# VisionLearningGroup/UDA_PoseEstimation

Hardware: AMD Instinct MI355X
Metric: images/sec (student+teacher step) 256x256 b=32 (higher is better)
Workload: dtype bf16; 1 GPU; pose_resnet101 K=16 mean-teacher step (student fwd+bwd on 2x32, teacher fwd on 32, JointsMSE+Cons, Adam, EMA), 256x256, b=32/GPU, no AdaIN (BASELINE.json configs[1]); global_batch=32, parallelism=dp1

## Files before the change

include/udapose.h:

```cpp
#ifndef UDAPOSE_H
#define UDAPOSE_H
#include <stddef.h>
#include <stdint.h>
#ifdef __cplusplus
extern "C" {
#endif

#define UDAPOSE_OK 0
#define UDAPOSE_ERR_ARG (-1)
#define UDAPOSE_ERR_LAUNCH (-2)
#define UDAPOSE_ERR_UNSUPPORTED (-3)
#define UDAPOSE_ERR_NOT_PREPARED (-4)

int udapose_version(void);
int udapose_elem_kind(void);

typedef struct {
    int igemm_tile, igemm_h3, igemm_lean, igemm_short_lds, igemm_tap0;
    int wgrad_tile, wgrad_ksplit, wgrad_fastgeo;
    int wgrad_group, wgrad_stages, wgrad_group_stem;
    int bn_bwd_fused, bn_fwd_chunked, bn_bwd_chunked, bn_bwd_pre_legacy;
    int igemm_wg_min;
    int wgrad_row3;
    int bn3_mask;
    int stem_fused;
    int debug_sync;
    int igemm_big_min;
    int patch_conv;
    int eval_fold;
    int bn_xcd_rows;
    int wgrad_det;
    int igemm_ns3_k;
    void* timeline;
} udapose_policy;
void udapose_policy_default(udapose_policy* p);

typedef struct {
    int N, Hi, Wi, Ci;
    int Co, KH, KW, stride, pad;
    int transposed;
    int reflect;
    int upsample;
    const udapose_policy* policy;
} udapose_conv_desc;
int udapose_conv_prepare(const udapose_conv_desc* d);

#define UDAPOSE_EPI_RELU 1
#define UDAPOSE_EPI_OUT_F32 2
#define UDAPOSE_EPI_F32 4
#define UDAPOSE_EPI_SPLIT 8
void udapose_conv_out_hw(const udapose_conv_desc* d, int* Ho, int* Wo);
int udapose_conv_stat_rows(const udapose_conv_desc* d);
int udapose_conv2d_fwd(void* stream, const udapose_conv_desc* d, const void* x, const void* w_fwd, void* y, const void* res,
                       const float* bias, float* stats, int epilogue_flags);
int udapose_conv2d_bwd_data(void* stream, const udapose_conv_desc* d, const void* dy, const void* w_bwd, void* dx, const void* res,
                            int out_f32);
int udapose_conv_bwd_stat_rows(const udapose_conv_desc* d);
int udapose_conv2d_bwd_data_bn(void* stream, const udapose_conv_desc* d, const void* dy, const void* w_bwd, void* dx, const void* res,
                               int out_f32, const void* bn_y, const void* bn_z, const float* bn_mean, const float* bn_invstd,
                               const float* bn_gamma, const float* bn_beta, float* slab);
int udapose_conv2d_bwd_weight(void* stream, const udapose_conv_desc* d, const void* dy, const void* x, float* dw, int accumulate);
int udapose_cast_f32_bf16(void* stream, const float* src, void* dst, size_t n);
int udapose_transpose_cast(void* stream, const float* src, void* dst, int A, int T, int B);
int udapose_pack_strided(void* stream, const float* src, void* dst, int A, int KH, int KWp, int KW, int Bp, int B, long sa, long skh,
                         long skw, long sb);

int udapose_nchw_f32_to_nhwc_bf16(void* stream, const float* src, void* dst, int N, int C, int HW, int Cpad);
int udapose_nchw_f32_to_nhwc_f32(void* stream, const float* src, float* dst, int N, int C, int HW, int Cpad);
int udapose_nchw_f32_to_nhwc_split(void* stream, const float* src, void* dst, int N, int C, int HW, int Cpad);
int udapose_f32_to_split(void* stream, const float* src, void* dst, size_t n);
int udapose_split_to_f32(void* stream, const void* src, float* dst, size_t n);
int udapose_nhwc_to_nchw_f32(void* stream, const void* src, int src_is_f32, float* dst, int N, int C, int HW, int Cstride,
                             const float* lo, const float* hi);

int udapose_bn_finalize(void* stream, const float* stats, int stat_rows, int C, double count, const float* gamma, const float* beta,
                        float* running_mean, float* running_var, long long* num_batches_tracked, float momentum, float eps,
                        float* scale, float* shift, float* save_mean, float* save_invstd);
int udapose_bn_eval_coeff(void* stream, int C, const float* gamma, const float* beta, const float* running_mean,
                          const float* running_var, float eps, float* scale, float* shift);
int udapose_bn_apply(void* stream, const void* y, const void* res, void* z, size_t numel, int C, const float* scale, const float* shift,
                     int relu);
int udapose_bn_bwd_rows(size_t npix);
int udapose_bn_bwd(void* stream, const void* dz, int dz_is_f32, const void* z, const void* y, void* dy, void* gout, size_t npix, int C,
                   const float* gamma, const float* save_mean, const float* save_invstd, int relu, float* slab, float* coef,
                   float* dgamma, float* dbeta, float beta_acc, const float* beta);
int udapose_bn_bwd_pre(void* stream, const void* g, int g_is_f32, const void* y, void* dy, size_t npix, int C, const float* gamma,
                       const float* save_mean, const float* save_invstd, const float* slab, int rows, float* coef, float* dgamma,
                       float* dbeta, float beta_acc);

int udapose_maxpool3x3s2_fwd(void* stream, const void* x, void* y, unsigned char* idx, int N, int H, int W, int C);
int udapose_maxpool3x3s2_bwd(void* stream, const void* dy, const unsigned char* idx, void* dx, int N, int H, int W, int C);
int udapose_maxpool2x2_ceil(void* stream, const void* x, void* y, int N, int H, int W, int C);
int udapose_maxpool2x2_ceil_f32(void* stream, const float* x, float* y, int N, int H, int W, int C);
int udapose_maxpool2x2_ceil_split(void* stream, const void* x, void* y, int N, int H, int W, int C);

typedef void* udapose_net_t;
int udapose_net_create(const int layers[4], int num_keypoints, int N, int H, int W, int fp32, udapose_net_t* out);
void udapose_net_destroy(udapose_net_t net);
int udapose_net_num_params(udapose_net_t net);
int udapose_net_num_buffers(udapose_net_t net);
long long udapose_net_param_numel(udapose_net_t net, int i);
size_t udapose_net_wpack_bytes(udapose_net_t net);
size_t udapose_net_act_bytes(udapose_net_t net);
size_t udapose_net_ws_bytes(udapose_net_t net);
void udapose_net_out_shape(udapose_net_t net, int shape[4]);
int udapose_net_set_policy(udapose_net_t net, const udapose_policy* p);
int udapose_net_get_policy(udapose_net_t net, udapose_policy* p);
int udapose_net_bind(udapose_net_t net, const void* const* h_params, void* const* h_buffers, void* wpack);
int udapose_net_bind_grads(udapose_net_t net, void* const* h_grads);
int udapose_net_pack_weights(udapose_net_t net, void* stream, const void* const* h_params, void* wpack, int with_bwd);
int udapose_net_forward(udapose_net_t net, void* stream, const float* x_nchw, const void* const* h_params, void* const* h_buffers,
                        const void* wpack, void* act, void* ws, float* out_nchw, int training, float momentum);
int udapose_net_apply_running(udapose_net_t net, void* stream, const void* act, void* const* h_buffers, float momentum);
int udapose_axpy_f32(void* stream, float* y, const float* x, size_t n);
int udapose_net_backward(udapose_net_t net, void* stream, const float* dout_nchw, const void* const* h_params, const void* wpack,
                         void* act, void* ws, void* const* h_grads, float beta);
int udapose_net_backward_part(udapose_net_t net, void* stream, const float* dout_nchw, const void* const* h_params, const void* wpack,
                              void* act, void* ws, void* const* h_grads, float beta, int part);
int udapose_net_backward_phase(udapose_net_t net, void* stream, const float* dout_nchw, const void* const* h_params, const void* wpack,
                               void* act, void* ws, void* const* h_grads, float beta, int part, int phase);
int udapose_net_wgrad_pair(udapose_net_t net, void* stream, const void* act_a, void* ws_a, void* const* h_grads_a, float beta_a,
                           const void* act_b, void* ws_b, void* const* h_grads_b, float beta_b, int part);
long long udapose_net_grad_split_param(udapose_net_t net);

int udapose_joints_mse_fwd(void* stream, const float* pred, const float* gt, const float* w, int R, int HW, float* rows, float* mean_out);
int udapose_joints_mse_bwd(void* stream, const float* pred, const float* gt, const float* w, const float* gscale, int R, int HW,
                           float* dpred);
int udapose_cons_loss_fwd(void* stream, const float* stu, const float* tea, const unsigned char* mask, int R, int HW, float* rows,
                          float* mean_out);
int udapose_cons_loss_bwd(void* stream, const float* stu, const float* tea, const unsigned char* mask, const float* gscale, int R,
                          int HW, float* dstu);
int udapose_mask_count(void* stream, const unsigned char* mask, size_t n, float* count);
int udapose_cons_loss_valid_fwd(void* stream, const float* stu, const float* tea, const unsigned char* mask, const unsigned char* valid,
                                const float* valid_count, int R, int K, int HW, float* rows, float* mean_out);
int udapose_cons_loss_valid_bwd(void* stream, const float* stu, const float* tea, const unsigned char* mask, const unsigned char* valid,
                                const float* valid_count, const float* gscale, int R, int K, int HW, float* dstu);
int udapose_joints_kl_fwd(void* stream, const float* pred, const float* gt, const float* w, float epsilon, int R, int group, int HW, float* rows,
                          float* stats, float* out);
int udapose_joints_kl_bwd(void* stream, const float* pred, const float* gt, const float* w, float epsilon, const float* stats,
                          const float* gscale, int R, int HW, float* dpred);
int udapose_entropy_loss_fwd(void* stream, const float* x, int R, int group, int HW, float threshold, float* rows, float* stats, float* out,
                             float* count);
int udapose_entropy_loss_bwd(void* stream, const float* x, const float* rows, const float* stats, const float* count, const float* gscale,
                             float threshold, int R, int HW, float* dx);
int udapose_cons_softmax_fwd(void* stream, const float* stu, const float* tea, const unsigned char* mask, const unsigned char* valid,
                             const float* valid_count, int R, int K, int HW, float* rows, float* stats, float* out);
int udapose_cons_softmax_bwd(void* stream, const float* stu, const float* tea, const unsigned char* mask, const unsigned char* valid,
                             const float* valid_count, const float* stats, const float* gscale, int R, int K, int HW, float* dstu);
int udapose_cons_kl_fwd(void* stream, const float* stu, const float* tea, const unsigned char* mask, const unsigned char* valid,
                        const float* valid_count, int log_target, int R, int K, int HW, float* rows, float* stats, float* out);
int udapose_cons_kl_bwd(void* stream, const float* stu, const float* tea, const unsigned char* mask, const unsigned char* valid,
                        const float* valid_count, int log_target, const float* stats, const float* gscale, int R, int K, int HW, float* dstu);
int udapose_heatmap_argmax(void* stream, const float* hm, int R, int H, int W, float* maxvals, int* flat_idx, float* preds_xy,
                           float* rectified, const float* patch, int rad);
int udapose_kth_mask(void* stream, const float* act, const float* tea_mask, int n, int k, float* thr_out, unsigned char* mask,
                     const float* act_local, int n_local);
int udapose_pck(void* stream, const float* pred_xy, const float* gt_xy, int B, int K, float norm_x, float norm_y, float thr, float* acc,
                float* avg_cnt);

int udapose_multi_chunk(void);
int udapose_ema_multi(void* stream, const long long* tgt_ptrs, const long long* src_ptrs, const long long* sizes, const int* blk_tensor,
                      const long long* blk_off, int nblocks, float alpha, float one_minus_alpha);
int udapose_adam_multi(void* stream, const long long* p, const long long* g, const long long* m, const long long* v,
                       const long long* sizes, const int* blk_tensor, const long long* blk_off, int nblocks, float lr, float beta1,
                       float beta2, float eps, float weight_decay, int step, float grad_scale, float* dev_state);
int udapose_sgd_multi(void* stream, const long long* p, const long long* g, const long long* buf, const long long* sizes,
                      const int* blk_tensor, const long long* blk_off, int nblocks, float lr, float momentum, float weight_decay,
                      int nesterov, int first_step, float grad_scale, float* dev_state);

int udapose_net_bind_update(udapose_net_t student, udapose_net_t teacher, void* const* h_params_s, void* const* h_grads,
                            void* const* h_exp_avg, void* const* h_exp_avg_sq, void* const* h_params_t, void* wpack_s, void* wpack_t);
int udapose_net_fused_update(udapose_net_t student, udapose_net_t teacher, void* stream, void* const* h_params_s, void* const* h_grads,
                             void* const* h_exp_avg, void* const* h_params_t, void* wpack_s, void* wpack_t, float lr, float beta1,
                             float beta2, float eps, float weight_decay, int step, float grad_scale, float* dev_state, float alpha,
                             float one_minus_alpha, int do_adam, long long grad2_delta_bytes);
// ... 67 lines not shown
```

uda_poseestimation_amd/_hip.py:

```python
import ctypes as C
import os

import torch

_HERE = os.path.dirname(os.path.abspath(__file__))
LIB_PATH = os.path.join(_HERE, "libudapose_hip.so")
LIB_PATHS = {"bf16": LIB_PATH, "fp16": os.path.join(_HERE, "libudapose_hip_f16.so")}
_libs = {}

vp, ci, cf, cd, sz, ll, cl = C.c_void_p, C.c_int, C.c_float, C.c_double, C.c_size_t, C.c_longlong, C.c_long


class Policy(C.Structure):
    _fields_ = [(k, C.c_int) for k in ("igemm_tile", "igemm_h3", "igemm_lean", "igemm_short_lds", "igemm_tap0", "wgrad_tile", "wgrad_ksplit",
                                       "wgrad_fastgeo", "wgrad_group", "wgrad_stages", "wgrad_group_stem", "bn_bwd_fused", "bn_fwd_chunked",
                                       "bn_bwd_chunked", "bn_bwd_pre_legacy", "igemm_wg_min", "wgrad_row3", "bn3_mask", "stem_fused", "debug_sync", "igemm_big_min", "patch_conv",
                                       "eval_fold", "bn_xcd_rows", "wgrad_det", "igemm_ns3_k")] + [("timeline", C.c_void_p)]


def policy(**overrides):
    p = Policy()
    lib().udapose_policy_default(C.byref(p))
    for k, v in overrides.items():
        if k not in dict(Policy._fields_):
            raise KeyError(f"udapose_policy has no field {k!r}")
        setattr(p, k, v)
    return p


class ConvDesc(C.Structure):
    _fields_ = [(k, C.c_int) for k in ("N", "Hi", "Wi", "Ci", "Co", "KH", "KW", "stride", "pad", "transposed", "reflect", "upsample")] + \
               [("policy", C.POINTER(Policy))]


_SIGS = {
    "udapose_version": (ci, []),
    "udapose_elem_kind": (ci, []),
    "udapose_grad_scaler_check": (ci, [vp, vp, vp, vp, vp, ci, vp]),
    "udapose_grad_scaler_check2": (ci, [vp, vp, vp, vp, vp, ci, vp, ll]),
    "udapose_grad_scaler_update": (ci, [vp, vp, cf, cf, ci]),
    "udapose_policy_default": (None, [vp]),
    "udapose_conv_prepare": (ci, [vp]),
    "udapose_net_set_policy": (ci, [vp, vp]),
    "udapose_net_get_policy": (ci, [vp, vp]),
    "udapose_net_bind": (ci, [vp, vp, vp, vp]),
    "udapose_net_bind_grads": (ci, [vp, vp]),
    "udapose_conv_out_hw": (None, [vp, vp, vp]),
    "udapose_conv_stat_rows": (ci, [vp]),
    "udapose_conv2d_fwd": (ci, [vp, vp, vp, vp, vp, vp, vp, vp, ci]),
    "udapose_conv2d_bwd_data": (ci, [vp, vp, vp, vp, vp, vp, ci]),
    "udapose_conv_bwd_stat_rows": (ci, [vp]),
    "udapose_conv2d_bwd_data_bn": (ci, [vp, vp, vp, vp, vp, vp, ci, vp, vp, vp, vp, vp, vp, vp]),
    "udapose_conv2d_bwd_weight": (ci, [vp, vp, vp, vp, vp, ci]),
    "udapose_cast_f32_bf16": (ci, [vp, vp, vp, sz]),
    "udapose_transpose_cast": (ci, [vp, vp, vp, ci, ci, ci]),
    "udapose_pack_strided": (ci, [vp, vp, vp, ci, ci, ci, ci, ci, ci, cl, cl, cl, cl]),
    "udapose_nchw_f32_to_nhwc_bf16": (ci, [vp, vp, vp, ci, ci, ci, ci]),
    "udapose_nchw_f32_to_nhwc_f32": (ci, [vp, vp, vp, ci, ci, ci, ci]),
    "udapose_nhwc_to_nchw_f32": (ci, [vp, vp, ci, vp, ci, ci, ci, ci, vp, vp]),
    "udapose_nchw_f32_to_nhwc_split": (ci, [vp, vp, vp, ci, ci, ci, ci]),
    "udapose_f32_to_split": (ci, [vp, vp, vp, sz]),
    "udapose_split_to_f32": (ci, [vp, vp, vp, sz]),
    "udapose_maxpool2x2_ceil_split": (ci, [vp, vp, vp, ci, ci, ci, ci]),
    "udapose_adain_split": (ci, [vp, vp, vp, vp, ci, ci, ci, ci, cf, cf, vp, vp]),
    "udapose_bn_finalize": (ci, [vp, vp, ci, ci, cd, vp, vp, vp, vp, vp, cf, cf, vp, vp, vp, vp]),
    "udapose_bn_eval_coeff": (ci, [vp, ci, vp, vp, vp, vp, cf, vp, vp]),
    "udapose_bn_apply": (ci, [vp, vp, vp, vp, sz, ci, vp, vp, ci]),
    "udapose_bn_bwd_rows": (ci, [sz]),
    "udapose_bn_bwd": (ci, [vp, vp, ci, vp, vp, vp, vp, sz, ci, vp, vp, vp, ci, vp, vp, vp, vp, cf, vp]),
    "udapose_bn_bwd_pre": (ci, [vp, vp, ci, vp, vp, sz, ci, vp, vp, vp, vp, ci, vp, vp, vp, cf]),
    "udapose_maxpool3x3s2_fwd": (ci, [vp, vp, vp, vp, ci, ci, ci, ci]),
    "udapose_maxpool3x3s2_bwd": (ci, [vp, vp, vp, vp, ci, ci, ci, ci]),
    "udapose_maxpool2x2_ceil": (ci, [vp, vp, vp, ci, ci, ci, ci]),
    "udapose_maxpool2x2_ceil_f32": (ci, [vp, vp, vp, ci, ci, ci, ci]),
    "udapose_net_create": (ci, [vp, ci, ci, ci, ci, ci, vp]),
    "udapose_net_destroy": (None, [vp]),
    "udapose_net_num_params": (ci, [vp]),
    "udapose_net_num_buffers": (ci, [vp]),
    "udapose_net_param_numel": (ll, [vp, ci]),
    "udapose_net_wpack_bytes": (sz, [vp]),
    "udapose_net_act_bytes": (sz, [vp]),
    "udapose_net_ws_bytes": (sz, [vp]),
    "udapose_net_out_shape": (None, [vp, vp]),
    "udapose_net_pack_weights": (ci, [vp, vp, vp, vp, ci]),
    "udapose_net_forward": (ci, [vp, vp, vp, vp, vp, vp, vp, vp, vp, ci, cf]),
    "udapose_net_apply_running": (ci, [vp, vp, vp, vp, cf]),
    "udapose_axpy_f32": (ci, [vp, vp, vp, sz]),
    "udapose_net_backward": (ci, [vp, vp, vp, vp, vp, vp, vp, vp, cf]),
    "udapose_net_backward_part": (ci, [vp, vp, vp, vp, vp, vp, vp, vp, cf, ci]),
    "udapose_net_backward_phase": (ci, [vp, vp, vp, vp, vp, vp, vp, vp, cf, ci, ci]),
    "udapose_net_wgrad_pair": (ci, [vp, vp, vp, vp, vp, cf, vp, vp, vp, cf, ci]),
    "udapose_net_grad_split_param": (ll, [vp]),
    "udapose_net_bind_update": (ci, [vp, vp, vp, vp, vp, vp, vp, vp, vp]),
    "udapose_net_fused_update": (ci, [vp, vp, vp, vp, vp, vp, vp, vp, vp, cf, cf, cf, cf, cf, ci, cf, vp, cf, cf, ci, ll]),
    "udapose_joints_mse_fwd": (ci, [vp, vp, vp, vp, ci, ci, vp, vp]),
    "udapose_joints_mse_bwd": (ci, [vp, vp, vp, vp, vp, ci, ci, vp]),
    "udapose_cons_loss_fwd": (ci, [vp, vp, vp, vp, ci, ci, vp, vp]),
    "udapose_cons_loss_bwd": (ci, [vp, vp, vp, vp, vp, ci, ci, vp]),
    "udapose_mask_count": (ci, [vp, vp, sz, vp]),
    "udapose_cons_loss_valid_fwd": (ci, [vp, vp, vp, vp, vp, vp, ci, ci, ci, vp, vp]),
    "udapose_cons_loss_valid_bwd": (ci, [vp, vp, vp, vp, vp, vp, vp, ci, ci, ci, vp]),
    "udapose_joints_kl_fwd": (ci, [vp, vp, vp, vp, cf, ci, ci, ci, vp, vp, vp]),
    "udapose_joints_kl_bwd": (ci, [vp, vp, vp, vp, cf, vp, vp, ci, ci, vp]),
    "udapose_entropy_loss_fwd": (ci, [vp, vp, ci, ci, ci, cf, vp, vp, vp, vp]),
    "udapose_entropy_loss_bwd": (ci, [vp, vp, vp, vp, vp, vp, cf, ci, ci, vp]),
    "udapose_cons_softmax_fwd": (ci, [vp, vp, vp, vp, vp, vp, ci, ci, ci, vp, vp, vp]),
    "udapose_cons_softmax_bwd": (ci, [vp, vp, vp, vp, vp, vp, vp, vp, ci, ci, ci, vp]),
    "udapose_cons_kl_fwd": (ci, [vp, vp, vp, vp, vp, vp, ci, ci, ci, ci, vp, vp, vp]),
    "udapose_cons_kl_bwd": (ci, [vp, vp, vp, vp, vp, vp, ci, vp, vp, ci, ci, ci, vp]),
    "udapose_heatmap_argmax": (ci, [vp, vp, ci, ci, ci, vp, vp, vp, vp, vp, ci]),
    "udapose_kth_mask": (ci, [vp, vp, vp, ci, ci, vp, vp, vp, ci]),
    "udapose_pck": (ci, [vp, vp, vp, ci, ci, cf, cf, cf, vp, vp]),
    "udapose_multi_chunk": (ci, []),
    "udapose_ema_multi": (ci, [vp, vp, vp, vp, vp, vp, ci, cf, cf]),
    "udapose_adam_multi": (ci, [vp, vp, vp, vp, vp, vp, vp, vp, ci, cf, cf, cf, cf, cf, ci, cf, vp]),
    "udapose_sgd_multi": (ci, [vp, vp, vp, vp, vp, vp, vp, ci, cf, cf, cf, ci, ci, cf, vp]),
    "udapose_comm_pack_bf16": (ci, [vp, vp, ll, vp, ll]),
    "udapose_comm_shard_mean": (ci, [vp, vp, ci, ll, vp]),
    "udapose_comm_unpack_bf16": (ci, [vp, vp, vp, ll]),
    "udapose_adain": (ci, [vp, vp, vp, vp, ci, ci, ci, ci, cf, cf, vp]),
    "udapose_adain_f32": (ci, [vp, vp, vp, vp, ci, ci, ci, ci, cf, cf, vp]),
    "udapose_adain_alpha_dev": (ci, [vp, vp, vp, vp, ci, ci, ci, ci, cf, vp, vp, ci]),
    "udapose_patch_paste": (ci, [vp, vp, vp, ci, ci, ci, ci, ci]),
    "udapose_occlusion_pick": (ci, [vp, vp, vp, vp, ci, ci, ci, cd, ci, cf, cf, ci, vp, vp]),
    "udapose_select_rows": (ci, [vp, vp, vp, vp, vp, ci, sz]),
    "udapose_aug_affine_u8": (ci, [vp, vp, vp, vp, ci, ci, ci]),
    "udapose_aug_color_op": (ci, [vp, vp, vp, vp, vp, ci, ci]),
    "udapose_aug_to_tensor": (ci, [vp, vp, vp, ci, ci, vp, vp]),
    "udapose_aug_gaussian_blur_u8": (ci, [vp, vp, vp, vp, ci, ci, ci]),
    "udapose_aug_resized_crop_u8": (ci, [vp, vp, vp, vp, vp, vp, vp, ci, ci, ci, ci, ci]),
    "udapose_gaussian_labels": (ci, [vp, vp, vp, vp, vp, ci, ci, ci, cd, cd, vp, ci]),
    "udapose_split_saturations": (ci, [ci, vp]),
    "udapose_mean_views": (ci, [vp, vp, ci, vp, sz]),
    "udapose_draw_labelmap_ori": (ci, [vp, vp, vp, vp, vp, vp, ci, ci, ci, cf, vp, ci]),
    "udapose_prof_begin": (None, []),
    "udapose_prof_end": (ci, [vp]),
    "udapose_affine_nearest": (ci, [vp, vp, vp, vp, ci, ci, ci, ci, ci, ci]),
    "udapose_recon_thetas": (ci, [vp, vp, ci, cd, vp, vp]),
    "udapose_conv_bwd_ws_bytes": (ll, [vp]),
    "udapose_conv_bwd_prepare": (ci, [vp]),
    "udapose_conv2d_bwd_data_reflect_padded": (ci, [vp, vp, vp, vp, vp]),
    "udapose_reflect_fold": (ci, [vp, vp, ci, vp, ci, vp, vp, vp, vp, cf, vp, ci, vp, ci, ci, ci, ci, cf]),
    "udapose_conv2d_bwd_data_reflect": (ci, [vp, vp, vp, vp, vp, vp, vp]),
    "udapose_conv2d_bwd_weight_reflect": (ci, [vp, vp, vp, vp, vp, ci, vp, cf]),
# ... 72 lines not shown
```

uda_poseestimation_amd/csrc/capi.hip:

```cpp
#include <cstdio>
#include "conv_plan.h"
#include "../../include/udapose.h"

int pw_nchw_f32_to_nhwc_bf16(hipStream_t, const float*, elem_t*, int, int, int, int);
int pw_nhwc_to_nchw_f32(hipStream_t, const void*, int, float*, int, int, int, int, const float*, const float*);
int pw_cast_f32_bf16(hipStream_t, const float*, elem_t*, size_t);
int pw_transpose_cast(hipStream_t, const float*, elem_t*, int, int, int);
int pw_pack_strided(hipStream_t, const float*, elem_t*, int, int, int, int, int, int, long, long, long, long);
int pw_bn_finalize(hipStream_t, const float*, int, int, double, const float*, const float*, float*, float*, long long*, float, float, float*, float*,
                   float*, float*, const float*);
int pw_bn_eval_coeff(hipStream_t, int, const float*, const float*, const float*, const float*, float, float*, float*);
int pw_bn_apply(hipStream_t, const elem_t*, const elem_t*, elem_t*, size_t, int, const float*, const float*, int, unsigned char*, int);
int pw_bn_bwd_rows(size_t);
int pw_bn_bwd_pre(hipStream_t, const void*, int, const elem_t*, elem_t*, size_t, int, const float*, const float*, const float*, const float*, int, float*,
                  float*, float*, float, int, int);
int pw_bn_bwd(hipStream_t, const void*, int, const elem_t*, const elem_t*, elem_t*, elem_t*, size_t, int, const float*, const float*, const float*, int,
              float*, float*, float*, float*, float, const float*, int);
int pw_maxpool3x3s2_fwd(hipStream_t, const elem_t*, elem_t*, unsigned char*, int, int, int, int);

size_t conv_bwd_ws_bytes(const ConvGeom& g);
int conv_bwd_prepare(const ConvGeom& g);
int conv_dgrad_reflect_padded(hipStream_t s, const ConvGeom& g, const elem_t* dy, const elem_t* w_bwd, elem_t* dP);
int reflect_fold(hipStream_t s, const elem_t* dP, int up, const elem_t* x, int mask, const float* stats, const float* gs_s, const elem_t* t,
                 const float* gs_c, float c_scale, const float* add_nchw, int add_c, elem_t* dx, int N, int H, int W, int C, float term_scale);
// ... 35 lines not shown
int opt_ema(hipStream_t, const long long*, const long long*, const long long*, const int*, const long long*, int, float, float);
int opt_adam(hipStream_t, const long long*, const long long*, const long long*, const long long*, const long long*, const int*, const long long*, int,
             float, float, float, float, float, int, float, float*);
int opt_sgd(hipStream_t, const long long*, const long long*, const long long*, const long long*, const int*, const long long*, int, float, float, float,
            int, int, float, float*);
int opt_grad_check(hipStream_t, const long long*, const long long*, const int*, const long long*, int, float*, long long);
int opt_scaler_update(hipStream_t, float*, float, float, int);
int comm_pack_bf16(hipStream_t, const float*, long long, void*, long long);
int comm_shard_mean(hipStream_t, const void*, int, long long, void*);
int comm_unpack_bf16(hipStream_t, const void*, float*, long long);
int adain_launch(hipStream_t, const elem_t*, const elem_t*, elem_t*, int, int, int, int, float, float, const float*, float*);
int aug_affine_u8(hipStream_t, const unsigned char*, unsigned char*, const long long*, int, int, int);
int aug_color_op(hipStream_t, unsigned char*, const int*, const float*, int*, int, int);
int aug_gaussian_blur_u8(hipStream_t, unsigned char*, unsigned char*, const unsigned int*, int, int, int);
int aug_resized_crop_u8(hipStream_t, const unsigned char*, unsigned char*, unsigned char*, const int*, const int*, const int*, int, int, int, int, int);
int aug_to_tensor(hipStream_t, const unsigned char*, float*, int, int, const float*, const float*);
int aug_gaussian_labels(hipStream_t, const double*, const float*, float*, float*, int, int, int, double, double, const float*, int);
int aug_draw_labelmap_ori(hipStream_t, const float*, const float*, const unsigned char*, float*, float*, int, int, int, float, const float*, int);
int affine_warp_chain(hipStream_t, const float*, float*, const float*, int, int, int, int, int, int);
int affine_recon_thetas(hipStream_t, const double*, int, double, float*, float*);
int affine_mean_views(hipStream_t, const float* const*, int, float*, size_t);
unsigned long long sp_sat_read_adain(int);
unsigned long long sp_sat_read_igemm(int);
unsigned long long sp_sat_read_patchconv(int);
unsigned long long sp_sat_read_pointwise(int);
int patch_paste(hipStream_t, float*, const int*, int, int, int, int, int);
int occlusion_pick(hipStream_t, const float*, const int*, const float*, int, int, int, double, int, float, float, int, int*, unsigned char*);
int select_rows(hipStream_t, float*, const float*, const float*, const unsigned char*, int, size_t);
int net_apply_running(void*, hipStream_t, const void*, void* const*, float);
int pw_axpy(hipStream_t, float*, const float*, size_t);
void prof_begin();
int prof_end(double*);
void* net_create(const int layers[4], int K, int N, int H, int W, int mode);
void net_destroy(void*);
void net_set_policy(void*, const Policy&);
const Policy& net_get_policy(void*);
int net_bind(void*, const void* const*, void* const*, void*);
int net_bind_grads(void*, void* const*);
long long net_grad_split_param(void*);
int net_bind_update(void*, void*, void* const*, void* const*, void* const*, void* const*, void* const*, void*, void*);
int net_fused_update(void*, void*, hipStream_t, void* const*, void* const*, void* const*, void* const*, void*, void*, float, float, float, float, float,
                     int, float, float*, float, float, int, long long);
int net_num_params(void*);
int net_num_buffers(void*);
long long net_param_numel(void*, int);
size_t net_wpack_bytes(void*);
size_t net_act_bytes(void*);
size_t net_ws_bytes(void*);
void net_out_shape(void*, int*);
int net_pack_weights(void*, hipStream_t, const void* const*, void*, int);
int net_forward(void*, hipStream_t, const float*, const void* const*, void* const*, const void*, void*, void*, float*, int, float);
int net_backward(void*, hipStream_t, const float*, const void* const*, const void*, void*, void*, void* const*, float, int, int);
int net_wgrad_pair(void*, hipStream_t, const void*, void*, void* const*, float, const void*, void*, void* const*, float, int);

static Policy from_c(const udapose_policy& c) {
    Policy p;
    p.igemm_tile = c.igemm_tile; p.igemm_h3 = c.igemm_h3; p.igemm_lean = c.igemm_lean; p.igemm_short_lds = c.igemm_short_lds;
    p.igemm_tap0 = c.igemm_tap0; p.wgrad_tile = c.wgrad_tile; p.wgrad_ksplit = c.wgrad_ksplit; p.wgrad_fastgeo = c.wgrad_fastgeo;
    p.wgrad_group = c.wgrad_group; p.wgrad_stages = c.wgrad_stages > 0 ? c.wgrad_stages : 128; p.wgrad_group_stem = c.wgrad_group_stem;
    p.bn_bwd_fused = c.bn_bwd_fused; p.bn_fwd_chunked = c.bn_fwd_chunked; p.bn_bwd_chunked = c.bn_bwd_chunked;
    p.bn_bwd_pre_legacy = c.bn_bwd_pre_legacy; p.igemm_wg_min = c.igemm_wg_min; p.wgrad_row3 = c.wgrad_row3; p.bn3_mask = c.bn3_mask; p.stem_fused = c.stem_fused; p.debug_sync = c.debug_sync; p.igemm_big_min = c.igemm_big_min; p.patch_conv = c.patch_conv; p.eval_fold = c.eval_fold; p.bn_xcd_rows = c.bn_xcd_rows; p.igemm_ns3_k = c.igemm_ns3_k; p.wgrad_det = c.wgrad_det; p.timeline = (unsigned long long*)c.timeline;
    return p;
}
static void to_c(const Policy& p, udapose_policy* c) {
    c->igemm_tile = p.igemm_tile; c->igemm_h3 = p.igemm_h3; c->igemm_lean = p.igemm_lean; c->igemm_short_lds = p.igemm_short_lds;
    c->igemm_tap0 = p.igemm_tap0; c->wgrad_tile = p.wgrad_tile; c->wgrad_ksplit = p.wgrad_ksplit; c->wgrad_fastgeo = p.wgrad_fastgeo;
    c->wgrad_group = p.wgrad_group; c->wgrad_stages = p.wgrad_stages; c->wgrad_group_stem = p.wgrad_group_stem;
    c->bn_bwd_fused = p.bn_bwd_fused; c->bn_fwd_chunked = p.bn_fwd_chunked; c->bn_bwd_chunked = p.bn_bwd_chunked;
    c->bn_bwd_pre_legacy = p.bn_bwd_pre_legacy; c->igemm_wg_min = p.igemm_wg_min; c->wgrad_row3 = p.wgrad_row3; c->bn3_mask = p.bn3_mask; c->stem_fused = p.stem_fused; c->debug_sync = p.debug_sync; c->igemm_big_min = p.igemm_big_min; c->patch_conv = p.patch_conv; c->eval_fold = p.eval_fold; c->bn_xcd_rows = p.bn_xcd_rows; c->igemm_ns3_k = p.igemm_ns3_k; c->wgrad_det = p.wgrad_det; c->timeline = p.timeline;
}
struct Geom {
    Policy pol;
    ConvGeom g;
    explicit Geom(const udapose_conv_desc* d)
        : g{d->N, d->Hi, d->Wi, d->Ci, d->Co, d->KH, d->KW, d->stride, d->pad, d->transposed, d->reflect, d->upsample} {
        if (d->policy) { pol = from_c(*d->policy); g.pol = &pol; }
    }
};
#define S(x) ((hipStream_t)(x))
#define B16(x) ((elem_t*)(x))
#define CB16(x) ((const elem_t*)(x))

extern "C" {

int udapose_version(void) { return 200; }
int udapose_elem_kind(void) { return UDAPOSE_ELEM_KIND; }

void udapose_policy_default(udapose_policy* p) { if (p) to_c(default_policy(), p); }
void udapose_conv_out_hw(const udapose_conv_desc* d, int* Ho, int* Wo) { Geom G(d); *Ho = G.g.Ho(); *Wo = G.g.Wo(); }
int udapose_conv_stat_rows(const udapose_conv_desc* d) { Geom G(d); return conv_stat_rows(G.g); }
int udapose_conv_prepare(const udapose_conv_desc* d) { if (!d) return UDAPOSE_ERR_ARG; Geom G(d); return conv_prepare(G.g); }
int udapose_conv2d_fwd(void* stream, const udapose_conv_desc* d, const void* x, const void* w_fwd, void* y, const void* res, const float* bias,
                       float* stats, int flags) {
    if (!d || !x || !w_fwd || !y) return UDAPOSE_ERR_ARG;
    ConvEpilogue e;
    e.res = CB16(res); e.bias = bias; e.stats = stats; e.relu = (flags & UDAPOSE_EPI_RELU) != 0; e.out_f32 = (flags & UDAPOSE_EPI_OUT_F32) != 0; e.f32 = (flags & UDAPOSE_EPI_F32) != 0;
    e.split = (flags & UDAPOSE_EPI_SPLIT) != 0;
    if (e.split && e.f32) return UDAPOSE_ERR_ARG;
    Geom G(d);
    return conv_fprop(S(stream), G.g, CB16(x), CB16(w_fwd), y, e);
}
int udapose_conv2d_bwd_data(void* stream, const udapose_conv_desc* d, const void* dy, const void* w_bwd, void* dx, const void* res, int out_f32) {
    if (!d || !dy || !w_bwd || !dx) return UDAPOSE_ERR_ARG;
    Geom G(d);
    return conv_dgrad(S(stream), G.g, CB16(dy), CB16(w_bwd), dx, CB16(res), out_f32);
}
int udapose_conv_bwd_stat_rows(const udapose_conv_desc* d) { if (!d) return UDAPOSE_ERR_ARG; Geom G(d); return conv_dgrad_stat_rows(G.g); }
int udapose_conv2d_bwd_data_bn(void* stream, const udapose_conv_desc* d, const void* dy, const void* w_bwd, void* dx, const void* res, int out_f32,
                               const void* bn_y, const void* bn_z, const float* bn_mean, const float* bn_invstd, const float* bn_gamma,
                               const float* bn_beta, float* slab) {
    if (!d || !dy || !w_bwd || !dx || !bn_y || !bn_mean || !bn_invstd || !slab) return UDAPOSE_ERR_ARG;
    DgradBnStat st;
    st.y = CB16(bn_y); st.z = CB16(bn_z); st.mean = bn_mean; st.invstd = bn_invstd; st.gamma = bn_gamma; st.beta = bn_beta; st.slab = slab;
    Geom G(d);
    return conv_dgrad(S(stream), G.g, CB16(dy), CB16(w_bwd), dx, CB16(res), out_f32, &st);
}
int udapose_conv2d_bwd_weight(void* stream, const udapose_conv_desc* d, const void* dy, const void* x, float* dw, int accumulate) {
    if (!d || !dy || !x || !dw) return UDAPOSE_ERR_ARG;
    Geom G(d);
    return conv_wgrad(S(stream), G.g, CB16(dy), CB16(x), dw, accumulate, -1);
}
int udapose_cast_f32_bf16(void* stream, const float* src, void* dst, size_t n) { return pw_cast_f32_bf16(S(stream), src, B16(dst), n); }
// ... 69 lines not shown
    return *out ? UDAPOSE_OK : UDAPOSE_ERR_ARG;
}
void udapose_net_destroy(udapose_net_t n) { net_destroy(n); }
int udapose_net_set_policy(udapose_net_t n, const udapose_policy* p) {
    if (!n || !p) return UDAPOSE_ERR_ARG;
    net_set_policy(n, from_c(*p));
    return UDAPOSE_OK;
}
int udapose_net_get_policy(udapose_net_t n, udapose_policy* p) {
    if (!n || !p) return UDAPOSE_ERR_ARG;
    to_c(net_get_policy(n), p);
    return UDAPOSE_OK;
}
int udapose_net_bind(udapose_net_t n, const void* const* params, void* const* buffers, void* wpack) {
    if (!n || !params || !wpack) return UDAPOSE_ERR_ARG;
    return net_bind(n, params, buffers, wpack);
}
int udapose_net_bind_grads(udapose_net_t n, void* const* grads) {
    if (!n || !grads) return UDAPOSE_ERR_ARG;
    return net_bind_grads(n, grads);
}
int udapose_net_num_params(udapose_net_t n) { return net_num_params(n); }
int udapose_net_num_buffers(udapose_net_t n) { return net_num_buffers(n); }
long long udapose_net_param_numel(udapose_net_t n, int i) { return net_param_numel(n, i); }
size_t udapose_net_wpack_bytes(udapose_net_t n) { return net_wpack_bytes(n); }
size_t udapose_net_act_bytes(udapose_net_t n) { return net_act_bytes(n); }
size_t udapose_net_ws_bytes(udapose_net_t n) { return net_ws_bytes(n); }
void udapose_net_out_shape(udapose_net_t n, int shape[4]) { net_out_shape(n, shape); }
int udapose_net_pack_weights(udapose_net_t n, void* stream, const void* const* params, void* wpack, int with_bwd) {
    return net_pack_weights(n, S(stream), params, wpack, with_bwd);
}
int udapose_net_forward(udapose_net_t n, void* stream, const float* x, const void* const* params, void* const* buffers, const void* wpack, void* act,
                        void* ws, float* out, int training, float momentum) {
    return net_forward(n, S(stream), x, params, buffers, wpack, act, ws, out, training, momentum);
}
int udapose_net_apply_running(udapose_net_t n, void* stream, const void* act, void* const* buffers, float momentum) {
    return net_apply_running(n, S(stream), act, buffers, momentum);
}
int udapose_axpy_f32(void* stream, float* y, const float* x, size_t n) { return pw_axpy(S(stream), y, x, n); }
int udapose_net_backward(udapose_net_t n, void* stream, const float* dout, const void* const* params, const void* wpack, void* act, void* ws,
                         void* const* grads, float beta) {
    return net_backward(n, S(stream), dout, params, wpack, act, ws, grads, beta, 0, 0);
}
int udapose_net_backward_part(udapose_net_t n, void* stream, const float* dout, const void* const* params, const void* wpack, void* act,
                              void* ws, void* const* grads, float beta, int part) {
    if (part != 1 && part != 2) return UDAPOSE_ERR_ARG;
    return net_backward(n, S(stream), dout, params, wpack, act, ws, grads, beta, part, 0);
}
int udapose_net_wgrad_pair(udapose_net_t n, void* stream, const void* act_a, void* ws_a, void* const* grads_a, float beta_a, const void* act_b,
                           void* ws_b, void* const* grads_b, float beta_b, int part) {
    if (!n || !act_a || !ws_a || !grads_a || !act_b || !ws_b || !grads_b) return UDAPOSE_ERR_ARG;
    return net_wgrad_pair(n, S(stream), act_a, ws_a, grads_a, beta_a, act_b, ws_b, grads_b, beta_b, part);
}
int udapose_net_backward_phase(udapose_net_t n, void* stream, const float* dout, const void* const* params, const void* wpack, void* act,
                               void* ws, void* const* grads, float beta, int part, int phase) {
    if (!n) return UDAPOSE_ERR_ARG;
    return net_backward(n, S(stream), dout, params, wpack, act, ws, grads, beta, part, phase);
}
long long udapose_net_grad_split_param(udapose_net_t n) { return net_grad_split_param(n); }
int udapose_net_bind_update(udapose_net_t student, udapose_net_t teacher, void* const* params_s, void* const* grads, void* const* exp_avg,
                            void* const* exp_avg_sq, void* const* params_t, void* wpack_s, void* wpack_t) {
    if (!student || !teacher || !params_s || !grads || !exp_avg || !exp_avg_sq || !params_t || !wpack_s || !wpack_t) return UDAPOSE_ERR_ARG;
    return net_bind_update(student, teacher, params_s, grads, exp_avg, exp_avg_sq, params_t, wpack_s, wpack_t);
}
int udapose_net_fused_update(udapose_net_t student, udapose_net_t teacher, void* stream, void* const* params_s, void* const* grads,
                             void* const* exp_avg, void* const* params_t, void* wpack_s, void* wpack_t, float lr, float beta1, float beta2,
                             float eps, float weight_decay, int step, float grad_scale, float* dev_state, float alpha, float one_minus_alpha,
                             int do_adam, long long grad2_delta_bytes) {
    if (!student || !teacher) return UDAPOSE_ERR_ARG;
    return net_fused_update(student, teacher, S(stream), params_s, grads, exp_avg, params_t, wpack_s, wpack_t, lr, beta1, beta2, eps, weight_decay,
                            step, grad_scale, dev_state, alpha, one_minus_alpha, do_adam, grad2_delta_bytes);
}

int udapose_joints_mse_fwd(void* stream, const float* pred, const float* gt, const float* w, int R, int HW, float* rows, float* mean_out) {
    return hm_sqdiff_rows(S(stream), pred, gt, w, nullptr, R, HW, 0.5f, rows, mean_out, nullptr, nullptr, 1);
}
int udapose_joints_mse_bwd(void* stream, const float* pred, const float* gt, const float* w, const float* gscale, int R, int HW, float* dpred) {
    return hm_sqdiff_bwd(S(stream), pred, gt, w, nullptr, gscale, (float)(1.0 / ((double)R * HW)), R, HW, dpred, nullptr, nullptr, 1);
}
int udapose_cons_loss_fwd(void* stream, const float* stu, const float* tea, const unsigned char* mask, int R, int HW, float* rows, float* mean_out) {
    return hm_sqdiff_rows(S(stream), stu, tea, nullptr, mask, R, HW, 1.0f, rows, mean_out, nullptr, nullptr, 1);
}
int udapose_cons_loss_bwd(void* stream, const float* stu, const float* tea, const unsigned char* mask, const float* gscale, int R, int HW, float* dstu) {
    return hm_sqdiff_bwd(S(stream), stu, tea, nullptr, mask, gscale, (float)(2.0 / ((double)R * HW)), R, HW, dstu, nullptr, nullptr, 1);
}
int udapose_mask_count(void* stream, const unsigned char* mask, size_t n, float* count) {
    if (!mask || !count) return UDAPOSE_ERR_ARG;
    return hm_mask_count(S(stream), mask, n, count);
}
int udapose_cons_loss_valid_fwd(void* stream, const float* stu, const float* tea, const unsigned char* mask, const unsigned char* valid,
                                const float* valid_count, int R, int K, int HW, float* rows, float* mean_out) {
    if (!valid || !valid_count) return UDAPOSE_ERR_ARG;
    return hm_sqdiff_rows(S(stream), stu, tea, nullptr, mask, R, HW, 1.0f, rows, mean_out, valid, valid_count, K);
}
int udapose_cons_loss_valid_bwd(void* stream, const float* stu, const float* tea, const unsigned char* mask, const unsigned char* valid,
                                const float* valid_count, const float* gscale, int R, int K, int HW, float* dstu) {
    if (!valid || !valid_count) return UDAPOSE_ERR_ARG;
    return hm_sqdiff_bwd(S(stream), stu, tea, nullptr, mask, gscale, (float)(2.0 / ((double)R * HW)), R, HW, dstu, valid, valid_count, K);
}
int udapose_joints_kl_fwd(void* stream, const float* pred, const float* gt, const float* w, float epsilon, int R, int group, int HW, float* rows,
                          float* stats, float* out) {
    return sml_kl_fwd(S(stream), pred, gt, w, epsilon, R, group, HW, rows, stats, out);
}
int udapose_joints_kl_bwd(void* stream, const float* pred, const float* gt, const float* w, float epsilon, const float* stats,
                          const float* gscale, int R, int HW, float* dpred) {
    return sml_kl_bwd(S(stream), pred, gt, w, epsilon, stats, gscale, R, HW, dpred);
// ... 206 lines not shown
```

uda_poseestimation_amd/csrc/conv_plan.h:

```cpp
#pragma once
#include <atomic>
#include <mutex>
#include <vector>
#include "igemm.h"

struct Policy {
    int igemm_tile = -1;
    int igemm_h3 = 1;
    int igemm_lean = 1;
    int igemm_short_lds = 1;
    int igemm_tap0 = 1;
    int wgrad_tile = -1;
    int wgrad_ksplit = -1;
    int wgrad_fastgeo = 2;
    int wgrad_group = 1;
    int wgrad_stages = 128;
    int wgrad_group_stem = 1;
    int bn_bwd_fused = 1;
    int bn_fwd_chunked = 1;
    int bn_bwd_chunked = 1;
    int bn_bwd_pre_legacy = 0;
    int igemm_wg_min = 512;
    int wgrad_row3 = 1;
    int bn3_mask = 1;
    int stem_fused = 1;
    int igemm_big_min = 0;
    int patch_conv = 2;
    int eval_fold = 1;
    int bn_xcd_rows = 1;
    int wgrad_det = 1;
    int igemm_ns3_k = 0;
    int debug_sync = 0;
    unsigned long long* timeline = nullptr;
};
inline const Policy& default_policy() { static const Policy p; return p; }

template <typename F>
inline void once_per_device(std::atomic<unsigned long long>& done, std::mutex& mu, F&& f) {
    int dev = 0;
    (void)hipGetDevice(&dev);
    const unsigned long long bit = 1ull << (dev & 63);
    if (done.load(std::memory_order_acquire) & bit) return;
    std::lock_guard<std::mutex> lk(mu);
    if (done.load(std::memory_order_relaxed) & bit) return;
    f();
    done.fetch_or(bit, std::memory_order_release);
}

struct ConvGeom {
    int N, Hi, Wi, Ci;
    int Co, KH, KW, stride, pad;
    int transposed;
    int reflect;
    int upsample;
    const Policy* pol = nullptr;
    const Policy& policy() const { return pol ? *pol : default_policy(); }
    int Ho() const { return transposed ? (Hi - 1) * stride - 2 * pad + KH : (((Hi << upsample) + 2 * pad - KH) / stride + 1); }
    int Wo() const { return transposed ? (Wi - 1) * stride - 2 * pad + KW : (((Wi << upsample) + 2 * pad - KW) / stride + 1); }
    bool smallc() const { return Ci == 8; }
    int KWp() const { return smallc() ? ((KW + 7) & ~7) : KW; }
    int wtaps() const { return KH * KWp(); }
};

struct TapPlan {
    std::vector<IgTap> taps;
    int nclass = 1;
    IgClass cls[4];
    const IgTap* d_taps = nullptr;
};

const TapPlan* get_tap_plan(const ConvGeom& g, int direction, hipStream_t stream = nullptr);
int conv_prepare(const ConvGeom& g);

int igemm_pick_tile(int M, int Co, int nclass, int K, int h3_ok, const Policy& pol);
int conv_h3_ok(const ConvGeom& g);
int igemm_stat_rows(int M, int Co, int nclass, int tile);
int igemm_launch(IgParams& p, int tile, hipStream_t stream, const Policy& pol);
int wgrad_pick_tile(int Rdim, int Cdim, int smallc, const Policy& pol);
int wgrad_launch(WgParams& p, int tile, int accumulate, hipStream_t stream, const Policy& pol);
int wgrad_parts_plan(int M, int Ci, int Co, int total_taps, int* tile_out);
int wgrad_launch_parts(WgParams& p, float* parts, hipStream_t stream);
#define WG_CLASSES 2
int wgrad_group_plan(WgParams& p, int accumulate, int stages_per_block, const Policy& pol);
int wgrad_group_launch(hipStream_t stream, int tile, const WgParams* d_tab, const WgGroupBlk* d_blk, int per_xcd, const void* x_base,
                       const void* dy_base, void* dw_base, const WgParams* d_tab2 = nullptr, const WgGroupBlk* d_blk2 = nullptr,
                       const void* x_base2 = nullptr, const void* dy_base2 = nullptr, void* dw_base2 = nullptr);

struct ConvEpilogue {
    const elem_t* res = nullptr;
    const float* bias = nullptr;
    const float* scale = nullptr;
    float* stats = nullptr;
    int relu = 0;
    int out_f32 = 0;
    int f32 = 0;
    int split = 0;
};
int conv_fprop(hipStream_t s, const ConvGeom& g, const elem_t* x, const elem_t* w_fwd, void* y, const ConvEpilogue& e);
int patch_conv_ok(const ConvGeom& g, const ConvEpilogue& e);
int patch_conv_fprop(hipStream_t s, const ConvGeom& g, const void* x, const void* w_fwd, void* y, const ConvEpilogue& e);
struct DgradBnStat {
    const elem_t* y = nullptr;
    const elem_t* z = nullptr;
    const unsigned char* mask = nullptr;
    const float* mean = nullptr; const float* invstd = nullptr; const float* gamma = nullptr; const float* beta = nullptr;
    float* slab = nullptr;
    int rows = 0;
};
int conv_dgrad(hipStream_t s, const ConvGeom& g, const elem_t* dy, const elem_t* w_bwd, void* dx, const elem_t* res, int out_f32,
               DgradBnStat* bs = nullptr);
int conv_wgrad(hipStream_t s, const ConvGeom& g, const elem_t* dy, const elem_t* x, float* dw, int accumulate, int rows_valid);
int conv_wgrad_params(const ConvGeom& g, const elem_t* dy, const elem_t* x, float* dw, int rows_valid, WgParams* out, double* flops);
int conv_prof_before(hipStream_t s, int kind, double flops);
void conv_prof_after(hipStream_t s, int token);
int conv_stat_rows(const ConvGeom& g);
int conv_dgrad_stat_rows(const ConvGeom& g);
```

uda_poseestimation_amd/csrc/net.hip:

```cpp
#include <algorithm>
#include <deque>
#include <cstdio>
#include <cstdlib>
#include <string>
#include <vector>
#include "conv_plan.h"

int pw_nchw_f32_to_nhwc_bf16(hipStream_t, const float*, elem_t*, int, int, int, int);
int pw_nhwc_to_nchw_f32(hipStream_t, const void*, int, float*, int, int, int, int, const float*, const float*);
int pw_cast_f32_bf16(hipStream_t, const float*, elem_t*, size_t);
int pw_transpose_cast(hipStream_t, const float*, elem_t*, int, int, int);
int pw_pack_strided(hipStream_t, const float*, elem_t*, int, int, int, int, int, int, long, long, long, long);
int pw_unpack_strided(hipStream_t, const float*, float*, int, int, int, int, int, int, long, long, long, long, float);
int pw_bn_finalize(hipStream_t, const float*, int, int, double, const float*, const float*, float*, float*, long long*, float, float, float*, float*,
                   float*, float*, const float*);
int pw_bn_eval_coeff(hipStream_t, int, const float*, const float*, const float*, const float*, float, float*, float*);
int pw_bn_apply(hipStream_t, const elem_t*, const elem_t*, elem_t*, size_t, int, const float*, const float*, int, unsigned char*, int);
int pw_bn_bwd_rows(size_t);
int pw_bn_bwd(hipStream_t, const void*, int, const elem_t*, const elem_t*, elem_t*, elem_t*, size_t, int, const float*, const float*, const float*, int,
              float*, float*, float*, float*, float, const float*, int);
int pw_bn_bwd_pre(hipStream_t, const void*, int, const elem_t*, elem_t*, size_t, int, const float*, const float*, const float*, const float*, int, float*,
                  float*, float*, float, int, int);
int pw_maxpool3x3s2_fwd(hipStream_t, const elem_t*, elem_t*, unsigned char*, int, int, int, int);
int pw_maxpool3x3s2_bwd(hipStream_t, const elem_t*, const unsigned char*, elem_t*, int, int, int, int);
int pw_bn_relu_maxpool3x3s2(hipStream_t, const elem_t*, elem_t*, unsigned char*, int, int, int, int, const float*, const float*);
int pw_bn_bwd_pooled(hipStream_t, const elem_t*, const unsigned char*, int, int, const elem_t*, elem_t*, size_t, int, const float*, const float*,
                     const float*, float*, float*, float*, float*, float, const float*);
int pw_plane_sum(hipStream_t, const float*, float*, int, int, int, float);
int pw_bn_running_update(hipStream_t, const float*, int, float*, float*, long long*, float);
int pw_bn_running_update_multi(hipStream_t, const BnRunJob*, int, int, const void*, float);
int pw_bn_train_fused(hipStream_t, const elem_t*, const elem_t*, elem_t*, size_t, int, const float*, int, const float*, const float*, float*, float*,
                      long long*, float, float, float*, int, int, unsigned char*);
int pw_zero_multi(hipStream_t, const ZeroJob*, int, void*);
int pw_pack_multi(hipStream_t, const void*, const int*, const int*, int);
int pw_nchw_f32_to_nhwc_f32(hipStream_t, const float*, float*, int, int, int, int);
size_t opt_tail_job_bytes();
int opt_chunk();
void opt_tail_job_fill(void*, float*, const float*, float*, float*, float*, void*, void*, void*, void*, int, int, int, int, long long);
int opt_tail(hipStream_t, const void*, const int*, const int*, int, float, float, float, float, float, int, float, float*, float, float, int, long long, int);
int pw_transpose_f32(hipStream_t, const float*, float*, int, int, int);
int pw_pack_strided_f32(hipStream_t, const float*, float*, int, int, int, int, int, int, long, long, long, long);
int pw_bn_apply_f32(hipStream_t, const float*, const float*, float*, size_t, int, const float*, const float*, int);
int pw_maxpool3x3s2_fwd_f32(hipStream_t, const float*, float*, unsigned char*, int, int, int, int);
int pw_nchw_f32_to_nhwc_split(hipStream_t, const float*, void*, int, int, int, int, void*);
int pw_f32_to_split(hipStream_t, const float*, void*, size_t);
int pw_transpose_split(hipStream_t, const float*, void*, int, int, int);
int pw_pack_strided_split(hipStream_t, const float*, void*, int, int, int, int, int, int, long, long, long, long);
int pw_bn_apply_split(hipStream_t, const float*, const void*, void*, size_t, int, const float*, const float*, int, void*, void*, unsigned char*, int);
int pw_bn_train_fused_split(hipStream_t, const float*, const void*, void*, size_t, int, const float*, int, const float*, const float*, float*, float*,
                            long long*, float, float, float*, int, int, void*, void*, unsigned char*);
int pw_maxpool3x3s2_fwd_split(hipStream_t, const void*, void*, unsigned char*, int, int, int, int, void*);

namespace {

inline size_t align_up(size_t v, size_t a = 256) { return (v + a - 1) / a * a; }
static thread_local int t_dbg_sync = 0;
struct DbgSyncScope { int prev; explicit DbgSyncScope(int on) : prev(t_dbg_sync) { t_dbg_sync = on; } ~DbgSyncScope() { t_dbg_sync = prev; } };
#define CK(expr) do { int _e = (expr); \
    if (t_dbg_sync) { fprintf(stderr, "[udapose] net.hip:%d %s\n", __LINE__, #expr); fflush(stderr); \
        if (hipDeviceSynchronize() != hipSuccess) { fprintf(stderr, "[udapose] FAILED at net.hip:%d\n", __LINE__); return UDAPOSE_ERR_LAUNCH; } } \
    if (_e != UDAPOSE_OK) return _e; } while (0)

struct ConvL {
    ConvGeom g;
    int w_idx = -1;
    int bias_idx = -1;
    size_t wf_off = 0, wb_off = 0;
    size_t in_off = 0;
    size_t y_off = 0;
    size_t fin_off = 0, fy_off = 0;
    size_t dy_off = 0;
};
struct BnL {
    int C = 0;
    int g_idx = -1, b_idx = -1;
    int rm_idx = -1, rv_idx = -1, nbt_idx = -1;
    size_t save_off = 0;
    size_t z_off = 0;
    size_t mask_off = 0;
    size_t fz_off = 0;
    size_t npix = 0;
};
struct Block {
    ConvL c1, c2, c3, cd;
    BnL b1, b2, b3, bd;
    bool has_ds = false;
    size_t in_off = 0, zd_off = 0;
    size_t fin_off = 0, fzd_off = 0;
    size_t npix_in = 0;
};

struct Net {
    int layers[4], K, N, H, W;
    int split_dz_idx = -1;
    Policy policy;
    int f32 = 0;
    int strict = 0;
    int fwd_only = 0;
    struct Scratch { size_t need[6] = {0, 0, 0, 0, 0, 0}, off[6] = {0, 0, 0, 0, 0, 0}; bool sizing = false; } sc;
    int deconv_bias = 0;
    size_t es = 2;
    int n_params = 0, n_buffers = 0;
    std::vector<long long> param_numel;
    ConvL stem; BnL stem_bn;
    size_t x8_off = 0, pool_off = 0, poolidx_off = 0;
    size_t fx8_off = 0, fpool_off = 0;
    int Hs = 0, Ws = 0, Hp = 0, Wp = 0;
    std::vector<Block> blocks;
    ConvL up[3]; BnL up_bn[3];
    ConvL head;
    size_t head_out_off = 0;
    int fc_w_idx = -1, fc_b_idx = -1;
    size_t act_bytes = 0, wpack_bytes = 0, ws_bytes = 0;
    size_t ws_slab = 0, ws_slabf = 0, ws_coef = 0, ws_gbuf[6] = {0, 0, 0, 0, 0, 0}, ws_dyhead = 0, ws_dwtmp = 0, ws_headbwd = 0;
    size_t ws_wgpart = 0, ws_wgpart_bytes = 0;
    size_t gbuf_bytes = 0;
    int Hout = 0, Wout = 0;
    struct PackTab { void* jobs = nullptr; int* blk_job = nullptr; int* blk_sub = nullptr; int nblocks = 0; const void* key0 = nullptr;
                     const void* key1 = nullptr; const void* keyw = nullptr; };
    PackTab pack_fwd, pack_all;
    struct WgGroup {
        float k_beta = -1.f; int k_stages = 0; int k_part = 0;
        bool k_det = false, k_stem = false;
        size_t part_bytes = 0;
        std::vector<std::pair<int, ptrdiff_t>> rel;
        std::vector<size_t> rel_bytes;
        std::vector<int> rel_cls;
        WgParams* d_tab[WG_CLASSES] = {}; WgGroupBlk* d_blk[WG_CLASSES] = {}; int per_xcd[WG_CLASSES] = {};
        double flops[WG_CLASSES] = {};
        std::vector<std::pair<ptrdiff_t, size_t>> zero;
        ZeroJob* d_zero = nullptr; int n_zero = 0;
        SumJob* d_sum = nullptr; int* d_sum_blk = nullptr; int n_sum_blk = 0;
        unsigned long long last_use = 0;
    };
    std::deque<WgGroup> wg_groups;
    struct UpdTab { void* jobs = nullptr; int* blk_job = nullptr; int* blk_sub = nullptr; int nblocks = 0;
                    const void* k_ps = nullptr; const void* k_pt = nullptr; const void* k_g = nullptr; const void* k_m = nullptr;
                    const void* k_ws = nullptr; const void* k_wt = nullptr; };
    UpdTab upd;
    BnRunJob* d_runjobs = nullptr; int n_runjobs = 0; const void* runjobs_key = nullptr;
    unsigned long long wg_tick = 0;
};
struct PackJobH { const float* src; elem_t* dst; int A, T, B, kind; long long n; };

size_t act_alloc(Net& n, size_t bytes) { size_t o = n.act_bytes; n.act_bytes = align_up(o + bytes); return o; }
size_t wp_alloc(Net& n, size_t bytes) { size_t o = n.wpack_bytes; n.wpack_bytes = align_up(o + bytes); return o; }

enum { SC_Y = 0, SC_A, SC_B, SC_MID, SC_MID2, SC_DS, SC_COUNT };
size_t sc_take(Net& n, int slot, size_t bytes) {
    if (n.sc.sizing) { n.sc.need[slot] = std::max(n.sc.need[slot], align_up(bytes)); return 0; }
    return n.sc.off[slot];
}
void add_conv(Net& n, ConvL& c, int Hi, int Wi, int Ci, int Co, int K, int stride, int pad, int transposed, size_t in_off, size_t fin_off, bool need_bwd_pack,
              int y_slot = -1) {
    c.g = ConvGeom{n.N, Hi, Wi, Ci, Co, K, K, stride, pad, transposed, 0, 0};
    c.w_idx = n.n_params++;
    n.param_numel.push_back((long long)Co * (Ci == 8 ? 3 : Ci) * K * K);
    c.in_off = in_off;
    c.fin_off = fin_off;
    const size_t welems = (size_t)Co * c.g.wtaps() * Ci;
    if (n.f32 != 1 || c.g.smallc() || transposed) c.wf_off = wp_alloc(n, welems * (n.f32 ? 4 : 2));
    if (need_bwd_pack && (!n.f32 || n.strict)) c.wb_off = wp_alloc(n, welems * 2);
    const size_t ybytes = (size_t)n.N * c.g.Ho() * c.g.Wo() * Co * n.es;
    c.y_off = (n.fwd_only && y_slot >= 0) ? sc_take(n, y_slot, ybytes) : act_alloc(n, ybytes);
    c.fy_off = n.strict ? sc_take(n, y_slot, (size_t)n.N * c.g.Ho() * c.g.Wo() * Co * 4) : c.y_off;
}
void add_bn(Net& n, BnL& b, int C, size_t npix, bool alloc_z = true, int z_slot = -1) {
    b.C = C;
    b.g_idx = n.n_params++; n.param_numel.push_back(C);
    b.b_idx = n.n_params++; n.param_numel.push_back(C);
    b.rm_idx = n.n_buffers++; b.rv_idx = n.n_buffers++; b.nbt_idx = n.n_buffers++;
    b.save_off = act_alloc(n, (size_t)3 * C * 4);
    b.npix = npix;
    if (alloc_z) {
        b.z_off = (n.fwd_only && z_slot >= 0) ? sc_take(n, z_slot, npix * C * n.es) : act_alloc(n, npix * C * n.es);
        b.fz_off = n.strict ? sc_take(n, z_slot, npix * C * 4) : b.z_off;
    }
}

Net* build(const int layers[4], int K, int N, int H, int W, int mode) {
    Net* np = new Net();
    Net& n = *np;
    const int f32 = mode & 0xff;
    n.deconv_bias = (mode >> 8) & 1;
    n.strict = f32 == 3;
    n.f32 = f32 >= 2 ? 2 : (f32 ? 1 : 0);
    n.es = (f32 && !n.strict) ? 4 : 2;
    for (int i = 0; i < 4; ++i) n.layers[i] = layers[i];
    n.K = K; n.N = N; n.H = H; n.W = W;
    n.fwd_only = (mode >> 9) & 1;
    auto layout = [&](Net& n) {
    const bool fo = n.fwd_only != 0;
// ... 409 lines not shown
    if (pre)
        CK(pw_bn_bwd_pre(s, dz, dz_f32, (const elem_t*)(act + c.y_off), dy, b.npix, b.C, (const float*)params[b.g_idx], save, save + b.C, pre->slab,
                         pre->rows, coef, (float*)grads[b.g_idx], (float*)grads[b.b_idx], beta, n.policy.bn_bwd_chunked | (n.policy.bn_xcd_rows ? (1 << 30) : 0) | (n.policy.bn_xcd_rows >= 2 ? (1 << 29) : 0),
                         n.policy.bn_bwd_pre_legacy));
    else
        CK(pw_bn_bwd(s, dz, dz_f32, (const elem_t*)(act + b.z_off), (const elem_t*)(act + c.y_off), dy, gout, b.npix, b.C, (const float*)params[b.g_idx],
                     save, save + b.C, relu, slab, coef, (float*)grads[b.g_idx], (float*)grads[b.b_idx], beta, (const float*)params[b.b_idx],
                     n.policy.bn_bwd_chunked));
    const elem_t* xin = (const elem_t*)(act + c.in_off);
    if (c.bias_idx >= 0 && beta == 0.f) {
        if (pw_zero(s, grads[c.bias_idx], (size_t)c.g.Co * sizeof(float)) != UDAPOSE_OK) return UDAPOSE_ERR_LAUNCH;
    }
    if (c.g.smallc() && grouped_wgrad && n.policy.wgrad_group_stem) {
    } else if (c.g.smallc()) {
        float* tmp = (float*)(ws + n.ws_dwtmp);
        CK(conv_wgrad(s, c.g, dy, xin, tmp, 0, -1));
        CK(pw_unpack_strided(s, tmp, (float*)grads[c.w_idx], c.g.Co, c.g.KH, c.g.KWp(), c.g.KW, 8, 3, (long)c.g.KH * c.g.KW * 3, (long)c.g.KW * 3, 3, 1,
                             beta));
    } else if (!grouped_wgrad) {
        CK(conv_wgrad(s, c.g, dy, xin, (float*)grads[c.w_idx], beta != 0.f, -1));
    }
    if (need_dx) {
        elem_t* dx = pool.get();
        if (!dx) return UDAPOSE_ERR_ARG;
        CK(conv_dgrad(s, c.g, dy, (const elem_t*)(wpack + c.wb_off), dx, dx_res, dx_f32, next));
        *dx_out = dx;
    }
    return UDAPOSE_OK;
}

DgradBnStat bn_stat_of(const Net& n, const ConvL& c, const BnL& b, const void* const* params, char* act, char* ws, int relu) {
    DgradBnStat st;
    const float* save = (const float*)(act + b.save_off);
    st.y = (const elem_t*)(act + c.y_off);
    st.z = relu == 1 ? (const elem_t*)(act + b.z_off) : nullptr;
    st.mask = (relu == 1 && b.mask_off && n.policy.bn3_mask) ? (const unsigned char*)(act + b.mask_off) : nullptr;
    st.mean = save; st.invstd = save + b.C;
    st.gamma = (const float*)params[b.g_idx]; st.beta = (const float*)params[b.b_idx];
    st.slab = (float*)(ws + n.ws_slabf);
    return st;
}


inline int split_block(const Net& n) { return n.layers[0] + n.layers[1]; }

struct PartSel { bool head_up; int hi, lo; bool stem; };
PartSel part_sel(const Net& n, int part) {
    const int nb = (int)n.blocks.size(), split = split_block(n);
    if (part == 1) return PartSel{true, nb - 1, split, false};
    if (part == 2) return PartSel{false, split - 1, 0, true};
    return PartSel{true, nb - 1, 0, true};
}

int build_wg_group(Net& n, Net::WgGroup& G, void* const* grads, float beta, int part, bool sizing = false, size_t* need = nullptr) {
    const PartSel sel = part_sel(n, part);
    const bool upper = sel.head_up, lower = sel.stem;
    std::vector<WgParams> tab[WG_CLASSES];
    struct Unit { int prob, z, nblk; long load; };
    std::vector<Unit> units[WG_CLASSES];
    G.zero.clear();
    G.rel.clear();
    G.rel_bytes.clear();
    G.rel_cls.clear();
    for (int t = 0; t < WG_CLASSES; ++t) G.flops[t] = 0.0;
    std::vector<SumJob> sums;
    size_t part_cur = 0;
    const bool det = n.policy.wgrad_det && n.policy.wgrad_group;
    auto make_partial = [&](WgParams& p, long long dst_off, int dst_ws, int Cdim) -> int {
        const int ms_total = (p.M + 63) / 64, per = (ms_total + p.ksplit - 1) / p.ksplit;
        const int ks_eff = (ms_total + per - 1) / per;
        const size_t span = (size_t)p.rows_valid * p.wtaps * Cdim;
        if (span >= (1ull << 31) || (span & 3)) return UDAPOSE_ERR_UNSUPPORTED;
        p.flags = (p.flags & ~WG_FLAG_ATOMIC) | WG_FLAG_DW_WS;
        p.dw = (float*)(n.ws_wgpart + part_cur);
        p.part_stride = (unsigned)span;
        sums.push_back(SumJob{(long long)(n.ws_wgpart + part_cur), dst_off, (unsigned)span, (unsigned)span, ks_eff, dst_ws, dst_ws ? 0.f : beta, 0});
        part_cur = align_up(part_cur + (size_t)ks_eff * span * sizeof(float));
        return UDAPOSE_OK;
    };
    auto add_geom = [&](const ConvGeom& g, int w_idx, size_t dy_off, size_t in_off, int rows_valid) -> int {
        if (g.smallc()) return UDAPOSE_OK;
        WgParams p;
        double fl = 0.0;
        const ptrdiff_t drel = sizing ? 0 : (const char*)grads[w_idx] - (const char*)grads[0];
        G.rel.push_back({w_idx, drel});
        CK(conv_wgrad_params(g, (const elem_t*)dy_off, (const elem_t*)in_off, (float*)drel, rows_valid, &p, &fl));
        const int t = wgrad_group_plan(p, beta != 0.f, n.policy.wgrad_stages, n.policy);
        if (t < 0) return UDAPOSE_ERR_UNSUPPORTED;
        G.rel_bytes.push_back((size_t)p.rows_valid * p.wtaps * ((p.flags & WG_FLAG_SWAP) ? p.Co : p.Ci) * sizeof(float));
        if (p.ksplit > 1) {
            const bool swap = (p.flags & WG_FLAG_SWAP) != 0;
            if (det) CK(make_partial(p, (long long)drel, 0, swap ? p.Co : p.Ci));
            else if (beta == 0.f) G.zero.push_back({drel, (size_t)p.rows_valid * p.wtaps * (swap ? p.Co : p.Ci) * sizeof(float)});
        }
        const int prob = (int)tab[t].size();
        G.rel_cls.push_back(t);
        tab[t].push_back(p);
        G.flops[t] += fl;
        const int nblk = p.r_tiles * p.c_tiles * p.total_taps;
        const int ms_total = (p.M + 63) / 64, per = (ms_total + p.ksplit - 1) / p.ksplit;
        for (int z = 0; z < p.ksplit; ++z) {
            const int st = std::min(per, ms_total - z * per);
            if (st > 0) units[t].push_back(Unit{prob, z, nblk, (long)nblk * (st + 4)});
        }
        return UDAPOSE_OK;
    };
    auto add = [&](const ConvL& c) -> int { return add_geom(c.g, c.w_idx, c.dy_off, c.in_off, -1); };
    if (upper) {
        ConvGeom hg = n.head.g;
        hg.Co = 64;
        CK(add_geom(hg, n.head.w_idx, n.ws_dyhead, n.head.in_off, n.K));
        G.flops[1] -= 2.0 * n.N * n.Hout * n.Wout * 256.0 * (64 - n.K);
    }
    if (lower && n.policy.wgrad_group_stem) {
        WgParams p;
        double fl = 0.0;
        CK(conv_wgrad_params(n.stem.g, (const elem_t*)n.stem.dy_off, (const elem_t*)n.stem.in_off, (float*)n.ws_dwtmp, -2, &p, &fl));
        p.flags |= WG_FLAG_DW_WS;
        const int t = wgrad_group_plan(p, 1, n.policy.wgrad_stages, n.policy);
        if (t != 1) return UDAPOSE_ERR_UNSUPPORTED;
        if (det) CK(make_partial(p, (long long)n.ws_dwtmp, 1, 64));
        const int prob = (int)tab[t].size();
        tab[t].push_back(p);
        G.flops[t] += fl;
        const int nblk = p.r_tiles * p.c_tiles * p.total_taps;
        const int ms_total = (p.M + 63) / 64, per = (ms_total + p.ksplit - 1) / p.ksplit;
        for (int z = 0; z < p.ksplit; ++z) {
            const int st = std::min(per, ms_total - z * per);
            if (st > 0) units[t].push_back(Unit{prob, z, nblk, (long)nblk * (st + 4)});
        }
    }
    if (upper) for (int i = 2; i >= 0; --i) CK(add(n.up[i]));
    for (int bi = sel.hi; bi >= sel.lo; --bi) {
        Block& b = n.blocks[bi];
        CK(add(b.c3)); CK(add(b.c2));
        if (b.has_ds) CK(add(b.cd));
        CK(add(b.c1));
    }
    if (sizing) { if (need) *need = part_cur; return UDAPOSE_OK; }
    if (part_cur > n.ws_wgpart_bytes) return UDAPOSE_ERR_NOT_PREPARED;
    for (int t = 0; t < WG_CLASSES; ++t) {
        if (G.d_tab[t]) { (void)hipFree(G.d_tab[t]); G.d_tab[t] = nullptr; }
        if (G.d_blk[t]) { (void)hipFree(G.d_blk[t]); G.d_blk[t] = nullptr; }
        G.per_xcd[t] = 0;
        if (tab[t].empty()) continue;
        std::stable_sort(units[t].begin(), units[t].end(), [](const Unit& a, const Unit& b) { return a.load > b.load; });
        std::vector<WgGroupBlk> lst[8];
        long load[8] = {0, 0, 0, 0, 0, 0, 0, 0};
        for (const Unit& u : units[t]) {
            int x = 0;
            for (int k = 1; k < 8; ++k) if (load[k] < load[x]) x = k;
            load[x] += u.load;
            for (int l = 0; l < u.nblk; ++l) lst[x].push_back(WgGroupBlk{u.prob, u.z * u.nblk + l});
        }
        size_t per = 0;
        for (int k = 0; k < 8; ++k) per = std::max(per, lst[k].size());
        std::vector<WgGroupBlk> flat(8 * per, WgGroupBlk{-1, 0});
        for (int k = 0; k < 8; ++k) std::copy(lst[k].begin(), lst[k].end(), flat.begin() + k * per);
        if (hipMalloc((void**)&G.d_tab[t], tab[t].size() * sizeof(WgParams)) != hipSuccess) return UDAPOSE_ERR_LAUNCH;
        if (hipMalloc((void**)&G.d_blk[t], flat.size() * sizeof(WgGroupBlk)) != hipSuccess) return UDAPOSE_ERR_LAUNCH;
        if (hipMemcpy(G.d_tab[t], tab[t].data(), tab[t].size() * sizeof(WgParams), hipMemcpyHostToDevice) != hipSuccess) return UDAPOSE_ERR_LAUNCH;
        if (hipMemcpy(G.d_blk[t], flat.data(), flat.size() * sizeof(WgGroupBlk), hipMemcpyHostToDevice) != hipSuccess) return UDAPOSE_ERR_LAUNCH;
        G.per_xcd[t] = (int)per;
    }
    if (G.d_zero) { (void)hipFree(G.d_zero); G.d_zero = nullptr; }
    G.n_zero = 0;
    bool granular = !G.zero.empty();
    for (auto& z : G.zero) granular = granular && (z.second % 16 == 0) && ((((size_t)(const char*)grads[0]) + (size_t)z.first) % 16 == 0);
    if (granular) {
        std::vector<ZeroJob> zj;
        for (auto& z : G.zero) zj.push_back(ZeroJob{(long long)z.first, (long long)(z.second / 16)});
        if (hipMalloc((void**)&G.d_zero, zj.size() * sizeof(ZeroJob)) != hipSuccess) return UDAPOSE_ERR_LAUNCH;
        if (hipMemcpy(G.d_zero, zj.data(), zj.size() * sizeof(ZeroJob), hipMemcpyHostToDevice) != hipSuccess) return UDAPOSE_ERR_LAUNCH;
        G.n_zero = (int)zj.size();
    }
    if (G.d_sum) { (void)hipFree(G.d_sum); G.d_sum = nullptr; }
    if (G.d_sum_blk) { (void)hipFree(G.d_sum_blk); G.d_sum_blk = nullptr; }
    G.n_sum_blk = 0;
    if (!sums.empty()) {
        std::vector<int> blk;
        for (size_t j = 0; j < sums.size(); ++j)
            for (unsigned c = 0; c < (sums[j].n + UDAPOSE_SPLIT_SUM_CHUNK - 1u) / UDAPOSE_SPLIT_SUM_CHUNK; ++c) { blk.push_back((int)j); blk.push_back((int)c); }
        if (hipMalloc((void**)&G.d_sum, sums.size() * sizeof(SumJob)) != hipSuccess) return UDAPOSE_ERR_LAUNCH;
        if (hipMalloc((void**)&G.d_sum_blk, blk.size() * sizeof(int)) != hipSuccess) return UDAPOSE_ERR_LAUNCH;
        if (hipMemcpy(G.d_sum, sums.data(), sums.size() * sizeof(SumJob), hipMemcpyHostToDevice) != hipSuccess) return UDAPOSE_ERR_LAUNCH;
        if (hipMemcpy(G.d_sum_blk, blk.data(), blk.size() * sizeof(int), hipMemcpyHostToDevice) != hipSuccess) return UDAPOSE_ERR_LAUNCH;
        G.n_sum_blk = (int)(blk.size() / 2);
    }
    G.k_beta = beta; G.k_stages = n.policy.wgrad_stages; G.k_part = part;
    G.k_det = det; G.k_stem = n.policy.wgrad_group_stem != 0; G.part_bytes = part_cur;
    return UDAPOSE_OK;
}

size_t wg_partial_bytes(Net& n) {
    Net::WgGroup G;
    size_t need = 0;
    if (build_wg_group(n, G, nullptr, 0.f, 0, true, &need) != UDAPOSE_OK) return 0;
    return need;
}

Net::WgGroup* find_wg_group(Net& n, void* const* grads, float beta, int part) {
    const bool det = n.policy.wgrad_det && n.policy.wgrad_group, stem = n.policy.wgrad_group_stem != 0;
    for (auto& g : n.wg_groups) {
        if (g.k_beta != beta || g.k_stages != n.policy.wgrad_stages || g.k_part != part || g.k_det != det || g.k_stem != stem) continue;
        if (g.k_det && g.part_bytes > n.ws_wgpart_bytes) continue;
        bool same = true;
        for (auto& r : g.rel)
            if ((const char*)grads[r.first] - (const char*)grads[0] != r.second) { same = false; break; }
        if (same) return &g;
    }
    return nullptr;
}
int bind_wg_groups(Net& n, void* const* grads) {
    for (const int part : {0, 1, 2})
        for (const float beta : {0.f, 1.f}) {
            if (find_wg_group(n, grads, beta, part)) continue;
            n.wg_groups.emplace_back();
            Net::WgGroup* G = &n.wg_groups.back();
            const int rc = build_wg_group(n, *G, grads, beta, part);
            if (rc != UDAPOSE_OK) { n.wg_groups.pop_back(); return rc; }
            G->last_use = ++n.wg_tick;
        }
    return UDAPOSE_OK;
}
int wg_before(hipStream_t s, Net& n, Net::WgGroup* G, char* ws, void* const* grads, bool with_stem) {
    G->last_use = ++n.wg_tick;
    if (G->d_zero) {
        CK(pw_zero_multi(s, G->d_zero, G->n_zero, grads[0]));
    } else {
        for (auto& z : G->zero)
            if (pw_zero(s, (char*)grads[0] + z.first, z.second) != UDAPOSE_OK) return UDAPOSE_ERR_LAUNCH;
    }
    const ConvGeom& sg = n.stem.g;
    if (with_stem && !G->k_det && pw_zero(s, ws + n.ws_dwtmp, (size_t)sg.Co * sg.KH * 8 * 8 * sizeof(float)) != UDAPOSE_OK) return UDAPOSE_ERR_LAUNCH;
    return UDAPOSE_OK;
}
int wg_after(hipStream_t s, Net& n, Net::WgGroup* G, char* ws, void* const* grads, float beta, bool with_stem, bool sums_done = false) {
    if (G->n_sum_blk && !sums_done) CK(pw_split_sum(s, G->d_sum, G->d_sum_blk, G->n_sum_blk, ws, (char*)grads[0]));
    const ConvGeom& sg = n.stem.g;
    if (with_stem)
        CK(pw_unpack_strided(s, (const float*)(ws + n.ws_dwtmp), (float*)grads[n.stem.w_idx], sg.Co, sg.KH, sg.KWp(), sg.KW, 8, 3,
                             (long)sg.KH * sg.KW * 3, (long)sg.KW * 3, 3, 1, beta));
    return UDAPOSE_OK;
}
bool wg_overlap(const Net& n, const Net::WgGroup* GA, void* const* gradsA, const Net::WgGroup* GB, void* const* gradsB, bool with_stem) {
    auto span = [&](const Net::WgGroup* G, void* const* grads, uintptr_t& lo, uintptr_t& hi) {
        lo = UINTPTR_MAX; hi = 0;
        auto add = [&](int idx, size_t bytes) {
            const uintptr_t a = (uintptr_t)grads[idx];
            lo = std::min(lo, a); hi = std::max(hi, a + bytes);
        };
        for (size_t i = 0; i < G->rel.size(); ++i) add(G->rel[i].first, G->rel_bytes[i]);
        if (with_stem) add(n.stem.w_idx, (size_t)n.stem.g.Co * n.stem.g.KH * n.stem.g.KW * 3 * sizeof(float));
    };
    uintptr_t la, ha, lb, hb;
    span(GA, gradsA, la, ha);
    span(GB, gradsB, lb, hb);
    return la < hb && lb < ha;
}
int run_wg_group(hipStream_t s, Net& n, const char* act, char* ws, void* const* grads, float beta, int part) {
    Net::WgGroup* G = find_wg_group(n, grads, beta, part);
    if (!G) return UDAPOSE_ERR_NOT_PREPARED;
    const bool with_stem = part_sel(n, part).stem && G->k_stem;
    CK(wg_before(s, n, G, ws, grads, with_stem));
    for (int t = 0; t < WG_CLASSES; ++t) {
        if (!G->per_xcd[t]) continue;
        const int tok = conv_prof_before(s, 2, G->flops[t]);
        const int rc = wgrad_group_launch(s, t, G->d_tab[t], G->d_blk[t], G->per_xcd[t], act, ws, grads[0]);
        conv_prof_after(s, tok);
        CK(rc);
    }
    return wg_after(s, n, G, ws, grads, beta, with_stem);
}
int run_wg_pair(hipStream_t s, Net& n, const char* actA, char* wsA, void* const* gradsA, float betaA, const char* actB, char* wsB,
                void* const* gradsB, float betaB, int part) {
    Net::WgGroup* GA = find_wg_group(n, gradsA, betaA, part);
    Net::WgGroup* GB = find_wg_group(n, gradsB, betaB, part);
    if (!GA || !GB) return UDAPOSE_ERR_NOT_PREPARED;
    bool same = true;
    for (int t = 0; t < WG_CLASSES; ++t) same = same && GA->per_xcd[t] == GB->per_xcd[t];
    const bool with_stem = part_sel(n, part).stem && GA->k_stem;
    if (same && wg_overlap(n, GA, gradsA, GB, gradsB, with_stem)) same = false;
    if (!same) {
        CK(run_wg_group(s, n, actA, wsA, gradsA, betaA, part));
        return run_wg_group(s, n, actB, wsB, gradsB, betaB, part);
    }
    CK(wg_before(s, n, GA, wsA, gradsA, with_stem));
    CK(wg_before(s, n, GB, wsB, gradsB, with_stem));
    for (int t = 0; t < WG_CLASSES; ++t) {
        if (!GA->per_xcd[t]) continue;
        const int tok = conv_prof_before(s, 2, GA->flops[t] + GB->flops[t]);
        const int rc = wgrad_group_launch(s, t, GA->d_tab[t], GA->d_blk[t], GA->per_xcd[t], actA, wsA, gradsA[0], GB->d_tab[t], GB->d_blk[t], actB, wsB,
                                          gradsB[0]);
        conv_prof_after(s, tok);
        CK(rc);
    }
    const bool pair_sum = GA == GB && GA->n_sum_blk > 0;
    if (pair_sum) CK(pw_split_sum(s, GA->d_sum, GA->d_sum_blk, GA->n_sum_blk, wsA, (char*)gradsA[0], wsB, (char*)gradsB[0]));
    CK(wg_after(s, n, GA, wsA, gradsA, betaA, with_stem, pair_sum));
    return wg_after(s, n, GB, wsB, gradsB, betaB, with_stem, pair_sum);
}
}

int net_wgrad_pair(void* h, hipStream_t s, const void* actA, void* wsA, void* const* gradsA, float betaA, const void* actB, void* wsB,
                   void* const* gradsB, float betaB, int part) {
    Net& n = *(Net*)h;
    if (part < 0 || part > 2 || (n.f32 && !n.strict) || !n.policy.wgrad_group) return UDAPOSE_ERR_ARG;
    DbgSyncScope dbg(n.policy.debug_sync);
    return run_wg_pair(s, n, (const char*)actA, (char*)wsA, gradsA, betaA, (const char*)actB, (char*)wsB, gradsB, betaB, part);
}

int net_backward(void* h, hipStream_t s, const float* dout_nchw, const void* const* params, const void* wpack_, void* act_, void* ws_,
                 void* const* grads, float beta, int part, int phase) {
    Net& n = *(Net*)h;
    if (part < 0 || part > 2 || phase < 0 || phase > 2) return UDAPOSE_ERR_ARG;
    if (phase != 0 && !n.policy.wgrad_group) return UDAPOSE_ERR_ARG;
    if (phase == 2) {
        if ((n.f32 && !n.strict) || n.fwd_only) return UDAPOSE_ERR_UNSUPPORTED;
        DbgSyncScope dbg2(n.policy.debug_sync);
        return run_wg_group(s, n, (const char*)act_, (char*)ws_, grads, beta, part);
    }
    DbgSyncScope dbg(n.policy.debug_sync);
    if ((n.f32 && !n.strict) || n.fwd_only) return UDAPOSE_ERR_UNSUPPORTED;
    const char* wpack = (const char*)wpack_;
    char* act = (char*)act_;
    char* ws = (char*)ws_;
    Pool pool;
    pool.base = ws;
    for (int i = 0; i < 6; ++i) pool.off[i] = n.ws_gbuf[i];
    const bool grouped = n.policy.wgrad_group != 0;
    if (grouped && (!find_wg_group(n, grads, beta, part))) return UDAPOSE_ERR_NOT_PREPARED;
    const int HWo = n.Hout * n.Wout;
    const int split = split_block(n);
    const bool fused = n.policy.bn_bwd_fused != 0;
    DgradBnStat cur, nxt;
    bool have = false;
    elem_t* dz = nullptr;
    if (part != 2) {
    elem_t* dyh = (elem_t*)(ws + n.ws_dyhead);
    CK(pw_nchw_f32_to_nhwc_bf16(s, dout_nchw, dyh, n.N, n.K, HWo, 64));
    ConvGeom hg = n.head.g;
    hg.Co = 64;
    float* tmp = (float*)(ws + n.ws_dwtmp);
    if (!grouped) {
        CK(conv_wgrad(s, hg, dyh, (const elem_t*)(act + n.head.in_off), tmp, 0, n.K));
        CK(pw_unpack_strided(s, tmp, (float*)grads[n.head.w_idx], n.K, 1, 1, 1, 256, 256, 256, 0, 0, 1, beta));
    }
    dz = pool.get();
    if (fused) { cur = bn_stat_of(n, n.up[2], n.up_bn[2], params, act, ws, 2); have = true; }
    CK(conv_dgrad(s, hg, dyh, (const elem_t*)(wpack + n.head.wb_off), dz, nullptr, 1, have ? &cur : nullptr));
    CK(pw_plane_sum(s, dout_nchw, (float*)grads[n.head.bias_idx], n.N, n.K, HWo, beta));
    for (int i = 2; i >= 0; --i) {
        elem_t* dx = nullptr;
        if (fused) {
            if (i > 0) nxt = bn_stat_of(n, n.up[i - 1], n.up_bn[i - 1], params, act, ws, 2);
            else nxt = bn_stat_of(n, n.blocks.back().c3, n.blocks.back().b3, params, act, ws, 1);
        }
        CK(conv_bn_bwd(s, n, n.up[i], n.up_bn[i], params, wpack, act, ws, grads, beta, pool, dz, 1, nullptr, 2, nullptr, &dx, true, i > 0, grouped,
                       have ? &cur : nullptr, fused ? &nxt : nullptr));
        if (fused) cur = nxt;
        pool.put(dz);
        dz = dx;
// ... 49 lines not shown
        const float* save = (const float*)(act + sb.save_off);
        CK(pw_bn_bwd_pooled(s, dz, (const unsigned char*)(act + n.poolidx_off), n.Hs, n.Ws, (const elem_t*)(act + n.stem.y_off),
                            (elem_t*)(ws + n.stem.dy_off), sb.npix, sb.C, (const float*)params[sb.g_idx], save, save + sb.C, (float*)(ws + n.ws_slab),
                            (float*)(ws + n.ws_coef) + 4096, (float*)grads[sb.g_idx], (float*)grads[sb.b_idx], beta, (const float*)params[sb.b_idx]));
        pool.put(dz);
    } else {
    elem_t* dzs = pool.get();
    CK(pw_maxpool3x3s2_bwd(s, dz, (const unsigned char*)(act + n.poolidx_off), dzs, n.N, n.Hs, n.Ws, 64));
    pool.put(dz);
    elem_t* none = nullptr;
    CK(conv_bn_bwd(s, n, n.stem, n.stem_bn, params, wpack, act, ws, grads, beta, pool, dzs, 0, nullptr, 2, nullptr, &none, false, 0, grouped));
    pool.put(dzs);
    }
    if (grouped && phase == 0) CK(run_wg_group(s, n, act, ws, grads, beta, part));
    if (beta == 0.f && part == 0) {
        if (pw_zero(s, grads[n.fc_w_idx], (size_t)1000 * 2048 * 4) != UDAPOSE_OK) return UDAPOSE_ERR_LAUNCH;
        if (pw_zero(s, grads[n.fc_b_idx], (size_t)1000 * 4) != UDAPOSE_OK) return UDAPOSE_ERR_LAUNCH;
    }
    return UDAPOSE_OK;
}

int net_apply_running(void* h, hipStream_t s, const void* act_, void* const* buffers, float momentum) {
    Net& n = *(Net*)h;
    if (!n.d_runjobs || n.runjobs_key != buffers[0]) return UDAPOSE_ERR_NOT_PREPARED;
    return pw_bn_running_update_multi(s, n.d_runjobs, n.n_runjobs, 2048, act_, momentum);
}
int net_bind_grads(void* h, void* const* grads) {
    Net& n = *(Net*)h;
    if (n.f32 && !n.strict) return UDAPOSE_OK;
    if (n.fwd_only) return UDAPOSE_ERR_UNSUPPORTED;
    return bind_wg_groups(n, grads);
}
long long net_grad_split_param(void* h) {
    Net& n = *(Net*)h;
    const int split = split_block(n);
    if (split < 1 || split >= (int)n.blocks.size()) return -1;
    return n.blocks[split].c1.w_idx;
}

int net_bind_update(void* hs, void* ht, void* const* params_s, void* const* grads, void* const* h_m, void* const* h_v, void* const* params_t,
                    void* wpack_s_, void* wpack_t_) {
    Net& n = *(Net*)hs;
    const Net& nt = *(const Net*)ht;
    const bool t_split = nt.f32 == 2;
    const bool s_split = n.strict != 0;
    if ((n.f32 && !s_split) || nt.f32 == 1 || nt.strict || n.n_params != nt.n_params || (!t_split && (s_split || n.wpack_bytes != nt.wpack_bytes)))
        return UDAPOSE_ERR_UNSUPPORTED;
    char* ws_ = (char*)wpack_s_;
    char* wt_ = (char*)wpack_t_;
    const size_t jb = opt_tail_job_bytes();
    std::vector<char> jobs;
    std::vector<int> bj, bs;
    std::vector<char> covered(n.n_params, 0);
    auto push = [&](int idx, void* sd, void* td, void* sx, void* tx, int A, int T, int B) -> int {
        const long long numel = n.param_numel[idx];
        const int adam = (h_m[idx] && h_v[idx] && grads[idx]) ? 1 : 0;
        if (A) {
            const uintptr_t al = (uintptr_t)params_s[idx] | (uintptr_t)params_t[idx] | (adam ? ((uintptr_t)grads[idx] | (uintptr_t)h_m[idx] | (uintptr_t)h_v[idx]) : 0);
            if ((al & 15) || (A & 63) || (B & 63) || (long long)A * T * B != numel) return UDAPOSE_ERR_UNSUPPORTED;
        }
        jobs.resize(jobs.size() + jb);
        opt_tail_job_fill(jobs.data() + jobs.size() - jb, (float*)params_s[idx], (const float*)grads[idx], (float*)h_m[idx], (float*)h_v[idx],
                          (float*)params_t[idx], sd, td, sx, tx, A, T, B, adam, numel);
        const int j = (int)(jobs.size() / jb) - 1;
        const long nb = A ? (long)(A / 64) * (B / 64) * T : (long)((numel + opt_chunk() - 1) / opt_chunk());
        for (long k = 0; k < nb; ++k) { bj.push_back(j); bs.push_back((int)k); }
        covered[idx] = 1;
        return UDAPOSE_OK;
    };
    auto conv = [&](const ConvL& c) -> int {
        const ConvGeom& g = c.g;
        const int T = g.KH * g.KW;
        if (g.smallc()) return push(c.w_idx, nullptr, nullptr, nullptr, nullptr, 0, 0, 0);
        if (!g.transposed)
            return push(c.w_idx, s_split ? nullptr : ws_ + c.wf_off, t_split ? nullptr : wt_ + c.wf_off, ws_ + c.wb_off, nullptr, g.Co, T, g.Ci);
        return push(c.w_idx, ws_ + c.wb_off, nullptr, s_split ? nullptr : ws_ + c.wf_off, t_split ? nullptr : wt_ + c.wf_off, g.Ci, T, g.Co);
    };
    CK(conv(n.stem));
    for (auto& b : n.blocks) {
        CK(conv(b.c1)); CK(conv(b.c2)); CK(conv(b.c3));
        if (b.has_ds) CK(conv(b.cd));
    }
    for (int i = 0; i < 3; ++i) CK(conv(n.up[i]));
    CK(push(n.head.w_idx, s_split ? nullptr : ws_ + n.head.wf_off, t_split ? nullptr : wt_ + n.head.wf_off, nullptr, nullptr, 0, 0, 0));
    for (int i = 0; i < n.n_params; ++i)
        if (!covered[i]) CK(push(i, nullptr, nullptr, nullptr, nullptr, 0, 0, 0));
    Net::UpdTab& u = n.upd;
    if (u.jobs) { (void)hipFree(u.jobs); (void)hipFree(u.blk_job); (void)hipFree(u.blk_sub); u.jobs = nullptr; }
    if (hipMalloc(&u.jobs, jobs.size()) != hipSuccess) return UDAPOSE_ERR_LAUNCH;
    if (hipMalloc((void**)&u.blk_job, bj.size() * sizeof(int)) != hipSuccess) return UDAPOSE_ERR_LAUNCH;
    if (hipMalloc((void**)&u.blk_sub, bs.size() * sizeof(int)) != hipSuccess) return UDAPOSE_ERR_LAUNCH;
    if (hipMemcpy(u.jobs, jobs.data(), jobs.size(), hipMemcpyHostToDevice) != hipSuccess) return UDAPOSE_ERR_LAUNCH;
    if (hipMemcpy(u.blk_job, bj.data(), bj.size() * sizeof(int), hipMemcpyHostToDevice) != hipSuccess) return UDAPOSE_ERR_LAUNCH;
    if (hipMemcpy(u.blk_sub, bs.data(), bs.size() * sizeof(int), hipMemcpyHostToDevice) != hipSuccess) return UDAPOSE_ERR_LAUNCH;
    u.nblocks = (int)bj.size();
    u.k_ps = params_s[0]; u.k_pt = params_t[0]; u.k_g = grads[0]; u.k_m = h_m[0]; u.k_ws = wpack_s_; u.k_wt = wpack_t_;
    return UDAPOSE_OK;
}

int net_fused_update(void* hs, void* ht, hipStream_t s, void* const* params_s, void* const* grads, void* const* h_m, void* const* params_t,
                     void* wpack_s_, void* wpack_t_, float lr, float beta1, float beta2, float eps, float wd, int step, float gscale,
                     float* dev_state, float alpha, float oma, int do_adam, long long grad2_delta) {
    Net& n = *(Net*)hs;
    const Net& nt = *(const Net*)ht;
    DbgSyncScope dbg(n.policy.debug_sync);
    const Net::UpdTab& u = n.upd;
    if (!u.jobs || u.k_ps != params_s[0] || u.k_pt != params_t[0] || u.k_g != grads[0] || u.k_m != h_m[0] || u.k_ws != wpack_s_ || u.k_wt != wpack_t_)
        return UDAPOSE_ERR_NOT_PREPARED;
    CK(opt_tail(s, u.jobs, u.blk_job, u.blk_sub, u.nblocks, lr, beta1, beta2, eps, wd, step, gscale, dev_state, alpha, oma, do_adam, grad2_delta, 1));
    if (n.strict)
        CK(net_pack_weights(hs, s, (const void* const*)params_s, wpack_s_, 0));
    else
        CK(pack_conv(s, n, n.stem, (const void* const*)params_s, (char*)wpack_s_, false));
    if (nt.f32 != 2) CK(pack_conv(s, nt, nt.stem, (const void* const*)params_t, (char*)wpack_t_, false));
    CK(pw_pack_strided(s, (const float*)params_s[n.head.w_idx], (elem_t*)((char*)wpack_s_ + n.head.wb_off), 256, 1, 1, 1, 64, n.K, 1, 0, 0, 256));
    return UDAPOSE_OK;
}
```

uda_poseestimation_amd/csrc/optim.hip:

```cpp
#include "common.h"

#pragma clang fp contract(off)
__device__ __forceinline__ float ema1(float p, float s, float a, float b) {
    float t1 = p * a, t2 = s * b;
    asm volatile("" : "+v"(t1), "+v"(t2));
    return t1 + t2;
}

namespace {
constexpr int TPB = 256;
constexpr int CHUNK = 4096;

struct MtTable {
    const long long* a;
    const long long* b;
    const long long* c;
    const long long* d;
    const long long* sizes;
    const int* blk_tensor;
    const long long* blk_off;
};

__global__ void ema_k(MtTable t, float alpha, float one_minus_alpha) {
    const int ti = t.blk_tensor[blockIdx.x];
// ... 66 lines not shown
    const long long off = t.blk_off[blockIdx.x];
    float* p = (float*)t.a[ti];
    const float* g = (const float*)t.b[ti];
    float* buf = (float*)t.c[ti];
    const long long n = t.sizes[ti];
    const long long end = off + CHUNK < n ? off + CHUNK : n;
    for (long long i = off + threadIdx.x; i < end; i += TPB) {
        float gr = g[i] * gscale + wd * p[i];
        const float b = first_step ? gr : buf[i] * momentum + gr;
        buf[i] = b;
        gr = nesterov ? gr + momentum * b : b;
        p[i] -= lr * gr;
    }
}
__global__ void grad_check_k(MtTable t, float* __restrict__ state, long long g2) {
    const int ti = t.blk_tensor[blockIdx.x];
    const long long off = t.blk_off[blockIdx.x];
    const float* g = (const float*)t.b[ti];
    const long long n = t.sizes[ti];
    const long long end = off + CHUNK < n ? off + CHUNK : n;
    bool bad = false;
    long long i0 = off;
    if (((uintptr_t)(g + off) & 15) == 0 && (g2 & 15) == 0) {
        const long long n4 = (end - off) >> 2;
        for (long long q = threadIdx.x; q < n4; q += TPB) {
            f32x4 v = *(const f32x4*)(g + off + q * 4);
            if (g2) {
                const f32x4 w = *(const f32x4*)((const char*)(g + off + q * 4) + g2);
                v[0] += w[0]; v[1] += w[1]; v[2] += w[2]; v[3] += w[3];
            }
            bad = bad || !(fabsf(v[0]) <= 3.4028234e38f) || !(fabsf(v[1]) <= 3.4028234e38f) || !(fabsf(v[2]) <= 3.4028234e38f) || !(fabsf(v[3]) <= 3.4028234e38f);
        }
        i0 = off + n4 * 4;
    }
    for (long long i = i0 + threadIdx.x; i < end; i += TPB) {
        float v = g[i];
        if (g2) v += *(const float*)((const char*)(g + i) + g2);
        bad = bad || !(fabsf(v) <= 3.4028234e38f);
    }
    if (bad) state[5] = 1.f;
}
__global__ void scaler_update_k(float* __restrict__ state, float growth, float backoff, float interval) {
    float scale = state[6], tr = state[7];
    if (state[5] != 0.f) { scale *= backoff; tr = 0.f; }
    else { tr += 1.f; if (tr >= interval) { scale *= growth; tr = 0.f; } }
    state[6] = scale; state[7] = tr; state[5] = 0.f;
    state[4] = 1.f / scale;
}
struct TailJob {
    float* p; const float* g; float* m; float* v; float* t;
    elem_t* sd; elem_t* td; elem_t* sx; elem_t* tx;
    int A, T, B, adam;
    long long n;
};

struct TailHyper { float lr, beta1, beta2, eps, wd, bc1, bc2_sqrt, gscale, alpha, oma; int do_adam; long long g2; };

__device__ __forceinline__ void tail1(const TailHyper& h, bool adam, float& pv, float gr, float& mi, float& vi, float& tv) {
    if (adam) {
        gr *= h.gscale;
        if (h.wd != 0.f) gr += h.wd * pv;
        mi = mi * h.beta1 + (1.f - h.beta1) * gr;
        vi = vi * h.beta2 + (1.f - h.beta2) * gr * gr;
        pv = pv - (h.lr / h.bc1) * (mi / (sqrtf(vi) / h.bc2_sqrt + h.eps));
    }
    tv = ema1(tv, pv, h.alpha, h.oma);
}

__global__ __launch_bounds__(TPB) void opt_tail_k(const TailJob* __restrict__ jobs, const int* __restrict__ blk_job, const int* __restrict__ blk_sub,
                                                  TailHyper h, const float* __restrict__ dev_state) {
    __shared__ elem_t ts[64][66], tt[64][66];
    if (dev_state) {
        h.bc1 = dev_state[1]; h.bc2_sqrt = dev_state[2]; h.lr = dev_state[3]; h.gscale = dev_state[4];
        if (dev_state[5] != 0.f) h.do_adam = 0;
    }
    const TailJob j = jobs[blk_job[blockIdx.x]];
    const int sub = blk_sub[blockIdx.x];
    const bool adam = j.adam && h.do_adam;
    if (j.A == 0) {
        const long long off = (long long)sub * CHUNK;
        const long long end = off + CHUNK < j.n ? off + CHUNK : j.n;
        for (long long i = off + threadIdx.x; i < end; i += TPB) {
            float pv = j.p[i], tv = j.t[i], mi = 0.f, vi = 0.f;
            if (adam) { mi = j.m[i]; vi = j.v[i]; }
            float gr = adam ? j.g[i] : 0.f;
            if (adam && h.g2) gr += *(const float*)((const char*)(j.g + i) + h.g2);
            tail1(h, adam, pv, gr, mi, vi, tv);
            if (adam) { j.p[i] = pv; j.m[i] = mi; j.v[i] = vi; }
            j.t[i] = tv;
            if (j.sd) j.sd[i] = (elem_t)pv;
            if (j.td) j.td[i] = (elem_t)tv;
        }
        return;
    }
    const int tb = j.B >> 6;
    const int t = sub % j.T, tile = sub / j.T;
    const int a0 = (tile / tb) << 6, b0 = (tile % tb) << 6;
    const int r = threadIdx.x >> 4, c4 = (threadIdx.x & 15) << 2;
#pragma unroll
    for (int i = 0; i < 4; ++i) {
        const int a = r + 16 * i;
        const size_t idx = ((size_t)(a0 + a) * j.T + t) * j.B + b0 + c4;
        f32x4 pv = *(const f32x4*)(j.p + idx), tv = *(const f32x4*)(j.t + idx);
        f32x4 mi = {0.f, 0.f, 0.f, 0.f}, vi = mi, gr = mi;
        if (adam) {
            mi = *(const f32x4*)(j.m + idx); vi = *(const f32x4*)(j.v + idx); gr = *(const f32x4*)(j.g + idx);
            if (h.g2) { const f32x4 g2 = *(const f32x4*)((const char*)(j.g + idx) + h.g2); gr[0] += g2[0]; gr[1] += g2[1]; gr[2] += g2[2]; gr[3] += g2[3]; }
        }
#pragma unroll
        for (int e = 0; e < 4; ++e) {
            float p1 = pv[e], m1 = mi[e], v1 = vi[e], t1 = tv[e];
            tail1(h, adam, p1, gr[e], m1, v1, t1);
            pv[e] = p1; mi[e] = m1; vi[e] = v1; tv[e] = t1;
        }
        if (adam) { *(f32x4*)(j.p + idx) = pv; *(f32x4*)(j.m + idx) = mi; *(f32x4*)(j.v + idx) = vi; }
        *(f32x4*)(j.t + idx) = tv;
        const elem4 ps = {(elem_t)pv[0], (elem_t)pv[1], (elem_t)pv[2], (elem_t)pv[3]};
        const elem4 pt = {(elem_t)tv[0], (elem_t)tv[1], (elem_t)tv[2], (elem_t)tv[3]};
        if (j.sd) *(elem4*)(j.sd + idx) = ps;
        if (j.td) *(elem4*)(j.td + idx) = pt;
        if (j.sx) { ts[a][c4] = ps[0]; ts[a][c4 + 1] = ps[1]; ts[a][c4 + 2] = ps[2]; ts[a][c4 + 3] = ps[3]; }
        if (j.tx) { tt[a][c4] = pt[0]; tt[a][c4 + 1] = pt[1]; tt[a][c4 + 2] = pt[2]; tt[a][c4 + 3] = pt[3]; }
    }
    if (!j.sx && !j.tx) return;
    __syncthreads();
#pragma unroll
    for (int i = 0; i < 4; ++i) {
        const int b = r + 16 * i;
        const size_t idx = ((size_t)(b0 + b) * j.T + t) * j.A + a0 + c4;
        if (j.sx) { const elem4 o = {ts[c4][b], ts[c4 + 1][b], ts[c4 + 2][b], ts[c4 + 3][b]}; *(elem4*)(j.sx + idx) = o; }
        if (j.tx) { const elem4 o = {tt[c4][b], tt[c4 + 1][b], tt[c4 + 2][b], tt[c4 + 3][b]}; *(elem4*)(j.tx + idx) = o; }
    }
}
}

int opt_chunk() { return CHUNK; }
size_t opt_tail_job_bytes() { return sizeof(TailJob); }
void opt_tail_job_fill(void* dst, float* p, const float* g, float* m, float* v, float* t, void* sd, void* td, void* sx, void* tx, int A, int T, int B,
                       int adam, long long n) {
    TailJob j{p, g, m, v, t, (elem_t*)sd, (elem_t*)td, (elem_t*)sx, (elem_t*)tx, A, T, B, adam, n};
    *(TailJob*)dst = j;
}
int opt_tail(hipStream_t s, const void* d_jobs, const int* blk_job, const int* blk_sub, int nblocks, float lr, float beta1, float beta2, float eps,
             float wd, int step, float gscale, float* dev_state, float alpha, float oma, int do_adam, long long grad2_delta, int tick) {
    if (grad2_delta % 16) return UDAPOSE_ERR_ARG;
    double bc1 = 1.0, bc2 = 1.0;
    if (dev_state) { if (do_adam && tick) hipLaunchKernelGGL(adam_tick_k, dim3(1), dim3(1), 0, s, dev_state, beta1, beta2); }
    else { bc1 = 1.0 - pow((double)beta1, (double)step); bc2 = 1.0 - pow((double)beta2, (double)step); }
    if (nblocks <= 0) return UDAPOSE_OK;
    TailHyper h{lr, beta1, beta2, eps, wd, (float)bc1, (float)sqrt(bc2), gscale, alpha, oma, do_adam, grad2_delta};
    hipLaunchKernelGGL(opt_tail_k, dim3(nblocks), dim3(TPB), 0, s, (const TailJob*)d_jobs, blk_job, blk_sub, h, dev_state);
    return udapose_check_launch();
}
int opt_grad_check(hipStream_t s, const long long* g, const long long* sizes, const int* blk_tensor, const long long* blk_off, int nblocks,
                   float* dev_state, long long grad2_delta) {
    if (!dev_state || grad2_delta % 4) return UDAPOSE_ERR_ARG;
    MtTable t{nullptr, g, nullptr, nullptr, sizes, blk_tensor, blk_off};
    if (nblocks <= 0) return UDAPOSE_OK;
    hipLaunchKernelGGL(grad_check_k, dim3(nblocks), dim3(TPB), 0, s, t, dev_state, grad2_delta);
    return udapose_check_launch();
}
int opt_scaler_update(hipStream_t s, float* dev_state, float growth, float backoff, int interval) {
    if (!dev_state || interval < 1) return UDAPOSE_ERR_ARG;
    hipLaunchKernelGGL(scaler_update_k, dim3(1), dim3(1), 0, s, dev_state, growth, backoff, (float)interval);
    return udapose_check_launch();
}

int opt_ema(hipStream_t s, const long long* tgt, const long long* src, const long long* sizes, const int* blk_tensor, const long long* blk_off,
            int nblocks, float alpha, float one_minus_alpha) {
    MtTable t{tgt, src, nullptr, nullptr, sizes, blk_tensor, blk_off};
    if (nblocks <= 0) return UDAPOSE_OK;
    hipLaunchKernelGGL(ema_k, dim3(nblocks), dim3(TPB), 0, s, t, alpha, one_minus_alpha);
    return udapose_check_launch();
}
int opt_adam(hipStream_t s, const long long* p, const long long* g, const long long* m, const long long* v, const long long* sizes,
             const int* blk_tensor, const long long* blk_off, int nblocks, float lr, float beta1, float beta2, float eps, float wd, int step,
             float gscale, float* dev_state) {
    MtTable t{p, g, m, v, sizes, blk_tensor, blk_off};
    if (nblocks <= 0) return UDAPOSE_OK;
    double bc1 = 1.0, bc2 = 1.0;
    if (dev_state) hipLaunchKernelGGL(adam_tick_k, dim3(1), dim3(1), 0, s, dev_state, beta1, beta2);
    else { bc1 = 1.0 - pow((double)beta1, (double)step); bc2 = 1.0 - pow((double)beta2, (double)step); }
    hipLaunchKernelGGL(adam_k, dim3(nblocks), dim3(TPB), 0, s, t, lr, beta1, beta2, eps, wd, (float)bc1, (float)sqrt(bc2), gscale, dev_state);
    return udapose_check_launch();
}
int opt_sgd(hipStream_t s, const long long* p, const long long* g, const long long* buf, const long long* sizes, const int* blk_tensor,
            const long long* blk_off, int nblocks, float lr, float momentum, float wd, int nesterov, int first_step, float gscale,
            float* dev_state) {
    MtTable t{p, g, buf, nullptr, sizes, blk_tensor, blk_off};
    if (nblocks <= 0) return UDAPOSE_OK;
    if (dev_state) hipLaunchKernelGGL(sgd_tick_k, dim3(1), dim3(1), 0, s, dev_state);
    hipLaunchKernelGGL(sgd_k, dim3(nblocks), dim3(TPB), 0, s, t, lr, momentum, wd, nesterov, first_step, gscale, dev_state);
    return udapose_check_launch();
}

namespace {
__global__ void comm_pack_bf16_k(const float* __restrict__ src, long long n, __bf16* __restrict__ dst, long long npad) {
    for (long long i = (long long)blockIdx.x * 256 + threadIdx.x; i < npad; i += (long long)gridDim.x * 256) dst[i] = (__bf16)(i < n ? src[i] : 0.f);
}
__global__ void comm_shard_mean_k(const __bf16* __restrict__ in, int W, long long m, float inv_w, __bf16* __restrict__ out) {
    for (long long i = (long long)blockIdx.x * 256 + threadIdx.x; i < m; i += (long long)gridDim.x * 256) {
        float a = 0.f;
        for (int w = 0; w < W; ++w) a += (float)in[(long long)w * m + i];
        out[i] = (__bf16)(a * inv_w);
// ... 23 lines not shown
```

uda_poseestimation_amd/csrc/wgrad.hip:

```cpp
#include <stdlib.h>
#include "conv_plan.h"

namespace {

template <int RT, int CT, int WR, int WC>
struct WgCfg {
    static constexpr int TR = RT / WR, TC = CT / WC;
    static constexpr int MT = TR / 16, NT = TC / 16;
    static constexpr int PSTR = RT * 2 + 32, QSTR = CT * 2 + 32;
    static constexpr int P_BYTES = 32 * PSTR, Q_BYTES = 32 * QSTR;
    static constexpr int P_CH = (32 * RT / 8 + 255) / 256, Q_CH = (32 * CT / 8 + 255) / 256;
    static constexpr int LDS_BYTES = 2 * (P_BYTES + Q_BYTES);
};

template <int RT, int CT, int WR, int WC>
__global__ __launch_bounds__(256) void wgrad_kernel(const WgParams p) {
    using C = WgCfg<RT, CT, WR, WC>;
    constexpr int TR = C::TR, TC = C::TC, MT = C::MT, NT = C::NT;
    extern __shared__ __attribute__((aligned(16))) char smem[];
    const int tid = threadIdx.x, lane = tid & 63, wid = tid >> 6;
    const int wr = wid / WC, wc = wid % WC;
    const bool smallc = (p.flags & IG_FLAG_SMALLC) != 0;
    const bool swap = (p.flags & WG_FLAG_SWAP) != 0;
    const int c_tile = blockIdx.x % p.c_tiles, r_tile = blockIdx.x / p.c_tiles;
// ... 666 lines not shown
                        const int row = 32 * kk + 16 * h + 4 * g + qq + t;
                        const int off = row * 128 + ((((col >> 3) ^ wswz<64>(row)) << 4) | ((col & 4) << 1));
                        const s16x4 v = __builtin_amdgcn_ds_read_tr16_b64_v4i16(LDS_PTR(s16x4, Q + off));
                        if (h == 0) bfr[j].s.a = v; else bfr[j].s.b = v;
                    }
                }
#pragma unroll
                for (int i = 0; i < 2; ++i) {
                    F8 a = af[i];
                    if (t == 0) { a.w[0] &= mL[kk][0]; a.w[1] &= mL[kk][1]; a.w[2] &= mL[kk][2]; a.w[3] &= mL[kk][3]; }
                    if (t == 2) { a.w[0] &= mR[kk][0]; a.w[1] &= mR[kk][1]; a.w[2] &= mR[kk][2]; a.w[3] &= mR[kk][3]; }
#pragma unroll
                    for (int j = 0; j < 2; ++j) acc[t][i][j] = UDAPOSE_MFMA_16x16x32(a.v, bfr[j].v, acc[t][i][j]);
                }
            }
        }
    }

    const bool atomic = (p.flags & WG_FLAG_ATOMIC) != 0;
#pragma unroll
    for (int t = 0; t < 3; ++t)
#pragma unroll
        for (int i = 0; i < 2; ++i)
#pragma unroll
            for (int j = 0; j < 2; ++j)
#pragma unroll
                for (int r = 0; r < 4; ++r) {
                    const int rr = r0 + wr * 32 + i * 16 + (lane >> 4) * 4 + r;
                    const int cc = c0 + wc * 32 + j * 16 + (lane & 15);
                    if (rr >= p.Co || rr >= p.rows_valid || cc >= p.Ci) continue;
                    const size_t off = ((size_t)rr * p.wtaps + (3 * by + t)) * p.Ci + cc + part_off;
                    const float v = acc[t][i][j][r];
                    if (atomic) atomicAdd(p.dw + off, v);
                    else p.dw[off] = v;
                }
}

template <int RT, int CT, int WR, int WC, int NS>
__global__ __launch_bounds__(256) void wgrad_dma_kernel(const WgParams p) {
    extern __shared__ __attribute__((aligned(16))) char smem[];
    const uint32_t gxy = gridDim.x * gridDim.y;
    const uint32_t lin = xcd_remap(blockIdx.x + gridDim.x * (blockIdx.y + gridDim.y * blockIdx.z), gxy * gridDim.z);
    const uint32_t bz = lin / gxy, bxy = lin - bz * gxy;
    const uint32_t by = bxy / gridDim.x, bx = bxy - by * gridDim.x;
    if constexpr (RT == 64 && CT == 64) {
        if (p.flags & WG_FLAG_ROW3) { wgrad_row3_body<NS>(p, bx, by, bz, smem); return; }
    }
    if (p.flags & WG_FLAG_FAST2) wgrad_fast2_body<RT, CT, WR, WC, NS, 64>(p, bx, by, bz, smem);
    else if (p.flags & WG_FLAG_FASTGEO) wgrad_dma_body<RT, CT, WR, WC, NS, 64, true>(p, bx, by, bz, smem);
    else wgrad_dma_body<RT, CT, WR, WC, NS>(p, bx, by, bz, smem);
}

template <int RT, int CT, int WR, int WC, int NS, int PX>
__global__ __launch_bounds__(256) __attribute__((amdgpu_waves_per_eu(4))) void wgrad_dma_group_kernel(const WgParams* __restrict__ tab, const WgGroupBlk* __restrict__ blk,
                                                              const uint32_t per_xcd, const char* x_base, const char* dy_base, char* dw_base,
                                                              const WgParams* __restrict__ tab2, const WgGroupBlk* __restrict__ blk2,
                                                              const char* x_base2, const char* dy_base2, char* dw_base2) {
    extern __shared__ __attribute__((aligned(16))) char smem[];
    uint32_t slot = blockIdx.x >> 3;
    if (tab2) {
        if (slot & 1u) { tab = tab2; blk = blk2; x_base = x_base2; dy_base = dy_base2; dw_base = dw_base2; }
        slot >>= 1;
    }
    const WgGroupBlk b = blk[(blockIdx.x & 7u) * per_xcd + slot];
    if (b.prob < 0) return;
    const WgParams& p = tab[b.prob];
    const uint32_t gx = (uint32_t)(p.r_tiles * p.c_tiles), gxy = gx * (uint32_t)p.total_taps;
    const uint32_t bz = (uint32_t)b.local / gxy, bxy = (uint32_t)b.local - bz * gxy;
    const uint32_t by = bxy / gx, bx = bxy - by * gx;
    if constexpr (RT == 64 && CT == 64 && PX == 64) {
        if (p.flags & WG_FLAG_ROW3) { wgrad_row3_body<NS>(p, bx, by, bz, smem, (uintptr_t)x_base, (uintptr_t)dy_base, (uintptr_t)dw_base); return; }
    }
    if (p.flags & WG_FLAG_FAST2) wgrad_fast2_body<RT, CT, WR, WC, NS, PX>(p, bx, by, bz, smem, (uintptr_t)x_base, (uintptr_t)dy_base, (uintptr_t)dw_base);
    else if (p.flags & WG_FLAG_FASTGEO) wgrad_dma_body<RT, CT, WR, WC, NS, PX, true>(p, bx, by, bz, smem, (uintptr_t)x_base, (uintptr_t)dy_base, (uintptr_t)dw_base);
    else wgrad_dma_body<RT, CT, WR, WC, NS, PX>(p, bx, by, bz, smem, (uintptr_t)x_base, (uintptr_t)dy_base, (uintptr_t)dw_base);
}

template <int RT, int CT, int WR, int WC, int NS, int PX>
int launch_wd_group(const WgParams* d_tab, const WgGroupBlk* d_blk, int per_xcd, const void* x_base, const void* dy_base, void* dw_base,
                    hipStream_t stream, const WgParams* d_tab2 = nullptr, const WgGroupBlk* d_blk2 = nullptr, const void* x_base2 = nullptr,
                    const void* dy_base2 = nullptr, void* dw_base2 = nullptr) {
    using C = WdCfg<RT, CT, WR, WC, NS, PX>;
    constexpr int LDS = (RT == 64 && CT == 64 && PX == 64 && Row3Cfg::lds_bytes(NS) > C::LDS_BYTES) ? Row3Cfg::lds_bytes(NS) : C::LDS_BYTES;
    static std::atomic<unsigned long long> attr_done{0};
    static std::mutex attr_mu;
    once_per_device(attr_done, attr_mu, [] {
        (void)hipFuncSetAttribute((const void*)wgrad_dma_group_kernel<RT, CT, WR, WC, NS, PX>, hipFuncAttributeMaxDynamicSharedMemorySize, LDS);
    });
    hipLaunchKernelGGL((wgrad_dma_group_kernel<RT, CT, WR, WC, NS, PX>), dim3(8 * per_xcd * (d_tab2 ? 2 : 1)), dim3(256), LDS, stream, d_tab, d_blk,
                       (uint32_t)per_xcd, (const char*)x_base, (const char*)dy_base, (char*)dw_base, d_tab2, d_blk2, (const char*)x_base2,
                       (const char*)dy_base2, (char*)dw_base2);
    return udapose_check_launch();
}

template <int RT, int CT, int WR, int WC, int NS>
int launch_wd(WgParams& p, hipStream_t stream) {
    using C = WdCfg<RT, CT, WR, WC, NS>;
    constexpr int LDS = (RT == 64 && CT == 64 && Row3Cfg::lds_bytes(NS) > C::LDS_BYTES) ? Row3Cfg::lds_bytes(NS) : C::LDS_BYTES;
    const bool swap = (p.flags & WG_FLAG_SWAP) != 0;
    const int Rdim = swap ? p.Ci : p.Co, Cdim = swap ? p.Co : p.Ci;
    p.r_tiles = (Rdim + RT - 1) / RT;
    p.c_tiles = (Cdim + CT - 1) / CT;
    static std::atomic<unsigned long long> attr_done{0};
    static std::mutex attr_mu;
    once_per_device(attr_done, attr_mu, [] {
        (void)hipFuncSetAttribute((const void*)wgrad_dma_kernel<RT, CT, WR, WC, NS>, hipFuncAttributeMaxDynamicSharedMemorySize, LDS);
    });
    dim3 grid(p.r_tiles * p.c_tiles, p.total_taps, p.ksplit);
    hipLaunchKernelGGL((wgrad_dma_kernel<RT, CT, WR, WC, NS>), grid, dim3(256), LDS, stream, p);
    return udapose_check_launch();
}

template <int RT, int CT, int WR, int WC>
int launch_wg(WgParams& p, hipStream_t stream) {
    using C = WgCfg<RT, CT, WR, WC>;
    const bool swap = (p.flags & WG_FLAG_SWAP) != 0;
    const bool smallc = (p.flags & IG_FLAG_SMALLC) != 0;
    const int Rdim = swap ? p.Ci : p.Co, Cdim = swap ? p.Co : p.Ci;
    p.r_tiles = (Rdim + RT - 1) / RT;
    p.c_tiles = smallc ? 1 : (Cdim + CT - 1) / CT;
    const int tapsy = smallc ? p.total_taps / 4 : p.total_taps;
    dim3 grid(p.r_tiles * p.c_tiles, tapsy, p.ksplit);
    hipLaunchKernelGGL((wgrad_kernel<RT, CT, WR, WC>), grid, dim3(256), C::LDS_BYTES, stream, p);
    return udapose_check_launch();
}

}

static bool wg_fastgeo_ok(const WgParams& p, const Policy& pol) {
    const bool pow2 = ((p.Hi & (p.Hi - 1)) | (p.Wi & (p.Wi - 1))) == 0;
    return pol.wgrad_fastgeo && !(p.flags & (IG_FLAG_SMALLC | WG_FLAG_SWAP)) && p.s == 1 && p.os == 1 && p.nclass == 1 && p.Hg == p.Hi && p.Wg == p.Wi &&
           p.Hg == p.Ho && p.Wg == p.Wo && pow2 && p.Hi > 0 && p.M < (1 << 24) && p.Ci < (1 << 24) && p.Co < (1 << 24) &&
           (long long)p.M * (p.Ci > p.Co ? p.Ci : p.Co) < (1ll << 31);
}

static bool wg_row3_ok(const WgParams& p, const Policy& pol) {
    return pol.wgrad_row3 && (p.flags & WG_FLAG_ROW3_OK) && p.total_taps == 9 && p.wtaps == 9 && wg_fastgeo_ok(p, pol) && p.Wi >= 8 && p.Wi <= 64 &&
           p.Ci % 64 == 0 && p.Co % 64 == 0;
}

int wgrad_pick_tile(int Rdim, int Cdim, int smallc, const Policy& pol) {
    if (smallc) return 2;
    if (pol.wgrad_tile >= 0 && Rdim > 32) return pol.wgrad_tile;
    if (Rdim <= 32) return 3;
// ... 25 lines not shown
    while (tiles * ks < 512 && ms_total / (ks * 2) >= min_stages) ks *= 2;
    if (pol.wgrad_ksplit > 0) { ks = pol.wgrad_ksplit; while (ks > 1 && ms_total / ks < 1) ks /= 2; }
    p.ksplit = ks;
    p.part_stride = 0;
    p.msteps_per_split = (ms_total + ks - 1) / ks;
    if (ks > 1 || accumulate) p.flags |= WG_FLAG_ATOMIC; else p.flags &= ~WG_FLAG_ATOMIC;
    if (ks > 1 && !accumulate) {
        const size_t n = (size_t)Rdim * p.wtaps * Cdim;
        if (pw_zero(stream, p.dw, n * sizeof(float)) != UDAPOSE_OK) return UDAPOSE_ERR_LAUNCH;
    }
    if (wg_fastgeo_ok(p, pol)) p.flags |= WG_FLAG_FASTGEO; else p.flags &= ~WG_FLAG_FASTGEO;
    if ((p.flags & WG_FLAG_FASTGEO) && !(p.flags & WG_FLAG_ROW3) && pol.wgrad_fastgeo >= 2 && p.M % 64 == 0) p.flags |= WG_FLAG_FAST2; else p.flags &= ~WG_FLAG_FAST2;
    if (dma) return tile == 0 ? launch_wd<128, 128, 2, 2, 2>(p, stream) : launch_wd<64, 64, 2, 2, 4>(p, stream);
    switch (tile) {
        case 0: return launch_wg<128, 128, 2, 2>(p, stream);
        case 1: return launch_wg<64, 64, 2, 2>(p, stream);
        case 2: return launch_wg<64, 32, 2, 2>(p, stream);
        case 3: return launch_wg<32, 128, 1, 4>(p, stream);
        default: return UDAPOSE_ERR_ARG;
    }
}

int wgrad_group_plan(WgParams& p, int accumulate, int stages_per_block, const Policy& pol) {
    const bool smallc = (p.flags & IG_FLAG_SMALLC) != 0;
    const bool swap = (p.flags & WG_FLAG_SWAP) != 0;
    if (smallc && (swap || p.Co % 64 != 0 || p.kw <= 0 || p.kw > 8)) return -1;
    if (!smallc && (p.Ci % 64 != 0 || p.Co % 64 != 0)) return -1;
    const int Rdim = swap ? p.Ci : p.Co, Cdim = smallc ? 64 : (swap ? p.Co : p.Ci);
    p.div_hw = make_fastdiv((uint32_t)(p.Hg * p.Wg));
    p.div_w = make_fastdiv((uint32_t)p.Wg);
    int tile = (Rdim >= 128 && Cdim >= 128) ? 0 : 1;
    if (wg_row3_ok(p, pol)) {
        tile = 1;
        p.flags |= WG_FLAG_ROW3;
        p.total_taps = 3;
    }
    const int TRr = tile == 0 ? 128 : 64, TCc = tile == 1 ? 64 : 128;
    p.r_tiles = (Rdim + TRr - 1) / TRr;
    p.c_tiles = (Cdim + TCc - 1) / TCc;
    const int ms_total = (p.M + 63) / 64;
    int ks = (ms_total + stages_per_block / 2) / stages_per_block;
    if (ks < 1) ks = 1;
    p.ksplit = ks;
    p.part_stride = 0;
    p.msteps_per_split = (ms_total + ks - 1) / ks;
    if (ks > 1 || accumulate) p.flags |= WG_FLAG_ATOMIC; else p.flags &= ~WG_FLAG_ATOMIC;
    if (wg_fastgeo_ok(p, pol)) p.flags |= WG_FLAG_FASTGEO; else p.flags &= ~WG_FLAG_FASTGEO;
    if ((p.flags & WG_FLAG_FASTGEO) && !(p.flags & WG_FLAG_ROW3) && pol.wgrad_fastgeo >= 2 && p.M % 64 == 0) p.flags |= WG_FLAG_FAST2; else p.flags &= ~WG_FLAG_FAST2;
    return tile;
}

int wgrad_group_launch(hipStream_t stream, int tile, const WgParams* d_tab, const WgGroupBlk* d_blk, int per_xcd, const void* x_base,
                       const void* dy_base, void* dw_base, const WgParams* d_tab2, const WgGroupBlk* d_blk2, const void* x_base2,
                       const void* dy_base2, void* dw_base2) {
    if (per_xcd <= 0) return UDAPOSE_OK;
    if (tile == 0) return launch_wd_group<128, 128, 2, 2, 2, 32>(d_tab, d_blk, per_xcd, x_base, dy_base, dw_base, stream, d_tab2, d_blk2, x_base2, dy_base2, dw_base2);
    return launch_wd_group<64, 64, 2, 2, 2, 64>(d_tab, d_blk, per_xcd, x_base, dy_base, dw_base, stream, d_tab2, d_blk2, x_base2, dy_base2, dw_base2);
}

int wgrad_parts_plan(int M, int Ci, int Co, int total_taps, int* tile_out) {
    const int tile = (Co >= 128 && Ci >= 128 && total_taps >= 9) ? 0 : 1;
    const int RT = tile == 0 ? 128 : 64;
    const long tiles = (long)((Co + RT - 1) / RT) * ((Ci + RT - 1) / RT) * total_taps;
    const int ms_total = (M + 63) / 64;
    const int min_stages = tile == 0 ? 16 : 4;
    int ks = 1;
    while (ks < 64 && tiles * ks < 512 && ms_total / (ks * 2) >= min_stages) ks *= 2;
    if (tile_out) *tile_out = tile;
    return ks;
}

int wgrad_launch_parts(WgParams& p, float* parts, hipStream_t stream) {
    if (p.Ci % 64 || p.Co % 64 || (p.flags & (IG_FLAG_SMALLC | WG_FLAG_SWAP | WG_FLAG_ROW3_OK))) return UDAPOSE_ERR_ARG;
    int tile = 1;
    const int ks = wgrad_parts_plan(p.M, p.Ci, p.Co, p.total_taps, &tile);
    p.div_hw = make_fastdiv((uint32_t)(p.Hg * p.Wg));
    p.div_w = make_fastdiv((uint32_t)p.Wg);
    p.ksplit = ks;
    p.msteps_per_split = ((p.M + 63) / 64 + ks - 1) / ks;
    p.dw = parts;
    p.part_stride = (unsigned)((size_t)p.Co * p.wtaps * p.Ci);
    p.flags &= ~(WG_FLAG_ATOMIC | WG_FLAG_FASTGEO | WG_FLAG_FAST2 | WG_FLAG_ROW3);
    return tile == 0 ? launch_wd<128, 128, 2, 2, 2>(p, stream) : launch_wd<64, 64, 2, 2, 4>(p, stream);
}
```

uda_poseestimation_amd/engine.py:

```python
import numpy as np
import os

import torch
import torch.distributed as dist

from . import optim as fused_optim
from . import utils as mt
from . import warp
from .lib import keypoint_detection as kd
from .lib.models.loss import ConsLoss, JointsMSELoss


def _dist_on():
    if not (dist.is_available() and dist.is_initialized()):
        return False
    return dist.get_world_size() > 1 or os.environ.get("UDAPOSE_FORCE_DIST", "0") == "1"


class GradSync:

    def __init__(self, model, comm_dtype="fp32"):
        self.model = model
        self._work, self._upper, self._cstream = None, None, None
        self.comm_dtype = comm_dtype
# ... 137 lines not shown
                 t2s_alpha=(0.0, 1.0), rng=None, occlude_rate=-1.0, occlude_thresh=0.9, occlude_size=10, image_px=None, precision=None,
                 loss_scale_init=65536.0, loss_scale_interval=2000, grad_comm="fp32", criterion=None, con_criterion=None, ent_criterion=None,
                 lambda_ent=0.0):
        student, teacher = getattr(student, "module", student), getattr(teacher, "module", teacher)
        self.student, self.teacher = student, teacher
        self.criterion = criterion if criterion is not None else JointsMSELoss()
        self.con_criterion = con_criterion if con_criterion is not None else ConsLoss()
        self.ent_criterion, self.lambda_ent = ent_criterion, lambda_ent
        stu_m, tea_m = getattr(student, "module", student), getattr(teacher, "module", teacher)
        if precision in ("reference", "reference_fp32"):
            hi = "f16x2" if precision == "reference" else "fp32"
            stu_m.precision, tea_m.precision = "fp16", hi
            sn = getattr(style_net, "module", style_net)
            if sn is not None and hasattr(sn, "precision"):
                sn.precision = hi
        elif precision == "strict":
            stu_m.precision, tea_m.precision = "strict", "f16x2"
            sn = getattr(style_net, "module", style_net)
            if sn is not None and hasattr(sn, "precision"):
                sn.precision = "f16x2"
        elif precision is not None:
            stu_m.precision = precision
            tea_m.precision = precision
        sp = getattr(stu_m, "precision", "bf16")
        scaled = sp in ("fp16", "auto", "strict")
        if hasattr(tea_m, "aux_lib_kind"):
            tea_m.aux_lib_kind = "fp16" if sp in ("fp16", "strict") else "bf16"
        sc = dict(dynamic_loss_scale=True, init_scale=loss_scale_init, growth_interval=loss_scale_interval) if scaled else {}
        if use_sgd:
            self.stu_optimizer = fused_optim.FusedSGD(student.parameters(), lr=lr, momentum=0.9, weight_decay=1e-4, nesterov=True, **sc)
        else:
            self.stu_optimizer = fused_optim.FusedAdam(student.parameters(), lr=lr, **sc)
        self.tea_optimizer = mt.OldWeightEMA(teacher, student, alpha=teacher_alpha)
        self.sync = GradSync(student, comm_dtype=grad_comm)
        self.lambda_c, self.mask_ratio, self.sigma = lambda_c, mask_ratio, sigma
        self.ratio = image_size / heatmap_size
        self.style_net, self.recover = style_net, recover
        self.s2t_freq, self.t2s_freq, self.s2t_alpha, self.t2s_alpha = s2t_freq, t2s_freq, s2t_alpha, t2s_alpha
        self.rng = rng if rng is not None else np.random
        self._side = None
        self.fuse_rectify = True
        self.concurrent = True
        self.occlude_rate, self.occlude_thresh, self.occlude_size = occlude_rate, occlude_thresh, occlude_size
        self.image_px = image_px if image_px is not None else image_size
        self.device_occlusion = False
        self.occl_rng = self.rng
        self._occl = None
        self.overlap_allreduce = None
        self.fuse_tail = True
        self.stream_priority = 0
        self.merge_wgrad = True
        self.single_graph = True
        self.sum_grads_in_tail = True
        self.fused_last = False

    def _check_scaler(self):
        hd = getattr(getattr(self.student, "module", self.student), "_last_hd", None)
        if hd is not None and hd.precision in ("fp16", "strict") and getattr(self.stu_optimizer, "_scaler", None) is None:
            raise RuntimeError(f"the student ran in {hd.precision} (an fp16 backward) but the trainer's optimizer has no dynamic loss scaling: fp16 "
                               "heat-map gradients underflow without it - construct MeanTeacherTrainer with precision='fp16' / 'reference' / "
                               "'strict' / 'auto'")

    def pretrain_step(self, x_s, label_s, weight_s, x_t=None):
        self.student.train()
        self.stu_optimizer.zero_grad()
        if self.style_net is not None and self.s2t_freq > self.rng.rand():
            a = self.rng.uniform(*self.s2t_alpha)
            x_s = self.style_net(x_s, x_t, a, clamp=self.recover)[2]
        y_s = self.student(x_s)
        loss = self.criterion(y_s, label_s, weight_s)
        self._check_scaler()
        overlap = self._overlap()
        self.student.split_backward = overlap
        self.stu_optimizer.scale_loss(loss).backward()
        self.student.split_backward = False
        if overlap:
            self.sync.start_upper()
        self._sync_grads()
        self.stu_optimizer.step()
        return {"loss_all": loss.detach(), "loss_s": loss.detach(), "y_s": y_s.detach()}

    def train_step(self, x_s, label_s, weight_s, x_t_stu, x_t_teas, aug_param_stu, aug_params_tea, with_accuracy=False):
        if not isinstance(x_t_teas, (list, tuple)):
            x_t_teas, aug_params_tea = [x_t_teas], [aug_params_tea]
        n, dev = x_t_stu.shape[0], x_t_stu.device
        theta_stu = warp.recon_thetas(aug_param_stu, n, self.ratio, dev)
        thetas_tea = [warp.recon_thetas(ap, n, self.ratio, dev) for ap in aug_params_tea]
        x_s_in, x_t_teas_in = self._style_part(x_s, list(x_t_teas))
        self._occl = None
        if self.occlude_rate > -1:
            if self.device_occlusion:
                self._occl = ("device", warp.occlusion_back_thetas(aug_param_stu, n, self.ratio, dev), self.draw_occlusion_uniforms(n, dev))
            else:
                if _dist_on() and self.style_net is not None and self.occl_rng is self.rng:
                    raise RuntimeError("data parallel with style transfer: the host occlusion draws are data dependent in number and "
                                       "would take the ranks' common style decisions out of step - set trainer.device_occlusion = True "
                                       "or give the occlusion its own generator (trainer.occl_rng)")
                self._occl = ("host", aug_param_stu)
        out = self._forward_backward(x_s_in, label_s, weight_s, x_t_stu, x_t_teas_in, theta_stu, thetas_tea)
        self._sync_grads()
        self._update()
        if with_accuracy:
            _, avg_acc, cnt, _ = kd.accuracy(out["y_s"], label_s)
            out["acc_s"], out["cnt_s"] = avg_acc, cnt
        return out

# ... 89 lines not shown

    def _overlap(self):
        on = self.overlap_allreduce
        if on is None:
            on = _dist_on()
        return bool(on) and hasattr(self.student, "finish_backward")

    def _sync_grads(self):
        if self._overlap() and self.student._pending_lower:
            self._backward_lower()
            self.sync.finish()
        else:
            self.sync()

    def _backward_lower(self, grads_part=2):
        student = self.student
        main = torch.cuda.current_stream()
        streams = {id(p[5]): p[5] for p in student._pending_lower}
        for stv in streams.values():
            if stv is not main:
                stv.wait_stream(main)
        student.finish_backward()
        for stv in streams.values():
            if stv is not main:
                main.wait_stream(stv)
        student.finish_grads(part=grads_part)

    def _loss_backward_part(self, st, gathered_activates):
        student = self.student
        main, s_stu = st["main"], st["s_stu"]
        overlap = self._overlap()
        student.split_backward = bool(overlap)
        merge = (not overlap) and self.merge_wgrad and hasattr(student, "finish_wgrad")
        student.merge_wgrad = bool(merge)
        if getattr(self, "_metrics_cb", None) is not None:
            self._metrics_cb(st)
        loss_s = self.criterion(st["y_s"], st["label_s"], st["weight_s"])
        self._check_scaler()
        with torch.no_grad():
            tea_mask, _, _ = mt.confidence_mask(st["y_t_tea_recon"], self.mask_ratio, None, gathered_activates, st["activates"])
            y_t_tea_rect = st["y_t_tea_rect"] if st.get("y_t_tea_rect") is not None else mt.rectify(st["y_t_tea_recon"], sigma=self.sigma)
        loss_c = self.con_criterion(st["y_t_stu_recon"], y_t_tea_rect, tea_mask=tea_mask)
        loss_all = loss_s + self.lambda_c * loss_c
        loss_ent = None
        if self.ent_criterion is not None:
            loss_ent = self.ent_criterion(st["y_t_stu_recon"])
            loss_all = loss_all + self.lambda_ent * loss_ent
        self.stu_optimizer.scale_loss(loss_all).backward()
        if s_stu is not main:
            main.wait_stream(s_stu)
        student.split_backward = False
        if merge:
            student.merge_wgrad = False
            student.finish_wgrad()
        if overlap:
            student.finish_grads(part=1)
            if not torch.cuda.is_current_stream_capturing() or getattr(self, "capture_comm", False):
                self.sync.start_upper()
        elif student._pending_lower:
            self._backward_lower(grads_part=0)
        else:
            student.finish_grads(defer=self._tail_sums_grads())
        out = {"loss_all": loss_all.detach(), "loss_s": loss_s.detach(), "loss_c": loss_c.detach(), "y_s": st["y_s"].detach(),
               "tea_mask": tea_mask, "y_t_tea_recon": st["y_t_tea_recon"], "y_t_stu_recon": st["y_t_stu_recon"].detach()}
        if loss_ent is not None:
            out["loss_ent"] = loss_ent.detach()
        return out

    def _forward_backward(self, x_s, label_s, weight_s, x_t_stu, x_t_teas, theta_stu, thetas_tea):
        st = self._forward_part(x_s, label_s, weight_s, x_t_stu, x_t_teas, theta_stu, thetas_tea)
        return self._loss_backward_part(st, gather_activates(st["activates"]))

    def _tail_sums_grads(self):
        return bool(self.fuse_tail and self.sum_grads_in_tail and not _dist_on() and hasattr(self.stu_optimizer, "fused_tail_step")
                    and hasattr(self.student, "pending_grad_sum"))

    def _update(self):
        fuse = self.fuse_tail and hasattr(self.stu_optimizer, "fused_tail_step")
        self.fused_last = bool(fuse and self.stu_optimizer.fused_tail_step(self.student, self.teacher, self.tea_optimizer))
        if not self.fused_last:
            if hasattr(self.student, "finish_grads"):
                self.student.finish_grads()
            self.stu_optimizer.step()
            self.tea_optimizer.step()


def validate(batches, model, criterion=None):
    criterion = criterion or JointsMSELoss()
    was_training = model.training
    model.eval()
    acc_sum = acc_cnt = loss_sum = None
    n_seen = 0
    with torch.no_grad():
        for batch in batches:
            x, label, weight = batch[0], batch[1], batch[2]
            dev = next(model.parameters()).device
            x, label, weight = x.to(dev, non_blocking=True), label.to(dev, non_blocking=True), weight.to(dev, non_blocking=True)
            y = model(x)
            loss = criterion(y, label, weight)
            acc, _, _ = kd.accuracy_device(y, label)
            n = x.shape[0]
            present = (acc != -1).to(torch.float32)
            if acc_sum is None:
                acc_sum, acc_cnt, loss_sum = torch.zeros_like(acc, dtype=torch.float64), torch.zeros_like(acc, dtype=torch.float64), \
                    torch.zeros((), dtype=torch.float64, device=dev)
            acc_sum += (acc * present).double() * n
            acc_cnt += present.double() * n
            loss_sum += loss.detach().double() * n
            n_seen += n
    if was_training:
        model.train()
    if acc_sum is None:
        return [], float("nan")
    avg = torch.where(acc_cnt > 0, acc_sum / acc_cnt.clamp(min=1), torch.zeros_like(acc_sum))
    out = torch.cat([avg, (loss_sum / max(n_seen, 1)).reshape(1)]).cpu().tolist()
    sat = mt.split_saturations(reset=True)
    if sat:
        import warnings
        warnings.warn(f"validate(): {sat} f16x2 stores saturated at |x| = 65504 (or were NaN) since the last check - activations outside fp16's "
                      "range; run the model with precision='fp32' (exact, slower) to rule the format out")
    return out[:-1], out[-1]


class GraphedTrainStep:

    def __init__(self, trainer, x_s, label_s, weight_s, x_t_stu, x_t_tea, aug_param_stu, aug_param_tea, warmup=2, split=None, metrics=True,
                 capture_comm=None):
        self.metrics = bool(metrics)
# ... 442 lines not shown
```

uda_poseestimation_amd/lib/models/pose_resnet.py:

```python
import ctypes as C
import weakref

import torch
import torch.nn as nn

from ... import _hip
from ..._hip import check, lib, ptr
from .resnet import _resnet
from .resnet import Bottleneck as Bottleneck_default

__all__ = ['pose_resnet101', 'pose_resnet50']


class Upsampling(nn.Sequential):

    def __init__(self, in_channel=2048, hidden_dims=(256, 256, 256), kernel_sizes=(4, 4, 4), bias=False):
        assert len(hidden_dims) == len(kernel_sizes), 'ERROR: len(hidden_dims) is different len(kernel_sizes)'
        layers = []
        for hidden_dim, kernel_size in zip(hidden_dims, kernel_sizes):
            if kernel_size == 4:
                padding, output_padding = 1, 0
            elif kernel_size == 3:
                padding, output_padding = 1, 1
            elif kernel_size == 2:
# ... 52 lines not shown
class _PoseNetFn(torch.autograd.Function):
    @staticmethod
    def forward(ctx, x, net, need_grad, defer_bn, *params):
        out, act, hd, ws = net._run_forward(x, save=need_grad, defer_bn=defer_bn)
        ctx.net, ctx.act, ctx.hd, ctx.ws = net, act, hd, ws
        ctx.nparams = len(params)
        return out

    @staticmethod
    def backward(ctx, dout):
        net = ctx.net
        if ctx.act is None:
            raise RuntimeError("PoseResNet backward without saved activations (forward ran without grad, or backward ran twice)")
        net._run_backward(dout, ctx.act, ctx.hd, ctx.ws)
        ctx.act = ctx.ws = None
        return (None, None, None, None) + (None,) * ctx.nparams


class PoseResNet(nn.Module):
    default_precision = 'auto'
    _warned_bf16_fallback = False
    fwd_only_plans = True

    def __init__(self, backbone, upsampling, feature_dim, num_keypoints, finetune=False):
        super().__init__()
        self.backbone = backbone
        self.upsampling = upsampling
        self.head = nn.Conv2d(in_channels=feature_dim, out_channels=num_keypoints, kernel_size=1, stride=1, padding=0)
        self.finetune = finetune
        for m in self.head.modules():
            nn.init.normal_(m.weight, std=0.001)
            nn.init.constant_(m.bias, 0)
        cfg = getattr(upsampling, "_cfg", None)
        if cfg is None or cfg[:2] != ((256, 256, 256), (4, 4, 4)) or feature_dim != 256:
            raise NotImplementedError("the MI355X executor implements the reference configuration: 3 x deconv(256, k=4)")
        self._deconv_bias = bool(cfg[2])
        self.num_keypoints = num_keypoints
        self.bn_momentum = 0.1
        self.precision = type(self).default_precision
        self.aux_lib_kind = 'bf16'
        self._handles = {}
        self._ptr_cache = None
        self._flat_grad = None
        self._flat_grad2 = None
        self._grad_state = None
        self._deferred_bn = []
        self._wepoch = 0
        self._capture_token = None
        self.policy = {}
        self.split_backward = False
        self._pending_lower = []
        self.merge_wgrad = False
        self._pending_wg = []
        self._to_channels_last()

    def _to_channels_last(self):
        for p in self.parameters():
            if p.dim() == 4 and not p.data.is_contiguous(memory_format=torch.channels_last):
                p.data = p.data.contiguous(memory_format=torch.channels_last)
            elif p.dim() == 4 and p.data.stride(1) != 1:
                p.data = p.data.contiguous(memory_format=torch.channels_last)

    def _apply(self, fn, *a, **k):
        r = super()._apply(fn, *a, **k)
        self._to_channels_last()
        self._ptr_cache = None
        self._flat_grad = None
        self._flat_grad2 = None
        self._grad_state = None
        self._deferred_bn = []
        self._handles = {}
        self._pending_lower = []
        self._pending_wg = []
        self._split_off = None
        return r

    def load_state_dict(self, state_dict, strict=True, **kw):
        if any(k.startswith("module.") for k in state_dict):
            state_dict = {(k[7:] if k.startswith("module.") else k): v for k, v in state_dict.items()}
        r = super().load_state_dict(state_dict, strict=strict, **kw)
        if kw.get("assign"):
            self._ptr_cache = None
            self._to_channels_last()
            self._handles = {}
        return r

    def _pointers(self):
        params = list(self.parameters())
        bufs = list(self.buffers())
        key = (params[0].data_ptr(), params[-1].data_ptr(), bufs[0].data_ptr(), len(params))
        if self._ptr_cache is None or self._ptr_cache[0] != key:
            for p in params:
                if p.dtype != torch.float32:
                    raise RuntimeError("PoseResNet master parameters must be fp32 (bf16 compute copies are made by the executor)")
                if p.dim() == 4 and p.stride(1) != 1 and p.shape[1] != 1:
                    self._to_channels_last()
                    return self._pointers()
            pa = (C.c_void_p * len(params))(*[p.data_ptr() for p in params])
            ba = (C.c_void_p * len(bufs))(*[b.data_ptr() for b in bufs])
            self._ptr_cache = (key, pa, ba, params)
        return self._ptr_cache[1], self._ptr_cache[2], self._ptr_cache[3]

    def _grad_views(self, params):
        if self._flat_grad is None or self._flat_grad.device != params[0].device:
            total = sum(p.numel() for p in params)
            self._flat_grad = torch.zeros(total, dtype=torch.float32, device=params[0].device)
            views, off = [], 0
            for p in params:
                views.append(self._flat_grad[off:off + p.numel()].as_strided(p.shape, p.stride()))
                off += p.numel()
            self._grad_view_list = views
        return self._grad_view_list

    def resolved_precision(self, differentiable):
        prec = self.precision
        if prec not in ('auto', 'bf16', 'fp16', 'fp32', 'f16x2', 'strict'):
            raise ValueError("precision must be 'auto', 'bf16', 'fp16', 'f16x2', 'fp32' or 'strict'")
        if prec == 'strict':
            return 'strict' if differentiable else 'f16x2'
        if prec != 'auto':
            return prec
        if torch.is_autocast_enabled():
            return 'bf16' if torch.get_autocast_dtype('cuda') == torch.bfloat16 else 'fp16'
        if differentiable and not PoseResNet._warned_bf16_fallback:
            PoseResNet._warned_bf16_fallback = True
            import warnings
# ... 59 lines not shown
            cap_tok, cap_bwd = getattr(hd, "_cap", (None, False))
            same = tok is not None and cap_tok is tok
            if same and (cap_bwd or not need_bwd):
                return
            if tok is not None and getattr(hd, "maintained", False) and hd.wpack_version in ((version, need_bwd), (version, True)):
                return
            check(hd.L.udapose_net_pack_weights(hd.h, _hip.stream(), pa, ptr(hd.wpack), int(need_bwd)), "net_pack_weights")
            hd._cap = (tok, bool(need_bwd) or (same and cap_bwd))
            hd.wpack_version = None
            return
        if hd.wpack_version != (version, need_bwd) and hd.wpack_version != (version, True):
            check(hd.L.udapose_net_pack_weights(hd.h, _hip.stream(), pa, ptr(hd.wpack), int(need_bwd)), "net_pack_weights")
            hd.wpack_version = (version, need_bwd)

    def _run_forward(self, x, save, defer_bn=False):
        _hip.require_cuda(x)
        if x.dtype != torch.float32:
            x = x.float()
        x = x.contiguous()
        if save and not self.training:
            save = False
        hd = self._handle(x, differentiable=save)
        self._last_hd = hd
        if save and hd.precision in ('fp32', 'f16x2'):
            raise RuntimeError(f"precision={hd.precision!r} is forward-only (run it under torch.no_grad(), as the reference does for the teacher)")
        pa, ba, params = self._pointers()
        s = _hip.stream()
        self._pack(hd, pa, params, need_bwd=save)
        if save:
            act = torch.empty(hd.act_bytes, dtype=torch.uint8, device=x.device)
            ws = torch.empty(hd.ws.numel(), dtype=torch.uint8, device=x.device)
        else:
            if hd.act_nograd is None:
                hd.act_nograd = torch.empty(hd.act_bytes, dtype=torch.uint8, device=x.device)
            act, ws = hd.act_nograd, hd.ws
        out = torch.empty(hd.out_shape, dtype=torch.float32, device=x.device)
        defer = bool(defer_bn) and self.training
        check(hd.L.udapose_net_forward(hd.h, s, ptr(x), pa, ba, ptr(hd.wpack), ptr(act), ptr(ws), ptr(out),
                                        int(self.training) | (2 if defer else 0), float(self.bn_momentum)), "net_forward")
        if defer:
            self._deferred_bn.append((hd, act))
        return out, (act if save else None), hd, (ws if save else None)

    def apply_deferred_bn(self):
        pa, ba, params = self._pointers()
        for hd, act in self._deferred_bn:
            check(hd.L.udapose_net_apply_running(hd.h, _hip.stream(), ptr(act), ba, float(self.bn_momentum)), "net_apply_running")
        self._deferred_bn = []

    def finish_grads(self, part=0, defer=False):
        st = self._grad_state
        if defer and part == 0:
            return
        if st is not None and st[1]:
            n, off = self._flat_grad.numel(), (self.grad_split_offset() if part else 0)
            lo, cnt = (0, n) if part == 0 else ((off, n - off) if part == 1 else (0, off))
            check(lib().udapose_axpy_f32(_hip.stream(), self._flat_grad.data_ptr() + 4 * lo, self._flat_grad2.data_ptr() + 4 * lo, cnt), "axpy")
        if part != 1:
            self._grad_state = None

    def pending_grad_sum(self, take=False):
        st = self._grad_state
        if st is None or not st[1]:
            return 0
        delta = self._flat_grad2.data_ptr() - self._flat_grad.data_ptr()
        if take:
            self._grad_state = None
        return delta

    def grad_split_offset(self):
        off = getattr(self, "_split_off", None)
        if off is None:
            hd = next(iter(self._handles.values()))
            idx = hd.L.udapose_net_grad_split_param(hd.h)
            params = list(self.parameters())
            if idx < 0 or idx >= len(params):
                raise RuntimeError("this network has no layer3 boundary to split the backward at")
            off = sum(p.numel() for p in params[:idx])
            if off % 4:
                raise RuntimeError("gradient split offset is not 16-byte aligned")
            self._split_off = off
        return off

    def finish_backward(self):
        pending, self._pending_lower = self._pending_lower, []
        pa, ba, params = self._pointers()
        for hd, act, ws, gptrs, beta, stream in pending:
            with torch.cuda.stream(stream):
                check(hd.L.udapose_net_backward_part(hd.h, stream.cuda_stream, None, pa, ptr(hd.wpack), ptr(act), ptr(ws), gptrs, beta, 2), "net_backward part 2")
                act.record_stream(stream)
                ws.record_stream(stream)

    def _run_backward(self, dout, act, hd, ws):
        pa, ba, params = self._pointers()
        views = self._grad_views(params)
        cur = torch.cuda.current_stream()
        second_buffer = False
        if params[0].grad is None:
            beta = 0.0
            self._grad_state = [cur, False]
        elif params[0].grad.data_ptr() == views[0].data_ptr():
            beta = 1.0
            st = self._grad_state
            if st is not None and st[0] != cur:
                second_buffer, beta = True, (1.0 if st[1] else 0.0)
                st[1] = True
        else:
            for p, v in zip(params, views):
                if p.grad is not None:
                    v.copy_(p.grad)
                else:
                    v.zero_()
            beta = 1.0
        ga = getattr(self, "_grad_ptrs", None)
        if ga is None or ga[0] != views[0].data_ptr():
            ga = (views[0].data_ptr(), (C.c_void_p * len(views))(*[v.data_ptr() for v in views]))
            self._grad_ptrs = ga
        gptrs = ga[1]
        if second_buffer:
            if self._flat_grad2 is None or self._flat_grad2.device != self._flat_grad.device:
                self._flat_grad2 = torch.zeros_like(self._flat_grad)
                off, arr = 0, []
                for p in params:
                    arr.append(self._flat_grad2.data_ptr() + 4 * off)
                    off += p.numel()
                self._grad_ptrs2 = (C.c_void_p * len(arr))(*arr)
            gptrs = self._grad_ptrs2
        gkey = gptrs[0]
        if gkey not in hd.bound_grads:
            check(hd.L.udapose_net_bind_grads(hd.h, gptrs), "net_bind_grads")
            hd.bound_grads.add(gkey)
        dout = dout.contiguous().float()
        if self.split_backward:
            check(hd.L.udapose_net_backward_part(hd.h, _hip.stream(), ptr(dout), pa, ptr(hd.wpack), ptr(act), ptr(ws), gptrs, beta, 1), "net_backward part 1")
            self._pending_lower.append((hd, act, ws, gptrs, beta, cur))
        elif self.merge_wgrad and hd.grouped:
            check(hd.L.udapose_net_backward_phase(hd.h, _hip.stream(), ptr(dout), pa, ptr(hd.wpack), ptr(act), ptr(ws), gptrs, beta, 0, 1),
                  "net_backward gradient chain")
            self._pending_wg.append((hd, act, ws, gptrs, beta, cur))
        else:
            check(hd.L.udapose_net_backward(hd.h, _hip.stream(), ptr(dout), pa, ptr(hd.wpack), ptr(act), ptr(ws), gptrs, beta), "net_backward")
        nograd = self._no_grad_ids()
        for p, v in zip(params, views):
            if p.requires_grad and id(p) not in nograd:
                p.grad = v

    def finish_wgrad(self):
        pend, self._pending_wg = self._pending_wg, []
        if not pend:
            return
        s = _hip.stream()
        cur = torch.cuda.current_stream()
        pa, ba, params = self._pointers()
        if len(pend) == 2 and pend[0][0] is pend[1][0] and pend[0][3][0] != pend[1][3][0]:
            (hd, actA, wsA, gA, bA, _), (_, actB, wsB, gB, bB, _) = pend
            check(hd.L.udapose_net_wgrad_pair(hd.h, s, ptr(actA), ptr(wsA), gA, bA, ptr(actB), ptr(wsB), gB, bB, 0), "net_wgrad_pair")
        else:
            for hd, act, ws, gptrs, beta, _ in pend:
                check(hd.L.udapose_net_backward_phase(hd.h, s, None, pa, ptr(hd.wpack), ptr(act), ptr(ws), gptrs, beta, 0, 2), "net_backward weight gradients")
        for q in pend:
            q[1].record_stream(cur)
            q[2].record_stream(cur)

    def _no_grad_ids(self):
        fc = getattr(self.backbone, "fc", None)
        return {id(p) for p in fc.parameters()} if fc is not None else set()

    _warned_eval_grad = False

    def forward(self, x):
        params = list(self.parameters())
        need_grad = torch.is_grad_enabled() and any(p.requires_grad for p in params)
        if need_grad and not self.training:
            if not PoseResNet._warned_eval_grad:
                PoseResNet._warned_eval_grad = True
                import warnings
                warnings.warn("PoseResNet: an eval-mode forward with grad enabled is not differentiable on this path (eval-mode BatchNorm is folded into "
                              "the convolutions; there is no eval-mode BatchNorm backward): the output has no grad_fn.  Wrap evaluation in torch.no_grad(), "
                              "or call .train() for a differentiable forward.", stacklevel=2)
            with torch.no_grad():
                return _PoseNetFn.apply(x, self, False, False, *params)
        return _PoseNetFn.apply(x, self, need_grad, False, *params)

    def forward_deferred_bn(self, x):
        params = list(self.parameters())
        need_grad = torch.is_grad_enabled() and any(p.requires_grad for p in params)
        return _PoseNetFn.apply(x, self, need_grad, True, *params)

    def get_parameters(self, lr=1.):
        return [
            {'params': self.backbone.parameters(), 'lr': 0.1 * lr if self.finetune else lr},
            {'params': self.upsampling.parameters(), 'lr': lr},
            {'params': self.head.parameters(), 'lr': lr},
        ]


def _pose_resnet(arch, num_keypoints, block, layers, pretrained_backbone, deconv_with_bias, finetune=False, progress=True, **kwargs):
    backbone = _resnet(arch, block, layers, pretrained_backbone, progress, **kwargs)
    upsampling = Upsampling(backbone.out_features, bias=deconv_with_bias)
    model = PoseResNet(backbone, upsampling, 256, num_keypoints, finetune)
    return model


def pose_resnet101(num_keypoints, pretrained_backbone=True, deconv_with_bias=False, finetune=False, progress=True, **kwargs):
    return _pose_resnet('resnet101', num_keypoints, Bottleneck_default, [3, 4, 23, 3], pretrained_backbone, deconv_with_bias, finetune,
                        progress, **kwargs)


def pose_resnet50(num_keypoints, pretrained_backbone=True, deconv_with_bias=False, finetune=False, progress=True, **kwargs):
# ... 3 lines not shown
```

Measured before the change: 2031 images/sec.

## Deal wgrad blocks in fixed-size runs by stage depth and allow deferring split sums

```diff
diff --git a/include/udapose.h b/include/udapose.h
--- a/include/udapose.h
+++ b/include/udapose.h
@@ -32,6 +32,7 @@
     int wgrad_det;
     int igemm_ns3_k;
     void* timeline;
+    int wgrad_order;
 } udapose_policy;
 void udapose_policy_default(udapose_policy* p);
 
@@ -121,6 +122,11 @@
                                void* act, void* ws, void* const* h_grads, float beta, int part, int phase);
 int udapose_net_wgrad_pair(udapose_net_t net, void* stream, const void* act_a, void* ws_a, void* const* h_grads_a, float beta_a,
                            const void* act_b, void* ws_b, void* const* h_grads_b, float beta_b, int part);
+int udapose_net_wgrad_pair_defer(udapose_net_t net, void* stream, const void* act_a, void* ws_a, void* const* h_grads_a, float beta_a,
+                                 const void* act_b, void* ws_b, void* const* h_grads_b, float beta_b, int part, int* deferred);
+int udapose_net_split_sum_flush(udapose_net_t net, void* stream);
+int udapose_wgrad_deal(const int* nblk, const int* stages, int n_units, int order, int* ent_xcd, int* ent_unit, int* ent_first, int* ent_count, int cap,
+                       double* finish_out);
 long long udapose_net_grad_split_param(udapose_net_t net);
 
 int udapose_joints_mse_fwd(void* stream, const float* pred, const float* gt, const float* w, int R, int HW, float* rows, float* mean_out);
diff --git a/uda_poseestimation_amd/_hip.py b/uda_poseestimation_amd/_hip.py
--- a/uda_poseestimation_amd/_hip.py
+++ b/uda_poseestimation_amd/_hip.py
@@ -15,7 +15,7 @@
     _fields_ = [(k, C.c_int) for k in ("igemm_tile", "igemm_h3", "igemm_lean", "igemm_short_lds", "igemm_tap0", "wgrad_tile", "wgrad_ksplit",
                                        "wgrad_fastgeo", "wgrad_group", "wgrad_stages", "wgrad_group_stem", "bn_bwd_fused", "bn_fwd_chunked",
                                        "bn_bwd_chunked", "bn_bwd_pre_legacy", "igemm_wg_min", "wgrad_row3", "bn3_mask", "stem_fused", "debug_sync", "igemm_big_min", "patch_conv",
-                                       "eval_fold", "bn_xcd_rows", "wgrad_det", "igemm_ns3_k")] + [("timeline", C.c_void_p)]
+                                       "eval_fold", "bn_xcd_rows", "wgrad_det", "igemm_ns3_k")] + [("timeline", C.c_void_p), ("wgrad_order", C.c_int)]
 
 
 def policy(**overrides):
@@ -90,6 +90,9 @@
     "udapose_net_backward_part": (ci, [vp, vp, vp, vp, vp, vp, vp, vp, cf, ci]),
     "udapose_net_backward_phase": (ci, [vp, vp, vp, vp, vp, vp, vp, vp, cf, ci, ci]),
     "udapose_net_wgrad_pair": (ci, [vp, vp, vp, vp, vp, cf, vp, vp, vp, cf, ci]),
+    "udapose_net_wgrad_pair_defer": (ci, [vp, vp, vp, vp, vp, cf, vp, vp, vp, cf, ci, vp]),
+    "udapose_net_split_sum_flush": (ci, [vp, vp]),
+    "udapose_wgrad_deal": (ci, [vp, vp, ci, ci, vp, vp, vp, vp, ci, vp]),
     "udapose_net_grad_split_param": (ll, [vp]),
     "udapose_net_bind_update": (ci, [vp, vp, vp, vp, vp, vp, vp, vp, vp]),
     "udapose_net_fused_update": (ci, [vp, vp, vp, vp, vp, vp, vp, vp, vp, cf, cf, cf, cf, cf, ci, cf, vp, cf, cf, ci, ll]),
diff --git a/uda_poseestimation_amd/csrc/capi.hip b/uda_poseestimation_amd/csrc/capi.hip
--- a/uda_poseestimation_amd/csrc/capi.hip
+++ b/uda_poseestimation_amd/csrc/capi.hip
@@ -111,6 +111,9 @@
 int net_forward(void*, hipStream_t, const float*, const void* const*, void* const*, const void*, void*, void*, float*, int, float);
 int net_backward(void*, hipStream_t, const float*, const void* const*, const void*, void*, void*, void* const*, float, int, int);
 int net_wgrad_pair(void*, hipStream_t, const void*, void*, void* const*, float, const void*, void*, void* const*, float, int);
+int net_wgrad_pair_defer(void*, hipStream_t, const void*, void*, void* const*, float, const void*, void*, void* const*, float, int, int*);
+int net_split_sum_flush(void*, hipStream_t);
+int net_wgrad_deal(const int*, const int*, int, int, int*, int*, int*, int*, int, double*);
 
 static Policy from_c(const udapose_policy& c) {
     Policy p;
@@ -118,7 +121,7 @@
     p.igemm_tap0 = c.igemm_tap0; p.wgrad_tile = c.wgrad_tile; p.wgrad_ksplit = c.wgrad_ksplit; p.wgrad_fastgeo = c.wgrad_fastgeo;
     p.wgrad_group = c.wgrad_group; p.wgrad_stages = c.wgrad_stages > 0 ? c.wgrad_stages : 128; p.wgrad_group_stem = c.wgrad_group_stem;
     p.bn_bwd_fused = c.bn_bwd_fused; p.bn_fwd_chunked = c.bn_fwd_chunked; p.bn_bwd_chunked = c.bn_bwd_chunked;
-    p.bn_bwd_pre_legacy = c.bn_bwd_pre_legacy; p.igemm_wg_min = c.igemm_wg_min; p.wgrad_row3 = c.wgrad_row3; p.bn3_mask = c.bn3_mask; p.stem_fused = c.stem_fused; p.debug_sync = c.debug_sync; p.igemm_big_min = c.igemm_big_min; p.patch_conv = c.patch_conv; p.eval_fold = c.eval_fold; p.bn_xcd_rows = c.bn_xcd_rows; p.igemm_ns3_k = c.igemm_ns3_k; p.wgrad_det = c.wgrad_det; p.timeline = (unsigned long long*)c.timeline;
+    p.bn_bwd_pre_legacy = c.bn_bwd_pre_legacy; p.igemm_wg_min = c.igemm_wg_min; p.wgrad_row3 = c.wgrad_row3; p.bn3_mask = c.bn3_mask; p.stem_fused = c.stem_fused; p.debug_sync = c.debug_sync; p.igemm_big_min = c.igemm_big_min; p.patch_conv = c.patch_conv; p.eval_fold = c.eval_fold; p.bn_xcd_rows = c.bn_xcd_rows; p.igemm_ns3_k = c.igemm_ns3_k; p.wgrad_det = c.wgrad_det; p.wgrad_order = c.wgrad_order; p.timeline = (unsigned long long*)c.timeline;
     return p;
 }
 static void to_c(const Policy& p, udapose_policy* c) {
@@ -126,7 +129,7 @@
     c->igemm_tap0 = p.igemm_tap0; c->wgrad_tile = p.wgrad_tile; c->wgrad_ksplit = p.wgrad_ksplit; c->wgrad_fastgeo = p.wgrad_fastgeo;
     c->wgrad_group = p.wgrad_group; c->wgrad_stages = p.wgrad_stages; c->wgrad_group_stem = p.wgrad_group_stem;
     c->bn_bwd_fused = p.bn_bwd_fused; c->bn_fwd_chunked = p.bn_fwd_chunked; c->bn_bwd_chunked = p.bn_bwd_chunked;
-    c->bn_bwd_pre_legacy = p.bn_bwd_pre_legacy; c->igemm_wg_min = p.igemm_wg_min; c->wgrad_row3 = p.wgrad_row3; c->bn3_mask = p.bn3_mask; c->stem_fused = p.stem_fused; c->debug_sync = p.debug_sync; c->igemm_big_min = p.igemm_big_min; c->patch_conv = p.patch_conv; c->eval_fold = p.eval_fold; c->bn_xcd_rows = p.bn_xcd_rows; c->igemm_ns3_k = p.igemm_ns3_k; c->wgrad_det = p.wgrad_det; c->timeline = p.timeline;
+    c->bn_bwd_pre_legacy = p.bn_bwd_pre_legacy; c->igemm_wg_min = p.igemm_wg_min; c->wgrad_row3 = p.wgrad_row3; c->bn3_mask = p.bn3_mask; c->stem_fused = p.stem_fused; c->debug_sync = p.debug_sync; c->igemm_big_min = p.igemm_big_min; c->patch_conv = p.patch_conv; c->eval_fold = p.eval_fold; c->bn_xcd_rows = p.bn_xcd_rows; c->igemm_ns3_k = p.igemm_ns3_k; c->wgrad_det = p.wgrad_det; c->wgrad_order = p.wgrad_order; c->timeline = p.timeline;
 }
 struct Geom {
     Policy pol;
@@ -302,6 +305,16 @@
     if (!n || !act_a || !ws_a || !grads_a || !act_b || !ws_b || !grads_b) return UDAPOSE_ERR_ARG;
     return net_wgrad_pair(n, S(stream), act_a, ws_a, grads_a, beta_a, act_b, ws_b, grads_b, beta_b, part);
 }
+int udapose_net_wgrad_pair_defer(udapose_net_t n, void* stream, const void* act_a, void* ws_a, void* const* grads_a, float beta_a, const void* act_b,
+                                 void* ws_b, void* const* grads_b, float beta_b, int part, int* deferred) {
+    if (!n || !act_a || !ws_a || !grads_a || !act_b || !ws_b || !grads_b) return UDAPOSE_ERR_ARG;
+    return net_wgrad_pair_defer(n, S(stream), act_a, ws_a, grads_a, beta_a, act_b, ws_b, grads_b, beta_b, part, deferred);
+}
+int udapose_net_split_sum_flush(udapose_net_t n, void* stream) { return n ? net_split_sum_flush(n, S(stream)) : UDAPOSE_ERR_ARG; }
+int udapose_wgrad_deal(const int* nblk, const int* stages, int n_units, int order, int* ent_xcd, int* ent_unit, int* ent_first, int* ent_count, int cap,
+                       double* finish_out) {
+    return net_wgrad_deal(nblk, stages, n_units, order, ent_xcd, ent_unit, ent_first, ent_count, cap, finish_out);
+}
 int udapose_net_backward_phase(udapose_net_t n, void* stream, const float* dout, const void* const* params, const void* wpack, void* act,
                                void* ws, void* const* grads, float beta, int part, int phase) {
     if (!n) return UDAPOSE_ERR_ARG;
diff --git a/uda_poseestimation_amd/csrc/conv_plan.h b/uda_poseestimation_amd/csrc/conv_plan.h
--- a/uda_poseestimation_amd/csrc/conv_plan.h
+++ b/uda_poseestimation_amd/csrc/conv_plan.h
@@ -30,6 +30,7 @@
     int bn_xcd_rows = 1;
     int wgrad_det = 1;
     int igemm_ns3_k = 0;
+    int wgrad_order = 1;
     int debug_sync = 0;
     unsigned long long* timeline = nullptr;
 };
@@ -80,11 +81,13 @@
 int wgrad_launch(WgParams& p, int tile, int accumulate, hipStream_t stream, const Policy& pol);
 int wgrad_parts_plan(int M, int Ci, int Co, int total_taps, int* tile_out);
 int wgrad_launch_parts(WgParams& p, float* parts, hipStream_t stream);
+#define WG_STAMP_BLOCKS (1 << 17)
 #define WG_CLASSES 2
 int wgrad_group_plan(WgParams& p, int accumulate, int stages_per_block, const Policy& pol);
 int wgrad_group_launch(hipStream_t stream, int tile, const WgParams* d_tab, const WgGroupBlk* d_blk, int per_xcd, const void* x_base,
                        const void* dy_base, void* dw_base, const WgParams* d_tab2 = nullptr, const WgGroupBlk* d_blk2 = nullptr,
-                       const void* x_base2 = nullptr, const void* dy_base2 = nullptr, void* dw_base2 = nullptr);
+                       const void* x_base2 = nullptr, const void* dy_base2 = nullptr, void* dw_base2 = nullptr,
+                       unsigned long long* stamps = nullptr);
 
 struct ConvEpilogue {
     const elem_t* res = nullptr;
diff --git a/uda_poseestimation_amd/csrc/net.hip b/uda_poseestimation_amd/csrc/net.hip
--- a/uda_poseestimation_amd/csrc/net.hip
+++ b/uda_poseestimation_amd/csrc/net.hip
@@ -1,5 +1,7 @@
 #include <algorithm>
 #include <deque>
+#include <functional>
+#include <queue>
 #include <cstdio>
 #include <cstdlib>
 #include <string>
@@ -37,7 +39,9 @@
 size_t opt_tail_job_bytes();
 int opt_chunk();
 void opt_tail_job_fill(void*, float*, const float*, float*, float*, float*, void*, void*, void*, void*, int, int, int, int, long long);
-int opt_tail(hipStream_t, const void*, const int*, const int*, int, float, float, float, float, float, int, float, float*, float, float, int, long long, int);
+void opt_tail_job_split(void*, long long, unsigned, int);
+int opt_tail(hipStream_t, const void*, const int*, const int*, int, float, float, float, float, float, int, float, float*, float, float, int, long long, int,
+             const void*, const void*);
 int pw_transpose_f32(hipStream_t, const float*, float*, int, int, int);
 int pw_pack_strided_f32(hipStream_t, const float*, float*, int, int, int, int, int, int, long, long, long, long);
 int pw_bn_apply_f32(hipStream_t, const float*, const float*, float*, size_t, int, const float*, const float*, int);
@@ -121,7 +125,7 @@
     PackTab pack_fwd, pack_all;
     struct WgGroup {
         float k_beta = -1.f; int k_stages = 0; int k_part = 0;
-        bool k_det = false, k_stem = false;
+        bool k_det = false, k_stem = false; int k_order = 0;
         size_t part_bytes = 0;
         std::vector<std::pair<int, ptrdiff_t>> rel;
         std::vector<size_t> rel_bytes;
@@ -131,6 +135,8 @@
         std::vector<std::pair<ptrdiff_t, size_t>> zero;
         ZeroJob* d_zero = nullptr; int n_zero = 0;
         SumJob* d_sum = nullptr; int* d_sum_blk = nullptr; int n_sum_blk = 0;
+        int n_sum_ws_blk = 0;
+        std::vector<SumJob> h_sum;
         unsigned long long last_use = 0;
     };
     std::deque<WgGroup> wg_groups;
@@ -138,6 +144,8 @@
                     const void* k_ps = nullptr; const void* k_pt = nullptr; const void* k_g = nullptr; const void* k_m = nullptr;
                     const void* k_ws = nullptr; const void* k_wt = nullptr; };
     UpdTab upd;
+    struct Deferred { const WgGroup* G = nullptr; char* wsA = nullptr; char* wsB = nullptr; char* gA = nullptr; char* gB = nullptr; } deferred;
+    const WgGroup* upd_sum_group = nullptr;
     BnRunJob* d_runjobs = nullptr; int n_runjobs = 0; const void* runjobs_key = nullptr;
     unsigned long long wg_tick = 0;
 };
@@ -653,12 +661,49 @@
     return PartSel{true, nb - 1, 0, true};
 }
 
+#define WG_DEAL_RUN 32
+struct WgUnit { int prob, base, nblk, st; long load; };
+double wg_model_finish(const std::vector<WgUnit>& runs, const std::vector<int>& lst, int slots = 128) {
+    std::priority_queue<double, std::vector<double>, std::greater<double>> free_at;
+    for (int i = 0; i < slots; ++i) free_at.push(0.0);
+    double end = 0.0;
+    for (int ui : lst)
+        for (int l = 0; l < runs[ui].nblk; ++l) {
+            const double t = free_at.top() + runs[ui].st + 4;
+            free_at.pop();
+            free_at.push(t);
+            end = std::max(end, t);
+        }
+    return end;
+}
+void wg_deal(const std::vector<WgUnit>& units, int order, std::vector<WgUnit>& runs, std::vector<int> lst[8]) {
+    runs.clear();
+    for (const WgUnit& u : units) {
+        const int step = order == 0 ? u.nblk : WG_DEAL_RUN;
+        for (int l0 = 0; l0 < u.nblk; l0 += step) {
+            const int cnt = std::min(step, u.nblk - l0);
+            runs.push_back(WgUnit{u.prob, u.base + l0, cnt, u.st, (long)cnt * (u.st + 4)});
+        }
+    }
+    std::vector<int> idx(runs.size());
+    for (size_t i = 0; i < idx.size(); ++i) idx[i] = (int)i;
+    if (order == 0) std::stable_sort(idx.begin(), idx.end(), [&](int a, int b) { return runs[a].load > runs[b].load; });
+    else std::stable_sort(idx.begin(), idx.end(), [&](int a, int b) { return runs[a].st != runs[b].st ? runs[a].st > runs[b].st : runs[a].load > runs[b].load; });
+    long load[8] = {0, 0, 0, 0, 0, 0, 0, 0};
+    for (int k = 0; k < 8; ++k) lst[k].clear();
+    for (int ui : idx) {
+        int x = 0;
+        for (int k = 1; k < 8; ++k) if (load[k] < load[x]) x = k;
+        load[x] += runs[ui].load;
+        lst[x].push_back(ui);
+    }
+}
+
 int build_wg_group(Net& n, Net::WgGroup& G, void* const* grads, float beta, int part, bool sizing = false, size_t* need = nullptr) {
     const PartSel sel = part_sel(n, part);
     const bool upper = sel.head_up, lower = sel.stem;
     std::vector<WgParams> tab[WG_CLASSES];
-    struct Unit { int prob, z, nblk; long load; };
-    std::vector<Unit> units[WG_CLASSES];
+    std::vector<WgUnit> units[WG_CLASSES];
     G.zero.clear();
     G.rel.clear();
     G.rel_bytes.clear();
@@ -702,7 +747,7 @@
         const int ms_total = (p.M + 63) / 64, per = (ms_total + p.ksplit - 1) / p.ksplit;
         for (int z = 0; z < p.ksplit; ++z) {
             const int st = std::min(per, ms_total - z * per);
-            if (st > 0) units[t].push_back(Unit{prob, z, nblk, (long)nblk * (st + 4)});
+            if (st > 0) units[t].push_back(WgUnit{prob, z * nblk, nblk, st, (long)nblk * (st + 4)});
         }
         return UDAPOSE_OK;
     };
@@ -728,7 +773,7 @@
         const int ms_total = (p.M + 63) / 64, per = (ms_total + p.ksplit - 1) / p.ksplit;
         for (int z = 0; z < p.ksplit; ++z) {
             const int st = std::min(per, ms_total - z * per);
-            if (st > 0) units[t].push_back(Unit{prob, z, nblk, (long)nblk * (st + 4)});
+            if (st > 0) units[t].push_back(WgUnit{prob, z * nblk, nblk, st, (long)nblk * (st + 4)});
         }
     }
     if (upper) for (int i = 2; i >= 0; --i) CK(add(n.up[i]));
@@ -745,15 +790,15 @@
         if (G.d_blk[t]) { (void)hipFree(G.d_blk[t]); G.d_blk[t] = nullptr; }
         G.per_xcd[t] = 0;
         if (tab[t].empty()) continue;
-        std::stable_sort(units[t].begin(), units[t].end(), [](const Unit& a, const Unit& b) { return a.load > b.load; });
+        std::vector<int> deal[8];
+        std::vector<WgUnit> runs;
+        wg_deal(units[t], n.policy.wgrad_order, runs, deal);
         std::vector<WgGroupBlk> lst[8];
-        long load[8] = {0, 0, 0, 0, 0, 0, 0, 0};
-        for (const Unit& u : units[t]) {
-            int x = 0;
-            for (int k = 1; k < 8; ++k) if (load[k] < load[x]) x = k;
-            load[x] += u.load;
-            for (int l = 0; l < u.nblk; ++l) lst[x].push_back(WgGroupBlk{u.prob, u.z * u.nblk + l});
-        }
+        for (int x = 0; x < 8; ++x)
+            for (int ui : deal[x]) {
+                const WgUnit& u = runs[ui];
+                for (int l = 0; l < u.nblk; ++l) lst[x].push_back(WgGroupBlk{u.prob, u.base + l});
+            }
         size_t per = 0;
         for (int k = 0; k < 8; ++k) per = std::max(per, lst[k].size());
         std::vector<WgGroupBlk> flat(8 * per, WgGroupBlk{-1, 0});
@@ -777,19 +822,26 @@
     }
     if (G.d_sum) { (void)hipFree(G.d_sum); G.d_sum = nullptr; }
     if (G.d_sum_blk) { (void)hipFree(G.d_sum_blk); G.d_sum_blk = nullptr; }
-    G.n_sum_blk = 0;
+    G.n_sum_blk = 0; G.n_sum_ws_blk = 0;
     if (!sums.empty()) {
         std::vector<int> blk;
-        for (size_t j = 0; j < sums.size(); ++j)
-            for (unsigned c = 0; c < (sums[j].n + UDAPOSE_SPLIT_SUM_CHUNK - 1u) / UDAPOSE_SPLIT_SUM_CHUNK; ++c) { blk.push_back((int)j); blk.push_back((int)c); }
+        for (const int ws_jobs : {0, 1})
+            for (size_t j = 0; j < sums.size(); ++j) {
+                if ((sums[j].dst_ws != 0) != (ws_jobs != 0)) continue;
+                for (unsigned c = 0; c < (sums[j].n + UDAPOSE_SPLIT_SUM_CHUNK - 1u) / UDAPOSE_SPLIT_SUM_CHUNK; ++c) {
+                    blk.push_back((int)j); blk.push_back((int)c);
+                    G.n_sum_ws_blk += ws_jobs;
+                }
+            }
         if (hipMalloc((void**)&G.d_sum, sums.size() * sizeof(SumJob)) != hipSuccess) return UDAPOSE_ERR_LAUNCH;
         if (hipMalloc((void**)&G.d_sum_blk, blk.size() * sizeof(int)) != hipSuccess) return UDAPOSE_ERR_LAUNCH;
         if (hipMemcpy(G.d_sum, sums.data(), sums.size() * sizeof(SumJob), hipMemcpyHostToDevice) != hipSuccess) return UDAPOSE_ERR_LAUNCH;
         if (hipMemcpy(G.d_sum_blk, blk.data(), blk.size() * sizeof(int), hipMemcpyHostToDevice) != hipSuccess) return UDAPOSE_ERR_LAUNCH;
         G.n_sum_blk = (int)(blk.size() / 2);
     }
+    G.h_sum = sums;
     G.k_beta = beta; G.k_stages = n.policy.wgrad_stages; G.k_part = part;
-    G.k_det = det; G.k_stem = n.policy.wgrad_group_stem != 0; G.part_bytes = part_cur;
+    G.k_det = det; G.k_stem = n.policy.wgrad_group_stem != 0; G.part_bytes = part_cur; G.k_order = n.policy.wgrad_order;
     return UDAPOSE_OK;
 }
 
@@ -803,7 +855,8 @@
 Net::WgGroup* find_wg_group(Net& n, void* const* grads, float beta, int part) {
     const bool det = n.policy.wgrad_det && n.policy.wgrad_group, stem = n.policy.wgrad_group_stem != 0;
     for (auto& g : n.wg_groups) {
-        if (g.k_beta != beta || g.k_stages != n.policy.wgrad_stages || g.k_part != part || g.k_det != det || g.k_stem != stem) continue;
+        if (g.k_beta != beta || g.k_stages != n.policy.wgrad_stages || g.k_part != part || g.k_det != det || g.k_stem != stem ||
+            g.k_order != n.policy.wgrad_order) continue;
         if (g.k_det && g.part_bytes > n.ws_wgpart_bytes) continue;
         bool same = true;
         for (auto& r : g.rel)
@@ -860,24 +913,34 @@
     return la < hb && lb < ha;
 }
 int run_wg_group(hipStream_t s, Net& n, const char* act, char* ws, void* const* grads, float beta, int part) {
+    if (n.deferred.G) return UDAPOSE_ERR_NOT_PREPARED;
     Net::WgGroup* G = find_wg_group(n, grads, beta, part);
     if (!G) return UDAPOSE_ERR_NOT_PREPARED;
     const bool with_stem = part_sel(n, part).stem && G->k_stem;
     CK(wg_before(s, n, G, ws, grads, with_stem));
+    size_t stamped = 0;
     for (int t = 0; t < WG_CLASSES; ++t) {
         if (!G->per_xcd[t]) continue;
+        unsigned long long* stamps = nullptr;
+        if (n.policy.timeline) {
+            if (stamped + 8 * (size_t)G->per_xcd[t] > WG_STAMP_BLOCKS) return UDAPOSE_ERR_ARG;
+            stamps = n.policy.timeline + stamped * 8;
+            stamped += 8 * (size_t)G->per_xcd[t];
+        }
         const int tok = conv_prof_before(s, 2, G->flops[t]);
-        const int rc = wgrad_group_launch(s, t, G->d_tab[t], G->d_blk[t], G->per_xcd[t], act, ws, grads[0]);
+        const int rc = wgrad_group_launch(s, t, G->d_tab[t], G->d_blk[t], G->per_xcd[t], act, ws, grads[0], nullptr, nullptr, nullptr, nullptr, nullptr, stamps);
         conv_prof_after(s, tok);
         CK(rc);
     }
     return wg_after(s, n, G, ws, grads, beta, with_stem);
 }
 int run_wg_pair(hipStream_t s, Net& n, const char* actA, char* wsA, void* const* gradsA, float betaA, const char* actB, char* wsB,
-                void* const* gradsB, float betaB, int part) {
+                void* const* gradsB, float betaB, int part, bool defer = false, int* deferred = nullptr) {
+    if (deferred) *deferred = 0;
     Net::WgGroup* GA = find_wg_group(n, gradsA, betaA, part);
     Net::WgGroup* GB = find_wg_group(n, gradsB, betaB, part);
     if (!GA || !GB) return UDAPOSE_ERR_NOT_PREPARED;
+    if (n.deferred.G) return UDAPOSE_ERR_NOT_PREPARED;
     bool same = true;
     for (int t = 0; t < WG_CLASSES; ++t) same = same && GA->per_xcd[t] == GB->per_xcd[t];
     const bool with_stem = part_sel(n, part).stem && GA->k_stem;
@@ -888,16 +951,32 @@
     }
     CK(wg_before(s, n, GA, wsA, gradsA, with_stem));
     CK(wg_before(s, n, GB, wsB, gradsB, with_stem));
+    size_t stamped = 0;
     for (int t = 0; t < WG_CLASSES; ++t) {
         if (!GA->per_xcd[t]) continue;
+        unsigned long long* stamps = nullptr;
+        if (n.policy.timeline) {
+            if (stamped + 16 * (size_t)GA->per_xcd[t] > WG_STAMP_BLOCKS) return UDAPOSE_ERR_ARG;
+            stamps = n.policy.timeline + stamped * 8;
+            stamped += 16 * (size_t)GA->per_xcd[t];
+        }
         const int tok = conv_prof_before(s, 2, GA->flops[t] + GB->flops[t]);
         const int rc = wgrad_group_launch(s, t, GA->d_tab[t], GA->d_blk[t], GA->per_xcd[t], actA, wsA, gradsA[0], GB->d_tab[t], GB->d_blk[t], actB, wsB,
-                                          gradsB[0]);
+                                          gradsB[0], stamps);
         conv_prof_after(s, tok);
         CK(rc);
     }
     const bool pair_sum = GA == GB && GA->n_sum_blk > 0;
-    if (pair_sum) CK(pw_split_sum(s, GA->d_sum, GA->d_sum_blk, GA->n_sum_blk, wsA, (char*)gradsA[0], wsB, (char*)gradsB[0]));
+    const bool leave = defer && pair_sum && part == 0 && betaA == 0.f && n.upd.jobs && n.upd_sum_group == GA && n.upd.k_g == gradsA[0] &&
+                       GA->n_sum_blk > GA->n_sum_ws_blk;
+    if (leave) {
+        const int rest = GA->n_sum_blk - GA->n_sum_ws_blk;
+        CK(pw_split_sum(s, GA->d_sum, GA->d_sum_blk + 2 * rest, GA->n_sum_ws_blk, wsA, (char*)gradsA[0], wsB, (char*)gradsB[0]));
+        n.deferred = Net::Deferred{GA, wsA, wsB, (char*)gradsA[0], (char*)gradsB[0]};
+        if (deferred) *deferred = 1;
+    } else if (pair_sum) {
+        CK(pw_split_sum(s, GA->d_sum, GA->d_sum_blk, GA->n_sum_blk, wsA, (char*)gradsA[0], wsB, (char*)gradsB[0]));
+    }
     CK(wg_after(s, n, GA, wsA, gradsA, betaA, with_stem, pair_sum));
     return wg_after(s, n, GB, wsB, gradsB, betaB, with_stem, pair_sum);
 }
@@ -909,6 +988,41 @@
     if (part < 0 || part > 2 || (n.f32 && !n.strict) || !n.policy.wgrad_group) return UDAPOSE_ERR_ARG;
     DbgSyncScope dbg(n.policy.debug_sync);
     return run_wg_pair(s, n, (const char*)actA, (char*)wsA, gradsA, betaA, (const char*)actB, (char*)wsB, gradsB, betaB, part);
+}
+int net_wgrad_pair_defer(void* h, hipStream_t s, const void* actA, void* wsA, void* const* gradsA, float betaA, const void* actB, void* wsB,
+                         void* const* gradsB, float betaB, int part, int* deferred) {
+    Net& n = *(Net*)h;
+    if (part < 0 || part > 2 || (n.f32 && !n.strict) || !n.policy.wgrad_group) return UDAPOSE_ERR_ARG;
+    DbgSyncScope dbg(n.policy.debug_sync);
+    return run_wg_pair(s, n, (const char*)actA, (char*)wsA, gradsA, betaA, (const char*)actB, (char*)wsB, gradsB, betaB, part, true, deferred);
+}
+int net_split_sum_flush(void* h, hipStream_t s) {
+    Net& n = *(Net*)h;
+    const Net::Deferred d = n.deferred;
+    if (!d.G) return UDAPOSE_OK;
+    n.deferred = Net::Deferred{};
+    return pw_split_sum(s, d.G->d_sum, d.G->d_sum_blk, d.G->n_sum_blk - d.G->n_sum_ws_blk, d.wsA, d.gA, d.wsB, d.gB);
+}
+int net_wgrad_deal(const int* nblk, const int* stages, int n_units, int order, int* ent_xcd, int* ent_unit, int* ent_first, int* ent_count, int cap,
+                   double* finish_out) {
+    if (!nblk || !stages || n_units < 0 || order < 0 || order > 1 || cap < 0) return UDAPOSE_ERR_ARG;
+    std::vector<WgUnit> units;
+    for (int i = 0; i < n_units; ++i) {
+        if (nblk[i] < 1 || stages[i] < 1) return UDAPOSE_ERR_ARG;
+        units.push_back(WgUnit{i, 0, nblk[i], stages[i], (long)nblk[i] * (stages[i] + 4)});
+    }
+    std::vector<WgUnit> runs;
+    std::vector<int> lst[8];
+    wg_deal(units, order, runs, lst);
+    int ne = 0;
+    for (int x = 0; x < 8; ++x) {
+        for (int ri : lst[x]) {
+            if (ne < cap && ent_xcd && ent_unit && ent_first && ent_count) { ent_xcd[ne] = x; ent_unit[ne] = runs[ri].prob; ent_first[ne] = runs[ri].base; ent_count[ne] = runs[ri].nblk; }
+            ++ne;
+        }
+        if (finish_out) finish_out[x] = wg_model_finish(runs, lst[x]);
+    }
+    return ne;
 }
 
 int net_backward(void* h, hipStream_t s, const float* dout_nchw, const void* const* params, const void* wpack_, void* act_, void* ws_,
@@ -1064,6 +1178,9 @@
     std::vector<char> jobs;
     std::vector<int> bj, bs;
     std::vector<char> covered(n.n_params, 0);
+    const Net::WgGroup* SG = grads[0] ? find_wg_group(n, grads, 0.f, 0) : nullptr;
+    if (SG && (!SG->k_det || SG->n_sum_blk <= SG->n_sum_ws_blk)) SG = nullptr;
+    size_t split_found = 0;
     auto push = [&](int idx, void* sd, void* td, void* sx, void* tx, int A, int T, int B) -> int {
         const long long numel = n.param_numel[idx];
         const int adam = (h_m[idx] && h_v[idx] && grads[idx]) ? 1 : 0;
@@ -1074,6 +1191,13 @@
         jobs.resize(jobs.size() + jb);
         opt_tail_job_fill(jobs.data() + jobs.size() - jb, (float*)params_s[idx], (const float*)grads[idx], (float*)h_m[idx], (float*)h_v[idx],
                           (float*)params_t[idx], sd, td, sx, tx, A, T, B, adam, numel);
+        if (SG && adam)
+            for (const SumJob& sj : SG->h_sum)
+                if (!sj.dst_ws && sj.dst_off == (const char*)grads[idx] - (const char*)grads[0]) {
+                    if ((long long)sj.n != numel) return UDAPOSE_ERR_UNSUPPORTED;
+                    opt_tail_job_split(jobs.data() + jobs.size() - jb, sj.part_off, sj.stride, sj.ks);
+                    ++split_found;
+                }
         const int j = (int)(jobs.size() / jb) - 1;
         const long nb = A ? (long)(A / 64) * (B / 64) * T : (long)((numel + opt_chunk() - 1) / opt_chunk());
         for (long k = 0; k < nb; ++k) { bj.push_back(j); bs.push_back((int)k); }
@@ -1097,6 +1221,12 @@
     CK(push(n.head.w_idx, s_split ? nullptr : ws_ + n.head.wf_off, t_split ? nullptr : wt_ + n.head.wf_off, nullptr, nullptr, 0, 0, 0));
     for (int i = 0; i < n.n_params; ++i)
         if (!covered[i]) CK(push(i, nullptr, nullptr, nullptr, nullptr, 0, 0, 0));
+    if (SG) {
+        size_t want = 0;
+        for (const SumJob& sj : SG->h_sum) want += sj.dst_ws ? 0 : 1;
+        if (split_found != want) SG = nullptr;
+    }
+    n.upd_sum_group = nullptr;
     Net::UpdTab& u = n.upd;
     if (u.jobs) { (void)hipFree(u.jobs); (void)hipFree(u.blk_job); (void)hipFree(u.blk_sub); u.jobs = nullptr; }
     if (hipMalloc(&u.jobs, jobs.size()) != hipSuccess) return UDAPOSE_ERR_LAUNCH;
@@ -1107,6 +1237,7 @@
     if (hipMemcpy(u.blk_sub, bs.data(), bs.size() * sizeof(int), hipMemcpyHostToDevice) != hipSuccess) return UDAPOSE_ERR_LAUNCH;
     u.nblocks = (int)bj.size();
     u.k_ps = params_s[0]; u.k_pt = params_t[0]; u.k_g = grads[0]; u.k_m = h_m[0]; u.k_ws = wpack_s_; u.k_wt = wpack_t_;
+    n.upd_sum_group = SG;
     return UDAPOSE_OK;
 }
 
@@ -1119,7 +1250,11 @@
     const Net::UpdTab& u = n.upd;
     if (!u.jobs || u.k_ps != params_s[0] || u.k_pt != params_t[0] || u.k_g != grads[0] || u.k_m != h_m[0] || u.k_ws != wpack_s_ || u.k_wt != wpack_t_)
         return UDAPOSE_ERR_NOT_PREPARED;
-    CK(opt_tail(s, u.jobs, u.blk_job, u.blk_sub, u.nblocks, lr, beta1, beta2, eps, wd, step, gscale, dev_state, alpha, oma, do_adam, grad2_delta, 1));
+    const Net::Deferred d = n.deferred;
+    if (d.G && (d.G != n.upd_sum_group || d.gA != (char*)grads[0] || grad2_delta != (long long)(d.gB - d.gA))) return UDAPOSE_ERR_NOT_PREPARED;
+    n.deferred = Net::Deferred{};
+    CK(opt_tail(s, u.jobs, u.blk_job, u.blk_sub, u.nblocks, lr, beta1, beta2, eps, wd, step, gscale, dev_state, alpha, oma, do_adam, grad2_delta, 1,
+                d.G ? d.wsA : nullptr, d.G ? d.wsB : nullptr));
     if (n.strict)
         CK(net_pack_weights(hs, s, (const void* const*)params_s, wpack_s_, 0));
     else
diff --git a/uda_poseestimation_amd/csrc/optim.hip b/uda_poseestimation_amd/csrc/optim.hip
--- a/uda_poseestimation_amd/csrc/optim.hip
+++ b/uda_poseestimation_amd/csrc/optim.hip
@@ -142,9 +142,22 @@
     elem_t* sd; elem_t* td; elem_t* sx; elem_t* tx;
     int A, T, B, adam;
     long long n;
+    long long part_off; unsigned stride; int ks;
 };
 
-struct TailHyper { float lr, beta1, beta2, eps, wd, bc1, bc2_sqrt, gscale, alpha, oma; int do_adam; long long g2; };
+struct TailHyper { float lr, beta1, beta2, eps, wd, bc1, bc2_sqrt, gscale, alpha, oma; int do_adam; long long g2; const char* ws1; const char* ws2; };
+
+__device__ __forceinline__ float split_sum1(const float* __restrict__ part, size_t e, unsigned stride, int ks) {
+    float a = part[e];
+    for (int z = 1; z < ks; ++z) a += part[(size_t)z * stride + e];
+    return a;
+}
+__device__ __forceinline__ f32x4 split_sum4(const float* __restrict__ part, size_t e, unsigned stride, int ks) {
+    f32x4 a = *(const f32x4*)(part + e);
+#pragma unroll 4
+    for (int z = 1; z < ks; ++z) a += *(const f32x4*)(part + (size_t)z * stride + e);
+    return a;
+}
 
 __device__ __forceinline__ void tail1(const TailHyper& h, bool adam, float& pv, float gr, float& mi, float& vi, float& tv) {
     if (adam) {
@@ -157,6 +170,7 @@
     tv = ema1(tv, pv, h.alpha, h.oma);
 }
 
+template <bool SPLIT>
 __global__ __launch_bounds__(TPB) void opt_tail_k(const TailJob* __restrict__ jobs, const int* __restrict__ blk_job, const int* __restrict__ blk_sub,
                                                   TailHyper h, const float* __restrict__ dev_state) {
     __shared__ elem_t ts[64][66], tt[64][66];
@@ -173,8 +187,14 @@
         for (long long i = off + threadIdx.x; i < end; i += TPB) {
             float pv = j.p[i], tv = j.t[i], mi = 0.f, vi = 0.f;
             if (adam) { mi = j.m[i]; vi = j.v[i]; }
-            float gr = adam ? j.g[i] : 0.f;
-            if (adam && h.g2) gr += *(const float*)((const char*)(j.g + i) + h.g2);
+            float gr = 0.f;
+            if (SPLIT && adam && j.ks) {
+                gr = split_sum1((const float*)(h.ws1 + j.part_off), (size_t)i, j.stride, j.ks);
+                gr += split_sum1((const float*)(h.ws2 + j.part_off), (size_t)i, j.stride, j.ks);
+            } else if (adam) {
+                gr = j.g[i];
+                if (h.g2) gr += *(const float*)((const char*)(j.g + i) + h.g2);
+            }
             tail1(h, adam, pv, gr, mi, vi, tv);
             if (adam) { j.p[i] = pv; j.m[i] = mi; j.v[i] = vi; }
             j.t[i] = tv;
@@ -194,8 +214,15 @@
         f32x4 pv = *(const f32x4*)(j.p + idx), tv = *(const f32x4*)(j.t + idx);
         f32x4 mi = {0.f, 0.f, 0.f, 0.f}, vi = mi, gr = mi;
         if (adam) {
-            mi = *(const f32x4*)(j.m + idx); vi = *(const f32x4*)(j.v + idx); gr = *(const f32x4*)(j.g + idx);
-            if (h.g2) { const f32x4 g2 = *(const f32x4*)((const char*)(j.g + idx) + h.g2); gr[0] += g2[0]; gr[1] += g2[1]; gr[2] += g2[2]; gr[3] += g2[3]; }
+            mi = *(const f32x4*)(j.m + idx); vi = *(const f32x4*)(j.v + idx);
+            if (SPLIT && j.ks) {
+                gr = split_sum4((const float*)(h.ws1 + j.part_off), idx, j.stride, j.ks);
+                const f32x4 g2 = split_sum4((const float*)(h.ws2 + j.part_off), idx, j.stride, j.ks);
+                gr[0] += g2[0]; gr[1] += g2[1]; gr[2] += g2[2]; gr[3] += g2[3];
+            } else {
+                gr = *(const f32x4*)(j.g + idx);
+                if (h.g2) { const f32x4 g2 = *(const f32x4*)((const char*)(j.g + idx) + h.g2); gr[0] += g2[0]; gr[1] += g2[1]; gr[2] += g2[2]; gr[3] += g2[3]; }
+            }
         }
 #pragma unroll
         for (int e = 0; e < 4; ++e) {
@@ -228,18 +255,25 @@
 size_t opt_tail_job_bytes() { return sizeof(TailJob); }
 void opt_tail_job_fill(void* dst, float* p, const float* g, float* m, float* v, float* t, void* sd, void* td, void* sx, void* tx, int A, int T, int B,
                        int adam, long long n) {
-    TailJob j{p, g, m, v, t, (elem_t*)sd, (elem_t*)td, (elem_t*)sx, (elem_t*)tx, A, T, B, adam, n};
+    TailJob j{p, g, m, v, t, (elem_t*)sd, (elem_t*)td, (elem_t*)sx, (elem_t*)tx, A, T, B, adam, n, 0, 0u, 0};
     *(TailJob*)dst = j;
 }
+void opt_tail_job_split(void* dst, long long part_off, unsigned stride, int ks) {
+    TailJob& j = *(TailJob*)dst;
+    j.part_off = part_off; j.stride = stride; j.ks = ks;
+}
 int opt_tail(hipStream_t s, const void* d_jobs, const int* blk_job, const int* blk_sub, int nblocks, float lr, float beta1, float beta2, float eps,
-             float wd, int step, float gscale, float* dev_state, float alpha, float oma, int do_adam, long long grad2_delta, int tick) {
+             float wd, int step, float gscale, float* dev_state, float alpha, float oma, int do_adam, long long grad2_delta, int tick,
+             const void* split_ws1, const void* split_ws2) {
     if (grad2_delta % 16) return UDAPOSE_ERR_ARG;
+    if ((split_ws1 == nullptr) != (split_ws2 == nullptr)) return UDAPOSE_ERR_ARG;
     double bc1 = 1.0, bc2 = 1.0;
     if (dev_state) { if (do_adam && tick) hipLaunchKernelGGL(adam_tick_k, dim3(1), dim3(1), 0, s, dev_state, beta1, beta2); }
     else { bc1 = 1.0 - pow((double)beta1, (double)step); bc2 = 1.0 - pow((double)beta2, (double)step); }
     if (nblocks <= 0) return UDAPOSE_OK;
-    TailHyper h{lr, beta1, beta2, eps, wd, (float)bc1, (float)sqrt(bc2), gscale, alpha, oma, do_adam, grad2_delta};
-    hipLaunchKernelGGL(opt_tail_k, dim3(nblocks), dim3(TPB), 0, s, (const TailJob*)d_jobs, blk_job, blk_sub, h, dev_state);
+    TailHyper h{lr, beta1, beta2, eps, wd, (float)bc1, (float)sqrt(bc2), gscale, alpha, oma, do_adam, grad2_delta, (const char*)split_ws1, (const char*)split_ws2};
+    if (split_ws1) hipLaunchKernelGGL(opt_tail_k<true>, dim3(nblocks), dim3(TPB), 0, s, (const TailJob*)d_jobs, blk_job, blk_sub, h, dev_state);
+    else hipLaunchKernelGGL(opt_tail_k<false>, dim3(nblocks), dim3(TPB), 0, s, (const TailJob*)d_jobs, blk_job, blk_sub, h, dev_state);
     return udapose_check_launch();
 }
 int opt_grad_check(hipStream_t s, const long long* g, const long long* sizes, const int* blk_tensor, const long long* blk_off, int nblocks,
diff --git a/uda_poseestimation_amd/csrc/wgrad.hip b/uda_poseestimation_amd/csrc/wgrad.hip
--- a/uda_poseestimation_amd/csrc/wgrad.hip
+++ b/uda_poseestimation_amd/csrc/wgrad.hip
@@ -742,11 +742,10 @@
 }
 
 template <int RT, int CT, int WR, int WC, int NS, int PX>
-__global__ __launch_bounds__(256) __attribute__((amdgpu_waves_per_eu(4))) void wgrad_dma_group_kernel(const WgParams* __restrict__ tab, const WgGroupBlk* __restrict__ blk,
-                                                              const uint32_t per_xcd, const char* x_base, const char* dy_base, char* dw_base,
-                                                              const WgParams* __restrict__ tab2, const WgGroupBlk* __restrict__ blk2,
-                                                              const char* x_base2, const char* dy_base2, char* dw_base2) {
-    extern __shared__ __attribute__((aligned(16))) char smem[];
+__device__ __forceinline__ void wgrad_group_dispatch(const WgParams* __restrict__ tab, const WgGroupBlk* __restrict__ blk, const uint32_t per_xcd,
+                                                     const char* x_base, const char* dy_base, char* dw_base, const WgParams* __restrict__ tab2,
+                                                     const WgGroupBlk* __restrict__ blk2, const char* x_base2, const char* dy_base2, char* dw_base2,
+                                                     char* smem) {
     uint32_t slot = blockIdx.x >> 3;
     if (tab2) {
         if (slot & 1u) { tab = tab2; blk = blk2; x_base = x_base2; dy_base = dy_base2; dw_base = dw_base2; }
@@ -766,20 +765,53 @@
     else wgrad_dma_body<RT, CT, WR, WC, NS, PX>(p, bx, by, bz, smem, (uintptr_t)x_base, (uintptr_t)dy_base, (uintptr_t)dw_base);
 }
 
-template <int RT, int CT, int WR, int WC, int NS, int PX>
+template <int RT, int CT, int WR, int WC, int NS, int PX, bool STAMP = false>
+__global__ __launch_bounds__(256) __attribute__((amdgpu_waves_per_eu(4))) void wgrad_dma_group_kernel(const WgParams* __restrict__ tab, const WgGroupBlk* __restrict__ blk,
+                                                              const uint32_t per_xcd, const char* x_base, const char* dy_base, char* dw_base,
+                                                              const WgParams* __restrict__ tab2, const WgGroupBlk* __restrict__ blk2,
+                                                              const char* x_base2, const char* dy_base2, char* dw_base2,
+                                                              unsigned long long* __restrict__ stamps) {
+    extern __shared__ __attribute__((aligned(16))) char smem[];
+    if constexpr (STAMP) {
+        unsigned long long* const st = stamps + (size_t)blockIdx.x * 8;
+        const unsigned long long t0 = __builtin_amdgcn_s_memrealtime();
+        uint32_t slot = blockIdx.x >> 3, pass = 0;
+        if (tab2) { pass = slot & 1u; slot >>= 1; }
+        const WgGroupBlk b = (pass ? blk2 : blk)[(blockIdx.x & 7u) * per_xcd + slot];
+        long long stages = 0;
+        if (b.prob >= 0) {
+            const WgParams& p = (pass ? tab2 : tab)[b.prob];
+            const uint32_t gxy = (uint32_t)(p.r_tiles * p.c_tiles) * (uint32_t)p.total_taps;
+            const int bz = (int)((uint32_t)b.local / gxy), ms_total = (p.M + 63) / 64;
+            stages = ms_total - bz * p.msteps_per_split < p.msteps_per_split ? ms_total - bz * p.msteps_per_split : p.msteps_per_split;
+            if (p.flags & WG_FLAG_ROW3) stages |= 1ll << 32;
+            if (p.flags & IG_FLAG_SMALLC) stages |= 1ll << 33;
+        }
+        wgrad_group_dispatch<RT, CT, WR, WC, NS, PX>(tab, blk, per_xcd, x_base, dy_base, dw_base, tab2, blk2, x_base2, dy_base2, dw_base2, smem);
+        __syncthreads();
+        if (threadIdx.x == 0) {
+            st[0] = t0; st[1] = __builtin_amdgcn_s_memrealtime(); st[2] = blockIdx.x & 7u; st[3] = slot;
+            st[4] = (unsigned long long)(long long)b.prob; st[5] = (unsigned long long)stages; st[6] = pass; st[7] = RT;
+        }
+    } else {
+        wgrad_group_dispatch<RT, CT, WR, WC, NS, PX>(tab, blk, per_xcd, x_base, dy_base, dw_base, tab2, blk2, x_base2, dy_base2, dw_base2, smem);
+    }
+}
+
+template <int RT, int CT, int WR, int WC, int NS, int PX, bool STAMP = false>
 int launch_wd_group(const WgParams* d_tab, const WgGroupBlk* d_blk, int per_xcd, const void* x_base, const void* dy_base, void* dw_base,
                     hipStream_t stream, const WgParams* d_tab2 = nullptr, const WgGroupBlk* d_blk2 = nullptr, const void* x_base2 = nullptr,
-                    const void* dy_base2 = nullptr, void* dw_base2 = nullptr) {
+                    const void* dy_base2 = nullptr, void* dw_base2 = nullptr, unsigned long long* stamps = nullptr) {
     using C = WdCfg<RT, CT, WR, WC, NS, PX>;
     constexpr int LDS = (RT == 64 && CT == 64 && PX == 64 && Row3Cfg::lds_bytes(NS) > C::LDS_BYTES) ? Row3Cfg::lds_bytes(NS) : C::LDS_BYTES;
     static std::atomic<unsigned long long> attr_done{0};
     static std::mutex attr_mu;
     once_per_device(attr_done, attr_mu, [] {
-        (void)hipFuncSetAttribute((const void*)wgrad_dma_group_kernel<RT, CT, WR, WC, NS, PX>, hipFuncAttributeMaxDynamicSharedMemorySize, LDS);
+        (void)hipFuncSetAttribute((const void*)wgrad_dma_group_kernel<RT, CT, WR, WC, NS, PX, STAMP>, hipFuncAttributeMaxDynamicSharedMemorySize, LDS);
     });
-    hipLaunchKernelGGL((wgrad_dma_group_kernel<RT, CT, WR, WC, NS, PX>), dim3(8 * per_xcd * (d_tab2 ? 2 : 1)), dim3(256), LDS, stream, d_tab, d_blk,
+    hipLaunchKernelGGL((wgrad_dma_group_kernel<RT, CT, WR, WC, NS, PX, STAMP>), dim3(8 * per_xcd * (d_tab2 ? 2 : 1)), dim3(256), LDS, stream, d_tab, d_blk,
                        (uint32_t)per_xcd, (const char*)x_base, (const char*)dy_base, (char*)dw_base, d_tab2, d_blk2, (const char*)x_base2,
-                       (const char*)dy_base2, (char*)dw_base2);
+                       (const char*)dy_base2, (char*)dw_base2, stamps);
     return udapose_check_launch();
 }
 
@@ -911,8 +943,12 @@
 
 int wgrad_group_launch(hipStream_t stream, int tile, const WgParams* d_tab, const WgGroupBlk* d_blk, int per_xcd, const void* x_base,
                        const void* dy_base, void* dw_base, const WgParams* d_tab2, const WgGroupBlk* d_blk2, const void* x_base2,
-                       const void* dy_base2, void* dw_base2) {
+                       const void* dy_base2, void* dw_base2, unsigned long long* stamps) {
     if (per_xcd <= 0) return UDAPOSE_OK;
+    if (stamps) {
+        if (tile == 0) return launch_wd_group<128, 128, 2, 2, 2, 32, true>(d_tab, d_blk, per_xcd, x_base, dy_base, dw_base, stream, d_tab2, d_blk2, x_base2, dy_base2, dw_base2, stamps);
+        return launch_wd_group<64, 64, 2, 2, 2, 64, true>(d_tab, d_blk, per_xcd, x_base, dy_base, dw_base, stream, d_tab2, d_blk2, x_base2, dy_base2, dw_base2, stamps);
+    }
     if (tile == 0) return launch_wd_group<128, 128, 2, 2, 2, 32>(d_tab, d_blk, per_xcd, x_base, dy_base, dw_base, stream, d_tab2, d_blk2, x_base2, dy_base2, dw_base2);
     return launch_wd_group<64, 64, 2, 2, 2, 64>(d_tab, d_blk, per_xcd, x_base, dy_base, dw_base, stream, d_tab2, d_blk2, x_base2, dy_base2, dw_base2);
 }
diff --git a/uda_poseestimation_amd/engine.py b/uda_poseestimation_amd/engine.py
--- a/uda_poseestimation_amd/engine.py
+++ b/uda_poseestimation_amd/engine.py
@@ -213,6 +213,7 @@
         self.merge_wgrad = True
         self.single_graph = True
         self.sum_grads_in_tail = True
+        self.sum_splits_in_tail = False
         self.fused_last = False
 
     def _check_scaler(self):
@@ -408,7 +409,7 @@
         student.split_backward = False
         if merge:
             student.merge_wgrad = False
-            student.finish_wgrad()
+            student.finish_wgrad(defer_sum=self._tail_sums_splits())
         if overlap:
             student.finish_grads(part=1)
             if not torch.cuda.is_current_stream_capturing() or getattr(self, "capture_comm", False):
@@ -430,6 +431,9 @@
     def _tail_sums_grads(self):
         return bool(self.fuse_tail and self.sum_grads_in_tail and not _dist_on() and hasattr(self.stu_optimizer, "fused_tail_step")
                     and hasattr(self.student, "pending_grad_sum"))
+
+    def _tail_sums_splits(self):
+        return bool(self.sum_splits_in_tail and self._tail_sums_grads() and getattr(self.stu_optimizer, "_scaler", None) is None)
 
     def _update(self):
         fuse = self.fuse_tail and hasattr(self.stu_optimizer, "fused_tail_step")
diff --git a/uda_poseestimation_amd/lib/models/pose_resnet.py b/uda_poseestimation_amd/lib/models/pose_resnet.py
--- a/uda_poseestimation_amd/lib/models/pose_resnet.py
+++ b/uda_poseestimation_amd/lib/models/pose_resnet.py
@@ -128,6 +128,8 @@
         self._pending_lower = []
         self.merge_wgrad = False
         self._pending_wg = []
+        self._split_sum_hd = None
+        self.split_sums_deferred = 0
         self._to_channels_last()
 
     def _to_channels_last(self):
@@ -148,6 +150,7 @@
         self._handles = {}
         self._pending_lower = []
         self._pending_wg = []
+        self._split_sum_hd = None
         self._split_off = None
         return r
 
@@ -313,12 +316,18 @@
         st = self._grad_state
         if defer and part == 0:
             return
+        self.flush_split_sum()
         if st is not None and st[1]:
             n, off = self._flat_grad.numel(), (self.grad_split_offset() if part else 0)
             lo, cnt = (0, n) if part == 0 else ((off, n - off) if part == 1 else (0, off))
             check(lib().udapose_axpy_f32(_hip.stream(), self._flat_grad.data_ptr() + 4 * lo, self._flat_grad2.data_ptr() + 4 * lo, cnt), "axpy")
         if part != 1:
             self._grad_state = None
+
+    def flush_split_sum(self):
+        hd, self._split_sum_hd = getattr(self, "_split_sum_hd", None), None
+        if hd is not None:
+            check(hd.L.udapose_net_split_sum_flush(hd.h, _hip.stream()), "net_split_sum_flush")
 
     def pending_grad_sum(self, take=False):
         st = self._grad_state
@@ -327,6 +336,7 @@
         delta = self._flat_grad2.data_ptr() - self._flat_grad.data_ptr()
         if take:
             self._grad_state = None
+            self._split_sum_hd = None
         return delta
 
     def grad_split_offset(self):
@@ -406,7 +416,7 @@
             if p.requires_grad and id(p) not in nograd:
                 p.grad = v
 
-    def finish_wgrad(self):
+    def finish_wgrad(self, defer_sum=False):
         pend, self._pending_wg = self._pending_wg, []
         if not pend:
             return
@@ -415,7 +425,13 @@
         pa, ba, params = self._pointers()
         if len(pend) == 2 and pend[0][0] is pend[1][0] and pend[0][3][0] != pend[1][3][0]:
             (hd, actA, wsA, gA, bA, _), (_, actB, wsB, gB, bB, _) = pend
-            check(hd.L.udapose_net_wgrad_pair(hd.h, s, ptr(actA), ptr(wsA), gA, bA, ptr(actB), ptr(wsB), gB, bB, 0), "net_wgrad_pair")
+            if defer_sum:
+                took = C.c_int(0)
+                check(hd.L.udapose_net_wgrad_pair_defer(hd.h, s, ptr(actA), ptr(wsA), gA, bA, ptr(actB), ptr(wsB), gB, bB, 0, C.byref(took)), "net_wgrad_pair_defer")
+                self._split_sum_hd = hd if took.value else None
+                self.split_sums_deferred += int(took.value)
+            else:
+                check(hd.L.udapose_net_wgrad_pair(hd.h, s, ptr(actA), ptr(wsA), gA, bA, ptr(actB), ptr(wsB), gB, bB, 0), "net_wgrad_pair")
         else:
             for hd, act, ws, gptrs, beta, _ in pend:
                 check(hd.L.udapose_net_backward_phase(hd.h, s, None, pa, ptr(hd.wpack), ptr(act), ptr(ws), gptrs, beta, 0, 2), "net_backward weight gradients")
```

Measured after the change: 2052 images/sec, median of 6. +1.0%, better.
